# louislung/DAE_RNN_News_Recommendation

Measured on NVIDIA H100. Metric: articles/sec, higher is better.
Workload: dtype f32

## Files before the change

### dae_rnn_news_recommendation_b200/_cabi.py

```python
import ctypes
import ctypes as C
import os
from pathlib import Path

_PKG = Path(__file__).resolve().parent
LIB_PATH = Path(os.environ.get('DAE_SM100_LIB', _PKG / 'libdae_sm100.so'))

ACT = {'none': 0, 'sigmoid': 1, 'tanh': 2}
LOSS = {'cross_entropy': 0, 'mean_squared': 1, 'cosine_proximity': 2}
STRATEGY = {'none': 0, 'batch_all': 1, 'batch_hard': 2, 'explicit': 3}
OPT = {'gradient_descent': 0, 'ada_grad': 1, 'momentum': 2, 'adam': 3}
STAT = {'cost': 0, 'ae_loss': 1, 'triplet_loss': 2, 'fraction': 3, 'num': 4, 'sum_w': 5, 'n_valid': 6, 'sum_lw': 7,
        'triplet_sum': 8, 'n_active': 9}
STAT_SLOTS = 16
MAX_TRIPLET_BATCH = 32768
MAX_BLOCKED_BATCH = 262144


def act_code(name):
    return ACT.get(name, 0)


p, i32, i64, f32, u64, sz = C.c_void_p, C.c_int32, C.c_int64, C.c_float, C.c_uint64, C.c_size_t

_SIGNATURES = {
    'dae_version': (C.c_int, []),
    'dae_last_error': (C.c_int, [C.c_char_p, sz]),
    'dae_batch_prepare': (C.c_int, [p, i64, p, i32, p, i32, p, p, p, p, p, p, p]),
    'dae_batch_prepare_next': (C.c_int, [p, i64, i64, p, i32, p, i32, p, p, p, p, p, p, p]),
    'dae_batch_prepare_blocked': (C.c_int, [p, i64, p, i32, p, i32, p, p, p, p, p, p, p]),
    'dae_batch_prepare_next_blocked': (C.c_int, [p, i64, i64, p, i32, p, i32, p, p, p, p, p, p, p]),
    'dae_batch_commit': (C.c_int, [i32, p, p, p, p, p, p, p, p, p, p, p, p, p]),
    'dae_batch_prepare_explicit': (C.c_int, [p, i64, p, i32, i64, p, p, p]),
    'dae_step_advance': (C.c_int, [p, i64, p]),
    'dae_encode_csr_fwd': (C.c_int, [p, p, p, p, i32, i32, i32, f32, p, p, i32, p, i64, p, p, p, i64, p]),
    'dae_encode_csr_fwd_hot': (C.c_int, [p, p, p, i32, i32, i32, f32, p, p, i32, p, i64, p, p, i32, i32, p]),
    'dae_col_scan': (C.c_int, [p, i32, p, p, p]),
    'dae_encode_csr_bwd_gather': (C.c_int, [p, p, p, p, i32, i32, i32, f32, p, p, i32, p, p, i64, p, p, i32, p, p, p, p, p, p, p]),
    'dae_encode_csr_bwd': (C.c_int, [p, p, p, p, i32, i32, i32, f32, p, p, i32, p, p, i64, p, p, i32, p]),
    'dae_sgemm': (C.c_int, [i32, i32, i32, f32, p, i64, i64, p, i64, i64, f32, p, i64, p]),
    'dae_split_bf16': (C.c_int, [p, i32, i32, i64, p, p, i64, i32, f32, p]),
    'dae_sym_split_bf16': (C.c_int, [p, i32, i64, f32, p, p, i64, p]),
    'dae_gemm_bf16x3': (C.c_int, [i32, i32, i32, f32, p, p, i64, i32, p, p, i64, i32, p, i64, i32, i32, p, i32, i32, p]),
    'dae_gemm_config': (C.c_int, [i32, i32]),
    'dae_decode_prepare': (C.c_int, [i32, i32, p, p, p, p, p, p]),
    'dae_decode_fused_bf16x3': (C.c_int, [i32, i32, i32, p, p, i64, p, p, i64, p, p, p, p, p, i32, i32, p, p, p, p, i64, p, p, i32, p]),
    'dae_reduce_parts': (C.c_int, [p, i32, i32, p, p]),
    'dae_decode_loss_bwd': (C.c_int, [p, p, p, p, i32, i32, p, i32, i32, p, p, p, i64, p, p]),
    'dae_colsum': (C.c_int, [p, i32, i32, i64, p, p]),
    'dae_triplet_batch_all': (C.c_int, [p, i64, i32, p, p, p, i64, p, i32, p, p, i64, p]),
    'dae_triplet_config': (C.c_int, [i32]),
    'dae_gemm_sym_bf16x3': (C.c_int, [i32, i32, f32, p, p, i64, p, p, i64, p, i64, i32, p]),
    'dae_triplet_batch_hard': (C.c_int, [p, i64, i32, p, p, i64, p, p, p]),
    'dae_triplet_batch_all_rows': (C.c_int, [p, i64, i32, i32, i32, p, p, p, i64, p, i32, p, p, i64, p]),
    'dae_triplet_batch_hard_rows': (C.c_int, [p, i64, i32, i32, i32, p, p, i64, p, p, p]),
    'dae_triplet_batch_hard_finish': (C.c_int, [p, i32, p, p, i32, i64, p]),
    'dae_triplet_explicit': (C.c_int, [p, p, p, i32, i32, i64, f32, p, p, p, p, p]),
    'dae_step_finalize': (C.c_int, [p, p, i32, p, i32, i32, f32, p, p, p, p]),
    'dae_optimizer_step': (C.c_int, [p, p, p, p, i64, i32, f32, f32, f32, i32, p, p, p, i32, i32, i64, p]),
    'dae_rownorm_split_bf16': (C.c_int, [p, i32, i32, i64, i32, p, p, i64, p, i64, p]),
    'dae_row_argmax': (C.c_int, [p, i32, i32, i64, i64, i32, p, p, p]),
    'dae_similarity_topk_bf16x3': (C.c_int, [i32, i32, i32, p, p, i64, p, p, i64, i32, i64, i32, i32, p, i64, p, p, p]),
    'dae_similarity_topk_workspace': (C.c_int, [i32, i32, i32, i32, p]),
    'dae_csr_similarity_topk': (C.c_int, [p, p, p, i32, i64, i32, p, p, p, i32, i64, i32, i32, i64, i32, i32, p, i64, p, p, p]),
    'dae_csr_similarity_topk_workspace': (C.c_int, [i32, i32, i64, i32, i32, i32, p]),
    'dae_similarity_topk_excl_bf16x3': (C.c_int, [i32, i32, i32, p, p, i64, p, p, i64, i32, i64, i32, i32, p, i64, p, p, p, p, i64, p]),
    'dae_csr_similarity_topk_excl': (C.c_int, [p, p, p, i32, i64, i32, p, p, p, i32, i64, i32, i32, i64, i32, i32, p, i64, p, p, p, p,
                                               i64, p]),
    'dae_similarity_topk_groups_bf16x3': (C.c_int, [i32, i32, i32, p, p, i64, p, p, i64, i32, i64, i32, i32, p, i64, p, p, p, p, i64, p,
                                                    p]),
    'dae_csr_similarity_topk_groups': (C.c_int, [p, p, p, i32, i64, i32, p, p, p, i32, i64, i32, i32, i64, i32, i32, p, i64, p, p, p, p,
                                                 i64, p, p]),
    'dae_pair_partition': (C.c_int, [p, i64, i32, p, p, p, p, p]),
    'dae_auroc_count': (C.c_int, [p, i64, p, i64, i32, p, p]),
    'dae_similarity_pair_hist_bf16x3': (C.c_int, [i32, i32, p, p, i64, p, f32, i32, p, p, p]),
    'dae_csr_similarity_pair_hist': (C.c_int, [p, p, p, i32, i64, i32, p, f32, i32, p, i64, p, p, p]),
    'dae_csr_similarity_pair_hist_workspace': (C.c_int, [i32, i64, i32, p]),
    'dae_similarity_pairs_bf16x3': (C.c_int, [i32, i32, i32, p, p, i64, p, p, i64, i32, f32, p, i64, p, p, p, p]),
    'dae_csr_similarity_pairs': (C.c_int, [p, p, p, i32, i64, i32, p, p, p, i32, i64, i32, i32, f32, p, i64, p, i64, p, p, p, p]),
    'dae_csr_similarity_pairs_workspace': (C.c_int, [i32, i32, i64, i32, p]),
    'dae_pairs_sort': (C.c_int, [i64, i32, i32, p, p, p, p, p, i64, p, p]),
    'dae_pairs_sort_workspace': (C.c_int, [i64, i32, p]),
    'dae_allreduce_multimem': (C.c_int, [p, p, p, i32, i32, i64, i32, p]),
    'dae_mask_values': (C.c_int, [p, p, i64, f32, u64, u64, p, p]),
    'dae_salt_pepper_csr': (C.c_int, [p, p, p, i64, i64, i32, i64, f32, f32, p, u64, u64, p, p, p, i64, p, p, sz, p]),
    'dae_salt_pepper_workspace': (C.c_int, [i64, p]),
    'dae_gather_split_bf16': (C.c_int, [p, i64, p, i32, i32, p, p, i64, i32, p]),
    'dae_gru_cell_fwd': (C.c_int, [i32, i32, p, i64, p, i64, p, i64, p, i64, i32, p, p, i64, p, i64, p]),
    'dae_gru_cell_bwd': (C.c_int, [i32, i32, p, i64, p, i64, p, i64, p, i64, p, p, p, p, i64, p]),
    'dae_seq_negatives': (C.c_int, [p, i64, i32, u64, u64, u64, p, p]),
    'dae_seq_rank_loss': (C.c_int, [p, i64, p, i64, i32, p, p, i64, f32, p, i64, p, p]),
    'dae_gemm_det_workspace': (C.c_int, [p]),
    'dae_gemm_bf16x3_det': (C.c_int, [i32, i32, i32, f32, p, p, i64, i32, p, p, i64, i32, p, i64, i32, i32, p, i32, i32, p, i64, p]),
    'dae_gemm_sym_bf16x3_det': (C.c_int, [i32, i32, f32, p, p, i64, p, p, i64, p, i64, i32, p, i64, p]),
    'dae_decode_loss_parts': (C.c_int, [i32, p]),
    'dae_decode_fused_bf16x3_det': (C.c_int, [i32, i32, i32, p, p, i64, p, p, i64, p, p, p, p, p, i32, i32, p, p, p, p, i64, p, p, i32,
                                              p]),
    'dae_encode_csr_bwd_det_workspace': (C.c_int, [i32, i32, i32, i64, p]),
    'dae_encode_csr_bwd_det': (C.c_int, [p, p, p, p, i32, i32, i32, f32, p, p, i32, p, p, i64, p, p, i64, p, i64, p]),
    'dae_encode_sparse_dw_add': (C.c_int, [i32, i32, i32, i64, p, i64, p, p]),
    'dae_triplet_batch_all_det': (C.c_int, [p, i64, i32, p, p, p, i64, p, i32, p, p, i64, p, p]),
    'dae_triplet_batch_hard_det': (C.c_int, [p, i64, i32, p, p, i64, p, p, p, p]),
    'dae_triplet_batch_all_rows_det': (C.c_int, [p, i64, i32, i32, i32, p, p, p, i64, p, i32, p, p, i64, p, p]),
    'dae_triplet_batch_hard_rows_det': (C.c_int, [p, i64, i32, i32, i32, p, p, i64, p, p, p, p]),
    'dae_triplet_explicit_det': (C.c_int, [p, p, p, i32, i32, i64, f32, p, p, p, p, p, p]),
    'dae_triplet_loss_sum': (C.c_int, [p, i32, p, p]),
}


def query(name, *args, ctype=C.c_int64):
    out = ctype(0)
    call(name, *args, ctypes.addressof(out))
    return int(out.value)

_lib = None


class DaeError(RuntimeError):
    pass


def exported_symbols():
    return list(_SIGNATURES)


def lib():
    global _lib
    if _lib is None:
        if not LIB_PATH.exists():
            raise DaeError('%s not found: build it with `python -m dae_rnn_news_recommendation_b200.build` '
                           '(there is no CPU fallback)' % LIB_PATH)
        l = ctypes.CDLL(str(LIB_PATH))
        for name, (res, args) in _SIGNATURES.items():
            fn = getattr(l, name)
            fn.restype = res
            fn.argtypes = args
        _lib = l
    return _lib


def last_error():
    buf = ctypes.create_string_buffer(512)
    lib().dae_last_error(buf, 512)
    return buf.value.decode()


def call(name, *args):
    rc = getattr(lib(), name)(*args)
    if rc != 0:
        raise DaeError('%s failed (%d): %s' % (name, rc, last_error()))


def ptr(t):
    return None if t is None else t.data_ptr()
```

### dae_rnn_news_recommendation_b200/csrc/gemm_tc.cu

```cuda
#include <cuda.h>
#include <cuda_bf16.h>
#include <type_traits>
#include "common.cuh"
#include "pair_hist.cuh"
#include "pairs.cuh"
#include "topk.cuh"

namespace dae {

constexpr int BLOCK_M = 128;
constexpr int BLOCK_K = 64;
constexpr int WGMMA_K = 16;
constexpr int kThreads = 384;
constexpr int kDecodeN = 128;

__device__ __forceinline__ uint32_t smem_u32(const void* p) { return (uint32_t)__cvta_generic_to_shared(p); }

__device__ __forceinline__ void mbar_init(uint64_t* bar, uint32_t count) {
  asm volatile("mbarrier.init.shared::cta.b64 [%0], %1;" ::"r"(smem_u32(bar)), "r"(count));
}
__device__ __forceinline__ void mbar_expect_tx(uint64_t* bar, uint32_t bytes) {
  asm volatile("mbarrier.arrive.expect_tx.shared::cta.b64 _, [%0], %1;" ::"r"(smem_u32(bar)), "r"(bytes) : "memory");
}
__device__ __forceinline__ void mbar_arrive(uint64_t* bar) {
  asm volatile("mbarrier.arrive.shared::cta.b64 _, [%0];" ::"r"(smem_u32(bar)) : "memory");
}
__device__ __forceinline__ bool mbar_try_wait(uint64_t* bar, uint32_t parity) {
  uint32_t ok;
  asm volatile(
      "{\n"
      ".reg .pred p;\n"
      "mbarrier.try_wait.parity.shared::cta.b64 p, [%1], %2;\n"
      "selp.u32 %0, 1, 0, p;\n"
      "}\n"
      : "=r"(ok)
      : "r"(smem_u32(bar)), "r"(parity)
      : "memory");
  return ok != 0;
}
__device__ __forceinline__ void mbar_wait(uint64_t* bar, uint32_t parity) {
  uint32_t spins = 0;
  while (!mbar_try_wait(bar, parity)) {
    if (++spins > 4096u) {
      __nanosleep(64);
      if (spins > (1u << 26)) __trap();
    }
  }
}
__device__ __forceinline__ void fence_barrier_init() { asm volatile("fence.mbarrier_init.release.cluster;" ::: "memory"); }

__device__ __forceinline__ void tma_load_2d(const CUtensorMap* map, uint64_t* bar, void* dst, int c0, int c1) {
  asm volatile(
      "cp.async.bulk.tensor.2d.shared::cluster.global.mbarrier::complete_tx::bytes [%0], [%1, {%3, %4}], [%2];" ::"r"(smem_u32(dst)),
      "l"(map), "r"(smem_u32(bar)), "r"(c0), "r"(c1)
      : "memory");
}
__device__ __forceinline__ uint32_t cluster_ctarank() { uint32_t r; asm volatile("mov.u32 %0, %%cluster_ctarank;" : "=r"(r)); return r; }
__device__ __forceinline__ void cluster_sync_all() {
  asm volatile("barrier.cluster.arrive.release.aligned;" ::: "memory");
  asm volatile("barrier.cluster.wait.acquire.aligned;" ::: "memory");
}
__device__ __forceinline__ void tma_load_2d_mc(const CUtensorMap* map, uint64_t* bar, void* dst, int c0, int c1, uint16_t cta_mask) {
  asm volatile(
      "cp.async.bulk.tensor.2d.shared::cluster.global.mbarrier::complete_tx::bytes.multicast::cluster [%0], [%1, {%3, %4}], [%2], %5;" ::"r"(
          smem_u32(dst)),
      "l"(map), "r"(smem_u32(bar)), "r"(c0), "r"(c1), "h"(cta_mask)
      : "memory");
}
__device__ __forceinline__ void mbar_arrive_cluster(uint64_t* bar, uint32_t rank) {
  uint32_t raddr;
  asm volatile("mapa.shared::cluster.u32 %0, %1, %2;" : "=r"(raddr) : "r"(smem_u32(bar)), "r"(rank));
  asm volatile("mbarrier.arrive.release.cluster.shared::cluster.b64 _, [%0];" ::"r"(raddr) : "memory");
}
__device__ __forceinline__ void mbar_wait_cluster(uint64_t* bar, uint32_t parity) {
  uint32_t spins = 0;
  for (;;) {
    uint32_t ok;
    asm volatile(
        "{\n"
        ".reg .pred p;\n"
        "mbarrier.try_wait.parity.acquire.cluster.shared::cta.b64 p, [%1], %2;\n"
        "selp.u32 %0, 1, 0, p;\n"
        "}\n"
        : "=r"(ok)
        : "r"(smem_u32(bar)), "r"(parity)
        : "memory");
    if (ok) return;
    if (++spins > 4096u) { __nanosleep(64); if (spins > (1u << 26)) __trap(); }
  }
}

__device__ __forceinline__ void prefetch_tmap(const CUtensorMap* map) {
  asm volatile("prefetch.tensormap [%0];" ::"l"(map) : "memory");
}
__device__ __forceinline__ void named_bar_sync(int id, int threads) { asm volatile("bar.sync %0, %1;" ::"r"(id), "r"(threads) : "memory"); }

__device__ __forceinline__ void wgmma_fence() { asm volatile("wgmma.fence.sync.aligned;" ::: "memory"); }
__device__ __forceinline__ void wgmma_commit() { asm volatile("wgmma.commit_group.sync.aligned;" ::: "memory"); }
template <int N>
__device__ __forceinline__ void wgmma_wait() { asm volatile("wgmma.wait_group.sync.aligned %0;" ::"n"(N) : "memory"); }

__device__ __forceinline__ uint64_t make_desc(uint32_t saddr, uint32_t lbo_bytes, uint32_t sbo_bytes, uint32_t layout = 1) {
  uint64_t d = 0;
  d |= (uint64_t)((saddr >> 4) & 0x3FFF);
  d |= (uint64_t)((lbo_bytes >> 4) & 0x3FFF) << 16;
  d |= (uint64_t)((sbo_bytes >> 4) & 0x3FFF) << 32;
  d |= (uint64_t)layout << 62;
  return d;
}


template <int TA, int TB>
__device__ __forceinline__ void wgmma_n128(float (&d)[64], uint64_t da, uint64_t db, uint32_t scale_d) {
  asm volatile(
      "{\n"
      ".reg .pred p;\n"
      "setp.ne.b32 p, %66, 0;\n"
      "wgmma.mma_async.sync.aligned.m64n128k16.f32.bf16.bf16 "
      "{%0, %1, %2, %3, %4, %5, %6, %7, %8, %9, %10, %11, %12, %13, %14, %15, %16, %17, %18, %19, %20, %21, %22, %23, %24, %25, %26, %27, %28, %29, %30, %31, %32, %33, %34, %35, %36, %37, %38, %39, %40, %41, %42, %43, %44, %45, %46, %47, %48, %49, %50, %51, %52, %53, %54, %55, %56, %57, %58, %59, %60, %61, %62, %63}, %64, %65, p, 1, 1, %67, %68;\n"
      "}\n"
      : "+f"(d[0]), "+f"(d[1]), "+f"(d[2]), "+f"(d[3]), "+f"(d[4]), "+f"(d[5]), "+f"(d[6]), "+f"(d[7]), "+f"(d[8]), "+f"(d[9]), "+f"(d[10]), "+f"(d[11]), "+f"(d[12]), "+f"(d[13]), "+f"(d[14]), "+f"(d[15]), "+f"(d[16]), "+f"(d[17]), "+f"(d[18]), "+f"(d[19]), "+f"(d[20]), "+f"(d[21]), "+f"(d[22]), "+f"(d[23]), "+f"(d[24]), "+f"(d[25]), "+f"(d[26]), "+f"(d[27]), "+f"(d[28]), "+f"(d[29]), "+f"(d[30]), "+f"(d[31]), "+f"(d[32]), "+f"(d[33]), "+f"(d[34]), "+f"(d[35]), "+f"(d[36]), "+f"(d[37]), "+f"(d[38]), "+f"(d[39]), "+f"(d[40]), "+f"(d[41]), "+f"(d[42]), "+f"(d[43]), "+f"(d[44]), "+f"(d[45]), "+f"(d[46]), "+f"(d[47]), "+f"(d[48]), "+f"(d[49]), "+f"(d[50]), "+f"(d[51]), "+f"(d[52]), "+f"(d[53]), "+f"(d[54]), "+f"(d[55]), "+f"(d[56]), "+f"(d[57]), "+f"(d[58]), "+f"(d[59]), "+f"(d[60]), "+f"(d[61]), "+f"(d[62]), "+f"(d[63])
      : "l"(da), "l"(db), "r"(scale_d), "n"(TA), "n"(TB));
}

template <int TA, int TB>
__device__ __forceinline__ void wgmma_n64(float (&d)[32], uint64_t da, uint64_t db, uint32_t scale_d) {
  asm volatile(
      "{\n"
      ".reg .pred p;\n"
      "setp.ne.b32 p, %34, 0;\n"
      "wgmma.mma_async.sync.aligned.m64n64k16.f32.bf16.bf16 "
      "{%0, %1, %2, %3, %4, %5, %6, %7, %8, %9, %10, %11, %12, %13, %14, %15, %16, %17, %18, %19, %20, %21, %22, %23, %24, %25, %26, %27, %28, %29, %30, %31}, %32, %33, p, 1, 1, %35, %36;\n"
      "}\n"
      : "+f"(d[0]), "+f"(d[1]), "+f"(d[2]), "+f"(d[3]), "+f"(d[4]), "+f"(d[5]), "+f"(d[6]), "+f"(d[7]), "+f"(d[8]), "+f"(d[9]), "+f"(d[10]), "+f"(d[11]), "+f"(d[12]), "+f"(d[13]), "+f"(d[14]), "+f"(d[15]), "+f"(d[16]), "+f"(d[17]), "+f"(d[18]), "+f"(d[19]), "+f"(d[20]), "+f"(d[21]), "+f"(d[22]), "+f"(d[23]), "+f"(d[24]), "+f"(d[25]), "+f"(d[26]), "+f"(d[27]), "+f"(d[28]), "+f"(d[29]), "+f"(d[30]), "+f"(d[31])
      : "l"(da), "l"(db), "r"(scale_d), "n"(TA), "n"(TB));
}

struct GemmParams {
  int M, N, K;
  int k_splits;
  int stream_k;
  int atomic;
  int a_mn, b_mn;
  int a_sym_kb;
  float alpha;
  float* C;
  int64_t ldc;
  int n_store;
  int special_col;
  float* special_out;
  const int64_t* indptr; const int32_t* indices; const float* values; const int32_t* rows;
  const float* bv; const float* weight; const double* stats;
  __nv_bfloat16* dz_hi; __nv_bfloat16* dz_lo; int64_t ld_dz;
  float* row_loss_part;
  const int32_t* tile_ptr;
  float* sk_ws;
  int loss_parts;
};

struct Sched {
  int tiles_m, tiles, kb_total, kb_per_split, n_work, stream, w, n_cta;
  long long u, u_end;
  __device__ __forceinline__ void init(const GemmParams& p, int block_n, int pair = 0, int block_k = BLOCK_K) {
    const int cta = pair ? (int)(blockIdx.x >> 1) : (int)blockIdx.x;
    n_cta = pair ? (int)(gridDim.x >> 1) : (int)gridDim.x;
    tiles_m = (p.M + BLOCK_M - 1) / BLOCK_M;
    if (pair) tiles_m = (tiles_m + 1) / 2;
    tiles = tiles_m * ((p.N + block_n - 1) / block_n);
    kb_total = (p.K + block_k - 1) / block_k;
    stream = p.stream_k;
    kb_per_split = (kb_total + p.k_splits - 1) / p.k_splits;
    n_work = tiles * p.k_splits;
    w = cta;
    const long long U = (long long)tiles * kb_total;
    u = (long long)cta * U / n_cta;
    u_end = (long long)(cta + 1) * U / n_cta;
  }
  __device__ __forceinline__ bool next(int& mb, int& nb, int& kb0, int& kb1) {
    int tile;
    if (stream) {
      if (u >= u_end) return false;
      tile = (int)(u / kb_total);
      kb0 = (int)(u - (long long)tile * kb_total);
      const long long left = u_end - u;
      kb1 = (left < (long long)(kb_total - kb0)) ? kb0 + (int)left : kb_total;
      u += kb1 - kb0;
    } else {
      if (w >= n_work) return false;
      tile = w % tiles;
      kb0 = (w / tiles) * kb_per_split;
      kb1 = min(kb_total, kb0 + kb_per_split);
      w += n_cta;
    }
    mb = tile % tiles_m;
    nb = tile / tiles_m;
    return true;
  }
};

__device__ __forceinline__ uint32_t pack_bf16(float a, float b) {
  const __nv_bfloat162 v = __floats2bfloat162_rn(a, b);
  return *reinterpret_cast<const uint32_t*>(&v);
}
__device__ __forceinline__ float f_rcp(float x) { float r; asm("rcp.approx.ftz.f32 %0, %1;" : "=f"(r) : "f"(x)); return r; }
__device__ __forceinline__ float f_lg2(float x) { float r; asm("lg2.approx.ftz.f32 %0, %1;" : "=f"(r) : "f"(x)); return r; }
__device__ __forceinline__ float f_ex2(float x) { float r; asm("ex2.approx.ftz.f32 %0, %1;" : "=f"(r) : "f"(x)); return r; }
constexpr float kLog2e = 1.4426950408889634f;

template <int ACT>
__device__ __forceinline__ float act_fast(float z) {
  if (ACT == DAE_ACT_SIGMOID) return f_rcp(1.0f + f_ex2(-kLog2e * z));
  if (ACT == DAE_ACT_TANH) return 1.0f - 2.0f * f_rcp(1.0f + f_ex2(2.0f * kLog2e * z));
  return z;
}


__device__ __forceinline__ float select16(const uint32_t (&r)[16], int j) {
  uint32_t v = r[0];
#pragma unroll
  for (int k = 1; k < 16; ++k) v = (j == k) ? r[k] : v;
  return __uint_as_float(v);
}

template <int ACT, int LOSS>
__device__ __forceinline__ void decode_chunk_generic(const uint32_t (&r)[16], const float* __restrict__ bias, float sc, bool edge,
                                                     int n_lim, int nc, uint32_t (&hpk)[8], uint32_t (&lpk)[8], float& lsum) {
#pragma unroll
  for (int j2 = 0; j2 < 8; ++j2) {
    float dzp[2];
#pragma unroll
    for (int e = 0; e < 2; ++e) {
      const int j = 2 * j2 + e;
      const float z = __uint_as_float(r[j]) + bias[j];
      const float d = act_fast<ACT>(z);
      float dz, lt;
      if (LOSS == DAE_LOSS_CE) {
        const float omd = 1.0f - d;
        const float b = omd + kEps;
        lt = -f_lg2(b);
        dz = (ACT == DAE_ACT_SIGMOID) ? ((omd != 0.0f) ? sc * d : 0.0f) : sc * act_grad_from_y<ACT>(d) * f_rcp(b);
      } else {
        lt = d * d;
        dz = 2.0f * sc * d * act_grad_from_y<ACT>(d);
      }
      if (edge) { const bool in = (nc + j < n_lim); lt = in ? lt : 0.0f; dz = in ? dz : 0.0f; }
      lsum += lt;
      dzp[e] = dz;
    }
    const uint32_t hp = pack_bf16(dzp[0], dzp[1]);
    hpk[j2] = hp;
    lpk[j2] = pack_bf16(dzp[0] - __uint_as_float(hp << 16), dzp[1] - __uint_as_float(hp & 0xffff0000u));
  }
}

__device__ __forceinline__ bool decode_chunk_sigmoid_ce(const uint32_t (&r)[16], const float* __restrict__ biasc, float sc,
                                                        uint32_t (&hpk)[8], uint32_t (&lpk)[8], float& lsum) {
  bool ok = true;
#pragma unroll
  for (int g = 0; g < 4; ++g) {
    float t[4], a[4];
#pragma unroll
    for (int j = 0; j < 4; ++j) {
      t[j] = f_ex2(fmaf(__uint_as_float(r[4 * g + j]), kLog2e, biasc[4 * g + j]));
      a[j] = 1.0f + t[j];
    }
    const float p01 = a[0] * a[1], p23 = a[2] * a[3], P = p01 * p23;
    ok = ok && (P <= 22026.0f);
    const float Rs = f_rcp(P) * sc;
    lsum += f_lg2(P);
    const float r23 = Rs * p23, r01 = Rs * p01;
    const float dz0 = t[0] * (r23 * a[1]), dz1 = t[1] * (r23 * a[0]), dz2 = t[2] * (r01 * a[3]), dz3 = t[3] * (r01 * a[2]);
    const uint32_t h0 = pack_bf16(dz0, dz1), h1 = pack_bf16(dz2, dz3);
    hpk[2 * g] = h0; hpk[2 * g + 1] = h1;
    lpk[2 * g] = pack_bf16(dz0 - __uint_as_float(h0 << 16), dz1 - __uint_as_float(h0 & 0xffff0000u));
    lpk[2 * g + 1] = pack_bf16(dz2 - __uint_as_float(h1 << 16), dz3 - __uint_as_float(h1 & 0xffff0000u));
  }
  return ok;
}

template <int BLOCK_N, int TA, int TB, int BK = BLOCK_K>
__device__ __forceinline__ void mma_kblock(float (&acc)[BLOCK_N / 2], uint32_t sa_hi, uint32_t sa_lo, uint32_t sb_hi, uint32_t sb_lo,
                                           bool first) {
  static_assert(BK == 64 || BK == 32, "k-blocks are 32 or 64 wide");
  constexpr uint32_t kmaj_layout = BK == 64 ? 1u : 2u, kmaj_sbo = BK == 64 ? 1024u : 512u, mn_lbo = 64u * BK * 2u;
  constexpr uint32_t a_layout = TA ? 1u : kmaj_layout, b_layout = TB ? 1u : kmaj_layout;
  constexpr uint32_t a_sbo = TA ? 1024u : kmaj_sbo, b_sbo = TB ? 1024u : kmaj_sbo;
  constexpr uint32_t a_lbo = TA ? mn_lbo : 16u, b_lbo = TB ? mn_lbo : 16u;
  constexpr uint32_t a_step = TA ? 2048u : 32u, b_step = TB ? 2048u : 32u;
#pragma unroll
  for (int k = 0; k < BK / WGMMA_K; ++k) {
    const uint64_t da_hi = make_desc(sa_hi + k * a_step, a_lbo, a_sbo, a_layout), da_lo = make_desc(sa_lo + k * a_step, a_lbo, a_sbo, a_layout);
    const uint64_t db_hi = make_desc(sb_hi + k * b_step, b_lbo, b_sbo, b_layout), db_lo = make_desc(sb_lo + k * b_step, b_lbo, b_sbo, b_layout);
    const uint32_t sc = (first && k == 0) ? 0u : 1u;
    if constexpr (BLOCK_N == 128) {
      wgmma_n128<TA, TB>(acc, da_lo, db_hi, sc);
      wgmma_n128<TA, TB>(acc, da_hi, db_lo, 1u);
      wgmma_n128<TA, TB>(acc, da_hi, db_hi, 1u);
    } else {
      wgmma_n64<TA, TB>(acc, da_lo, db_hi, sc);
      wgmma_n64<TA, TB>(acc, da_hi, db_lo, 1u);
      wgmma_n64<TA, TB>(acc, da_hi, db_hi, 1u);
    }
  }
}

__device__ __forceinline__ void stage_ld16(const float* src, uint32_t (&r)[16]) {
#pragma unroll
  for (int q = 0; q < 4; ++q) {
    const float4 v = reinterpret_cast<const float4*>(src)[q];
    r[4 * q] = __float_as_uint(v.x); r[4 * q + 1] = __float_as_uint(v.y); r[4 * q + 2] = __float_as_uint(v.z); r[4 * q + 3] = __float_as_uint(v.w);
  }
}


template <int BLOCK_N, int STAGES, int PAIR, int BK = BLOCK_K, class SchedT>
__device__ __forceinline__ void tma_produce(const GemmParams& p, SchedT& sched, uint8_t* smem, uint64_t* full_bar, uint64_t* empty_bar,
                                            uint32_t crank, const CUtensorMap* tm_a_hi, const CUtensorMap* tm_a_lo,
                                            const CUtensorMap* tm_b_hi, const CUtensorMap* tm_b_lo, const CUtensorMap* tm_at_hi,
                                            const CUtensorMap* tm_at_lo) {
  constexpr int A_TILE = BLOCK_M * BK * 2;
  constexpr int B_TILE = BLOCK_N * BK * 2;
  constexpr int STAGE_BYTES = 2 * A_TILE + 2 * B_TILE;
  int stage = 0; uint32_t phase = 0;
  int mb, nb, kb0, kb1;
  while (sched.next(mb, nb, kb0, kb1)) {
    for (int kb = kb0; kb < kb1; ++kb) {
      if (PAIR) mbar_wait_cluster(&empty_bar[stage], phase ^ 1); else mbar_wait(&empty_bar[stage], phase ^ 1);
      uint8_t* sa_hi = smem + stage * STAGE_BYTES;
      uint8_t* sa_lo = sa_hi + A_TILE;
      uint8_t* sb_hi = sa_lo + A_TILE;
      uint8_t* sb_lo = sb_hi + B_TILE;
      const int mt = PAIR ? mb * 2 + (int)crank : mb;
      mbar_expect_tx(&full_bar[stage], STAGE_BYTES);
      if (p.a_sym_kb > 0 && kb >= p.a_sym_kb) {
#pragma unroll
        for (int j = 0; j < BLOCK_M / 64; ++j) {
          tma_load_2d(tm_at_hi, &full_bar[stage], sa_hi + j * (64 * BK * 2), mt * BLOCK_M + j * 64, (kb - p.a_sym_kb) * BK);
          tma_load_2d(tm_at_lo, &full_bar[stage], sa_lo + j * (64 * BK * 2), mt * BLOCK_M + j * 64, (kb - p.a_sym_kb) * BK);
        }
      } else if (!p.a_mn) {
        tma_load_2d(tm_a_hi, &full_bar[stage], sa_hi, kb * BK, mt * BLOCK_M);
        tma_load_2d(tm_a_lo, &full_bar[stage], sa_lo, kb * BK, mt * BLOCK_M);
      } else {
#pragma unroll
        for (int j = 0; j < BLOCK_M / 64; ++j) {
          tma_load_2d(tm_a_hi, &full_bar[stage], sa_hi + j * (64 * BK * 2), mt * BLOCK_M + j * 64, kb * BK);
          tma_load_2d(tm_a_lo, &full_bar[stage], sa_lo + j * (64 * BK * 2), mt * BLOCK_M + j * 64, kb * BK);
        }
      }
      const int kbb = (p.a_sym_kb > 0 && kb >= p.a_sym_kb) ? kb - p.a_sym_kb : kb;
      if (PAIR) {
        const int off = (int)crank * 8192, n_half = nb * BLOCK_N + (int)crank * 64;
        if (!p.b_mn) {
          tma_load_2d_mc(tm_b_hi, &full_bar[stage], sb_hi + off, kbb * BK, n_half, 0x3);
          tma_load_2d_mc(tm_b_lo, &full_bar[stage], sb_lo + off, kbb * BK, n_half, 0x3);
        } else {
          tma_load_2d_mc(tm_b_hi, &full_bar[stage], sb_hi + off, n_half, kbb * BK, 0x3);
          tma_load_2d_mc(tm_b_lo, &full_bar[stage], sb_lo + off, n_half, kbb * BK, 0x3);
        }
      } else if (!p.b_mn) {
        tma_load_2d(tm_b_hi, &full_bar[stage], sb_hi, kbb * BK, nb * BLOCK_N);
        tma_load_2d(tm_b_lo, &full_bar[stage], sb_lo, kbb * BK, nb * BLOCK_N);
      } else {
#pragma unroll
        for (int j = 0; j < BLOCK_N / 64; ++j) {
          tma_load_2d(tm_b_hi, &full_bar[stage], sb_hi + j * (64 * BK * 2), nb * BLOCK_N + j * 64, kbb * BK);
          tma_load_2d(tm_b_lo, &full_bar[stage], sb_lo + j * (64 * BK * 2), nb * BLOCK_N + j * 64, kbb * BK);
        }
      }
      if (++stage == STAGES) { stage = 0; phase ^= 1; }
    }
  }
}

template <int BLOCK_N, int STAGES, int PAIR, int MAJ, int BK = BLOCK_K>
__device__ __forceinline__ void mma_work_item(float (&acc)[BLOCK_N / 2], const GemmParams& p, uint8_t* smem, uint64_t* full_bar,
                                              uint64_t* empty_bar, int wg, int lane, uint32_t crank, int& stage, uint32_t& phase,
                                              int kb0, int kb1) {
  constexpr int A_TILE = BLOCK_M * BK * 2;
  constexpr int B_TILE = BLOCK_N * BK * 2;
  constexpr int STAGE_BYTES = 2 * A_TILE + 2 * B_TILE;
  auto release = [&](int s) {
    __syncwarp();
    if (lane == 0) { mbar_arrive(&empty_bar[s]); if (PAIR) mbar_arrive_cluster(&empty_bar[s], crank ^ 1u); }
  };
  int prev = -1;
  auto run_k = [&](auto ta, auto tb, int kb_begin, int kb_end) {
    for (int kb = kb_begin; kb < kb_end; ++kb) {
      mbar_wait(&full_bar[stage], phase);
      const uint32_t sa_hi = smem_u32(smem + stage * STAGE_BYTES) + wg * (64 * BK * 2);
      const uint32_t sa_lo = sa_hi + A_TILE;
      const uint32_t sb_hi = smem_u32(smem + stage * STAGE_BYTES) + 2 * A_TILE, sb_lo = sb_hi + B_TILE;
      wgmma_fence();
      mma_kblock<BLOCK_N, decltype(ta)::value, decltype(tb)::value, BK>(acc, sa_hi, sa_lo, sb_hi, sb_lo, kb == kb0);
      wgmma_commit();
      wgmma_wait<1>();
      if (prev >= 0) release(prev);
      prev = stage;
      if (++stage == STAGES) { stage = 0; phase ^= 1; }
    }
  };
  using K0 = std::integral_constant<int, 0>;
  using K1 = std::integral_constant<int, 1>;
  if constexpr ((MAJ & 4) != 0) {
    run_k(K0{}, K1{}, kb0, min(kb1, p.a_sym_kb));
    run_k(K1{}, K1{}, max(kb0, p.a_sym_kb), kb1);
  } else {
    run_k(std::integral_constant<int, MAJ & 1>{}, std::integral_constant<int, (MAJ >> 1) & 1>{}, kb0, kb1);
  }
  wgmma_wait<0>();
  if (prev >= 0) release(prev);
}

template <int BLOCK_N, int STAGES, int PAIR, int MAJ, int BK = BLOCK_K>
__global__ void __launch_bounds__(kThreads, 1) gemm_bf16x3_kernel(const __grid_constant__ CUtensorMap tm_a_hi,
                                                                   const __grid_constant__ CUtensorMap tm_a_lo,
                                                                   const __grid_constant__ CUtensorMap tm_b_hi,
                                                                   const __grid_constant__ CUtensorMap tm_b_lo,
                                                                   const __grid_constant__ CUtensorMap tm_at_hi,
                                                                   const __grid_constant__ CUtensorMap tm_at_lo,
                                                                   const GemmParams p) {
  static_assert(!PAIR || BLOCK_N == 128, "CTA pairs split the B tile into two 64-row halves");
  constexpr int STAGE_BYTES = 2 * BLOCK_M * BK * 2 + 2 * BLOCK_N * BK * 2;
  constexpr int SROW = BLOCK_N + 4;
  constexpr int kParts = 2;
  constexpr int HALF_N = BLOCK_N / kParts;
  extern __shared__ __align__(1024) uint8_t smem_raw[];
  uint8_t* smem = reinterpret_cast<uint8_t*>((reinterpret_cast<uintptr_t>(smem_raw) + 1023) & ~(uintptr_t)1023);
  float* stg = reinterpret_cast<float*>(smem + STAGES * STAGE_BYTES);
  __shared__ __align__(8) uint64_t full_bar[STAGES], empty_bar[STAGES];

  const int warp = threadIdx.x >> 5, lane = threadIdx.x & 31;
  Sched sched;
  sched.init(p, BLOCK_N, PAIR, BK);
  const uint32_t crank = PAIR ? cluster_ctarank() : 0u;

  if (warp == 0 && lane == 0) {
    prefetch_tmap(&tm_a_hi); prefetch_tmap(&tm_a_lo); prefetch_tmap(&tm_b_hi); prefetch_tmap(&tm_b_lo);
    if (p.a_sym_kb > 0) { prefetch_tmap(&tm_at_hi); prefetch_tmap(&tm_at_lo); }
  }
  if (warp == 1 && lane == 0) {
    for (int s = 0; s < STAGES; ++s) { mbar_init(&full_bar[s], 1); mbar_init(&empty_bar[s], PAIR ? 16 : 8); }
    fence_barrier_init();
  }
  if (PAIR) cluster_sync_all(); else __syncthreads();

  if (warp == 0) {
    if (lane == 0)
      tma_produce<BLOCK_N, STAGES, PAIR, BK>(p, sched, smem, full_bar, empty_bar, crank, &tm_a_hi, &tm_a_lo, &tm_b_hi, &tm_b_lo, &tm_at_hi,
                                         &tm_at_lo);
  } else if (warp >= 4) {
    const int wg = (warp >> 2) - 1;
    const int wi = warp & 3;
    const int quarter = wg * 2 + (wi & 1);
    const int half = wi >> 1;
    float acc[BLOCK_N / 2];
#pragma unroll
    for (int i = 0; i < BLOCK_N / 2; ++i) acc[i] = 0.0f;
    int stage = 0; uint32_t phase = 0;
    int mb, nb, kb0, kb1;
    int seg = 0;
    while (sched.next(mb, nb, kb0, kb1)) {
      if (PAIR) mb = mb * 2 + (int)crank;
      mma_work_item<BLOCK_N, STAGES, PAIR, MAJ, BK>(acc, p, smem, full_bar, empty_bar, wg, lane, crank, stage, phase, kb0, kb1);
      float* ws_tile = nullptr;
      if (p.sk_ws != nullptr && !(kb0 == 0 && kb1 == sched.kb_total))
        ws_tile = p.sk_ws + ((int64_t)blockIdx.x * 2 + (seg == 0 ? 0 : 1)) * (BLOCK_M * BLOCK_N);
      ++seg;

      named_bar_sync(1 + wg, 128);
      {
        const int r0 = wg * 64 + wi * 16 + (lane >> 2), c0 = 2 * (lane & 3);
#pragma unroll
        for (int j = 0; j < BLOCK_N / 8; ++j) {
          *reinterpret_cast<float2*>(&stg[r0 * SROW + 8 * j + c0]) = make_float2(acc[4 * j], acc[4 * j + 1]);
          *reinterpret_cast<float2*>(&stg[(r0 + 8) * SROW + 8 * j + c0]) = make_float2(acc[4 * j + 2], acc[4 * j + 3]);
        }
      }
      named_bar_sync(1 + wg, 128);
      const int n0 = nb * BLOCK_N + half * HALF_N;
      const float* tr = stg + (quarter * 32) * SROW + half * HALF_N;
      const int m_base = mb * BLOCK_M + quarter * 32;
      const bool vec_ok = ((p.ldc & 3) == 0) && ((reinterpret_cast<uintptr_t>(p.C) & 15) == 0);
#pragma unroll 1
      for (int c = 0; c < HALF_N / 16; ++c) {
        const int nc = n0 + c * 16;
        if (ws_tile != nullptr) {
          const int rsub = lane >> 4, csub = lane & 15;
          float* dst = ws_tile + (int64_t)(quarter * 32) * BLOCK_N + half * HALF_N + c * 16 + csub;
#pragma unroll 4
          for (int i = 0; i < 16; ++i) {
            const int rr = 2 * i + rsub;
            dst[(int64_t)rr * BLOCK_N] = p.alpha * tr[rr * SROW + c * 16 + csub];
          }
          continue;
        }
        const bool interior = vec_ok && (m_base + 32 <= p.M) && (nc + 16 <= p.n_store) && (p.special_col < nc || p.special_col >= nc + 16);
        if (interior) {
          const int rsub = lane >> 2, c4 = (lane & 3) * 4;
          float* dst = p.C + (int64_t)(m_base + rsub) * p.ldc + nc + c4;
          const int64_t step = 8 * p.ldc;
#pragma unroll
          for (int i = 0; i < 4; ++i) {
            float4 v = *reinterpret_cast<const float4*>(&tr[(rsub + 8 * i) * SROW + c * 16 + c4]);
            v.x *= p.alpha; v.y *= p.alpha; v.z *= p.alpha; v.w *= p.alpha;
            if (p.atomic) atomicAdd(reinterpret_cast<float4*>(dst), v); else *reinterpret_cast<float4*>(dst) = v;
            dst += step;
          }
        } else {
          const int rsub = lane >> 4, csub = lane & 15;
          const int n = nc + csub;
          for (int i = 0; i < 16; ++i) {
            const int rr = 2 * i + rsub;
            const int mm = m_base + rr;
            const float v = p.alpha * tr[rr * SROW + c * 16 + csub];
            if (mm < p.M) {
              if (n == p.special_col) {
                if (p.atomic) atomicAdd(p.special_out + mm, v); else p.special_out[mm] = v;
              } else if (n < p.n_store) {
                float* dst = p.C + (int64_t)mm * p.ldc + n;
                if (p.atomic) atomicAdd(dst, v); else *dst = v;
              }
            }
          }
        }
      }
    }
  }

  if (PAIR) cluster_sync_all();
}

constexpr int kDecodeThreads = 640;
constexpr int kDecodeBK = 32;
constexpr int kDecodeStages = 4;
constexpr int kRegsProducer = 32, kRegsMma = 104, kRegsEpilogue = 120;
static_assert(128 * kRegsProducer + 256 * kRegsMma + 256 * kRegsEpilogue <= kDecodeThreads * 96, "register budget");

template <int R> __device__ __forceinline__ void regs_dec() { asm volatile("setmaxnreg.dec.sync.aligned.u32 %0;" ::"n"(R)); }
template <int R> __device__ __forceinline__ void regs_inc() { asm volatile("setmaxnreg.inc.sync.aligned.u32 %0;" ::"n"(R)); }

template <int ACT, int LOSS>
__global__ void __launch_bounds__(kDecodeThreads, 1) decode_fused_kernel(const __grid_constant__ CUtensorMap tm_a_hi,
                                                                         const __grid_constant__ CUtensorMap tm_a_lo,
                                                                         const __grid_constant__ CUtensorMap tm_b_hi,
                                                                         const __grid_constant__ CUtensorMap tm_b_lo,
                                                                         const GemmParams p) {
  constexpr int BLOCK_N = kDecodeN, STAGES = kDecodeStages, BK = kDecodeBK;
  constexpr int STAGE_BYTES = 2 * BLOCK_M * BK * 2 + 2 * BLOCK_N * BK * 2;
  constexpr int SROW = BLOCK_N + 4;
  constexpr int kParts = 2;
  constexpr int HALF_N = BLOCK_N / kParts;
  constexpr bool kFast = (ACT == DAE_ACT_SIGMOID) && (LOSS == DAE_LOSS_CE);
  extern __shared__ __align__(1024) uint8_t smem_raw[];
  uint8_t* smem = reinterpret_cast<uint8_t*>((reinterpret_cast<uintptr_t>(smem_raw) + 1023) & ~(uintptr_t)1023);
  float* stg = reinterpret_cast<float*>(smem + STAGES * STAGE_BYTES);
  __shared__ __align__(8) uint64_t full_bar[STAGES], empty_bar[STAGES], staged_bar[2], drained_bar[2];
  __shared__ float s_bias[2][BLOCK_N];
  __shared__ float s_biasc[kFast ? 2 : 1][kFast ? BLOCK_N : 1];
  __shared__ __align__(16) uint8_t s_stage[8][2][32][48];

  const int warp = threadIdx.x >> 5, lane = threadIdx.x & 31;
  const int role = warp >> 2;
  Sched sched;

  if (warp == 0 && lane == 0) { prefetch_tmap(&tm_a_hi); prefetch_tmap(&tm_a_lo); prefetch_tmap(&tm_b_hi); prefetch_tmap(&tm_b_lo); }
  if (warp == 1 && lane == 0) {
    for (int s = 0; s < STAGES; ++s) { mbar_init(&full_bar[s], 1); mbar_init(&empty_bar[s], 8); }
    for (int h = 0; h < 2; ++h) { mbar_init(&staged_bar[h], 4); mbar_init(&drained_bar[h], 4); }
    fence_barrier_init();
  }
  __syncthreads();

  if (role == 0) {
    regs_dec<kRegsProducer>();
    sched.init(p, BLOCK_N, 0, BK);
    if (warp == 0 && lane == 0)
      tma_produce<BLOCK_N, STAGES, 0, BK>(p, sched, smem, full_bar, empty_bar, 0u, &tm_a_hi, &tm_a_lo, &tm_b_hi, &tm_b_lo, &tm_a_hi, &tm_a_lo);
  } else if (role <= 2) {
    regs_inc<kRegsMma>();
    sched.init(p, BLOCK_N, 0, BK);
    const int h = role - 1;
    const int wi = warp & 3;
    float acc[BLOCK_N / 2];
#pragma unroll
    for (int i = 0; i < BLOCK_N / 2; ++i) acc[i] = 0.0f;
    int stage = 0; uint32_t phase = 0, tphase = 0;
    int mb, nb, kb0, kb1;
    while (sched.next(mb, nb, kb0, kb1)) {
      mma_work_item<BLOCK_N, STAGES, 0, 0, BK>(acc, p, smem, full_bar, empty_bar, h, lane, 0u, stage, phase, kb0, kb1);
      mbar_wait(&drained_bar[h], tphase ^ 1);
      const int r0 = h * 64 + wi * 16 + (lane >> 2), c0 = 2 * (lane & 3);
#pragma unroll
      for (int j = 0; j < BLOCK_N / 8; ++j) {
        *reinterpret_cast<float2*>(&stg[r0 * SROW + 8 * j + c0]) = make_float2(acc[4 * j], acc[4 * j + 1]);
        *reinterpret_cast<float2*>(&stg[(r0 + 8) * SROW + 8 * j + c0]) = make_float2(acc[4 * j + 2], acc[4 * j + 3]);
      }
      __syncwarp();
      if (lane == 0) mbar_arrive(&staged_bar[h]);
      tphase ^= 1;
    }
  } else {
    regs_inc<kRegsEpilogue>();
    sched.init(p, BLOCK_N, 0, BK);
    const int h = role - 3;
    const int ew = warp - 12;
    const int wi = warp & 3;
    const int quarter = h * 2 + (wi & 1);
    const int half = wi >> 1;
    const int row_in_tile = quarter * 32 + lane;
    const int tid = threadIdx.x - 128 * role;
    const int tiles_n = (p.N + BLOCK_N - 1) / BLOCK_N;
    uint8_t* stg_hi = reinterpret_cast<uint8_t*>(&s_stage[ew][0][0][0]);
    uint8_t* stg_lo = reinterpret_cast<uint8_t*>(&s_stage[ew][1][0][0]);
    const int rsub = lane >> 1, csub = lane & 1;
    uint32_t tphase = 0;
    int mb, nb, kb0, kb1;
    while (sched.next(mb, nb, kb0, kb1)) {
      const float* srow = stg + row_in_tile * SROW + half * HALF_N;
      const int m = mb * BLOCK_M + row_in_tile;
      const int n0 = nb * BLOCK_N + half * HALF_N;
      int64_t pc = 0, pe = 0;
      int c0 = 0x7fffffff, c1 = 0x7fffffff, c2 = 0x7fffffff;
      float v0 = 0.0f, v1 = 0.0f, v2 = 0.0f;
      float sc = 0.0f;
      if (m < p.M) {
        const int64_t row = p.rows ? (int64_t)p.rows[m] : (int64_t)m;
        const int64_t rbeg = p.indptr[row];
        const int32_t* tp = p.tile_ptr + (int64_t)m * (kParts * tiles_n + 1) + nb * kParts + half;
        pc = rbeg + tp[0]; pe = rbeg + tp[1];
        if (pc < pe) { c0 = p.indices[pc]; v0 = p.values[pc]; }
        if (pc + 1 < pe) { c1 = p.indices[pc + 1]; v1 = p.values[pc + 1]; }
        if (pc + 2 < pe) { c2 = p.indices[pc + 2]; v2 = p.values[pc + 2]; }
        sc = (p.weight ? p.weight[m] : 1.0f) / ((float)p.stats[DAE_STAT_SUM_W] + kEps);
      }
      named_bar_sync(1 + h, 128);
      {
        const float b = (nb * BLOCK_N + tid < p.N) ? p.bv[nb * BLOCK_N + tid] : 0.0f;
        s_bias[h][tid] = b;
        if (kFast) s_biasc[h][tid] = b * kLog2e;
      }
      mbar_wait(&staged_bar[h], tphase);
      named_bar_sync(1 + h, 128);
      const float inv_sc = (sc != 0.0f) ? 1.0f / sc : 0.0f;
      const bool edge = (n0 + HALF_N > p.N);
      float lsum = 0.0f;
      const int m_base = mb * BLOCK_M + quarter * 32;
      const int n_lim = edge ? p.N : 0x7fffffff;
#pragma unroll 1
      for (int c = 0; c < HALF_N / 16; ++c) {
        uint32_t r[16];
        stage_ld16(srow + c * 16, r);
        const int nc = n0 + c * 16;
        if (m < p.M) {
          const float* bias = &s_bias[h][half * HALF_N + c * 16];
          uint32_t hpk[8], lpk[8];
          bool fast_ok = false;
          if (kFast && !edge) {
            const float l0 = lsum;
            fast_ok = decode_chunk_sigmoid_ce(r, &s_biasc[h][half * HALF_N + c * 16], sc, hpk, lpk, lsum);
            if (!fast_ok) { lsum = l0; decode_chunk_generic<ACT, LOSS>(r, bias, sc, edge, n_lim, nc, hpk, lpk, lsum); }
          } else {
            decode_chunk_generic<ACT, LOSS>(r, bias, sc, edge, n_lim, nc, hpk, lpk, lsum);
          }
          uint4* sh = reinterpret_cast<uint4*>(stg_hi + lane * 48);
          uint4* sl = reinterpret_cast<uint4*>(stg_lo + lane * 48);
          sh[0] = make_uint4(hpk[0], hpk[1], hpk[2], hpk[3]); sh[1] = make_uint4(hpk[4], hpk[5], hpk[6], hpk[7]);
          sl[0] = make_uint4(lpk[0], lpk[1], lpk[2], lpk[3]); sl[1] = make_uint4(lpk[4], lpk[5], lpk[6], lpk[7]);
          while (c0 < nc + 16) {
            const float x = v0;
            const int j = c0 - nc;
            __nv_bfloat16* ph = reinterpret_cast<__nv_bfloat16*>(stg_hi + lane * 48) + j;
            __nv_bfloat16* pl = reinterpret_cast<__nv_bfloat16*>(stg_lo + lane * 48) + j;
            float d;
            if (kFast && fast_ok && sc != 0.0f) d = (__bfloat162float(*ph) + __bfloat162float(*pl)) * inv_sc;
            else d = act_fast<ACT>(select16(r, j) + bias[j]);
            const float gp = act_grad_from_y<ACT>(d);
            float dz;
            if (LOSS == DAE_LOSS_CE) {
              const float a = d + kEps, b = (1.0f - d) + kEps;
              const float la = f_lg2(a), lb = f_lg2(b);
              lsum += lb - (x * la + (1.0f - x) * lb);
              dz = sc * gp * ((1.0f - x) * f_rcp(b) - x * f_rcp(a));
            } else {
              const float e2 = x - d;
              lsum += e2 * e2 - d * d;
              dz = -2.0f * sc * e2 * gp;
            }
            const __nv_bfloat16 hb = __float2bfloat16_rn(dz);
            *ph = hb;
            *pl = __float2bfloat16_rn(dz - __bfloat162float(hb));
            ++pc;
            c0 = c1; v0 = v1; c1 = c2; v1 = v2;
            c2 = 0x7fffffff;
            if (pc + 2 < pe) { c2 = p.indices[pc + 2]; v2 = p.values[pc + 2]; }
          }
        }
        __syncwarp();
        if (nc < p.ld_dz) {
#pragma unroll
          for (int i = 0; i < 2; ++i) {
            const int rr = rsub + 16 * i;
            if (m_base + rr < p.M) {
              const int64_t off = (int64_t)(m_base + rr) * p.ld_dz + nc + csub * 8;
              *reinterpret_cast<uint4*>(p.dz_hi + off) = *reinterpret_cast<const uint4*>(stg_hi + rr * 48 + csub * 16);
              *reinterpret_cast<uint4*>(p.dz_lo + off) = *reinterpret_cast<const uint4*>(stg_lo + rr * 48 + csub * 16);
            }
          }
        }
        __syncwarp();
      }
      if (lane == 0) mbar_arrive(&drained_bar[h]);
      tphase ^= 1;
      if (m < p.M) {
        const float l = (LOSS == DAE_LOSS_CE) ? lsum * 0.6931471805599453f : lsum;
        if (p.loss_parts) p.row_loss_part[(int64_t)(nb * kParts + half) * p.M + m] = l;
        else atomicAdd(p.row_loss_part + m, l);
      }
    }
  }
}

constexpr int kTopkMaxK = 32;
constexpr int kTopkMaxSplits = 32;
constexpr int kTopkMinTiles = 4;
constexpr int kTopkBK = 64;
constexpr int kTopkStages = 2;

struct TopkParams {
  GemmParams g;
  int k, splits;
  int exclude;
  int64_t diag_offset;
  float* ws_val; int32_t* ws_idx;
  const int64_t* ex_indptr; const int32_t* ex_indices;
  const int32_t* groups;
};

struct TopkSched {
  int tiles_n, splits, kb_total, n_work, n_cta, w;
  int mb, split, t, t_end;
  bool first, last;
  __device__ __forceinline__ void init(const TopkParams& tp, int block_n, int block_k) {
    const int tiles_m = (tp.g.M + BLOCK_M - 1) / BLOCK_M;
    tiles_n = (tp.g.N + block_n - 1) / block_n;
    splits = tp.splits;
    kb_total = (tp.g.K + block_k - 1) / block_k;
    n_work = tiles_m * splits;
    n_cta = (int)gridDim.x;
    w = (int)blockIdx.x - n_cta;
    mb = split = t = t_end = 0;
    first = last = false;
  }
  __device__ __forceinline__ bool next(int& mb_, int& nb, int& kb0, int& kb1) {
    first = false;
    if (t >= t_end) {
      w += n_cta;
      if (w >= n_work) return false;
      mb = w / splits;
      split = w - mb * splits;
      t = split * tiles_n / splits;
      t_end = (split + 1) * tiles_n / splits;
      first = true;
    }
    mb_ = mb; nb = t; kb0 = 0; kb1 = kb_total;
    last = (++t == t_end);
    return true;
  }
};

template <int KMAX>
__device__ __forceinline__ void topk_offer(float (&sv)[KMAX], int (&si)[KMAX], float& thr, int k, float v, int col, int n_lim,
                                           int excl) {
  if (!(v > thr) || col >= n_lim || col == excl) return;
#pragma unroll
  for (int j = KMAX - 1; j >= 0; --j) {
    const bool up = (j > 0) && (v > sv[j > 0 ? j - 1 : 0]);
    const bool here = v > sv[j];
    si[j] = up ? si[j > 0 ? j - 1 : 0] : (here ? col : si[j]);
    sv[j] = up ? sv[j > 0 ? j - 1 : 0] : (here ? v : sv[j]);
  }
  float t = sv[0];
#pragma unroll
  for (int j = 1; j < KMAX; ++j)
    asm("{\n.reg .pred q;\nsetp.eq.s32 q, %1, %2;\nselp.f32 %0, %3, %0, q;\n}\n" : "+f"(t) : "r"(j), "r"(k - 1), "f"(sv[j]));
  thr = t;
}

template <int KMAX, bool REG>
__device__ __forceinline__ void topk_offer_group(float (&sv)[KMAX], int (&si)[KMAX], int (&sg)[REG ? KMAX : 1], float& thr, int k,
                                                 float v, int col, int g, int n_lim, int excl, const int32_t* __restrict__ groups) {
  if (!(v > thr) || col >= n_lim || col == excl) return;
  int gp = KMAX - 1;
  bool drop = false;
#pragma unroll
  for (int j = 0; j < KMAX; ++j) {
    if (j < k) {
      const int gj = REG ? sg[REG ? j : 0] : (si[j] >= 0 ? __ldg(groups + si[j]) : -1);
      if (gj == g) { gp = j; drop = !(v > sv[j]); }
    }
  }
  if (drop) return;
#pragma unroll
  for (int j = KMAX - 1; j >= 0; --j) {
    const bool up = (j > 0) && j <= gp && (v > sv[j > 0 ? j - 1 : 0]);
    const bool here = j <= gp && v > sv[j];
    si[j] = up ? si[j > 0 ? j - 1 : 0] : (here ? col : si[j]);
    if constexpr (REG) sg[REG ? j : 0] = up ? sg[REG && j > 0 ? j - 1 : 0] : (here ? g : sg[REG ? j : 0]);
    sv[j] = up ? sv[j > 0 ? j - 1 : 0] : (here ? v : sv[j]);
  }
  float t = sv[0];
#pragma unroll
  for (int j = 1; j < KMAX; ++j)
    asm("{\n.reg .pred q;\nsetp.eq.s32 q, %1, %2;\nselp.f32 %0, %3, %0, q;\n}\n" : "+f"(t) : "r"(j), "r"(k - 1), "f"(sv[j]));
  thr = t;
}

template <int KMAX, bool EXCL = false, bool GROUPS = false>
__global__ void __launch_bounds__(kDecodeThreads, 1) topk_kernel(const __grid_constant__ CUtensorMap tm_a_hi,
                                                                 const __grid_constant__ CUtensorMap tm_a_lo,
                                                                 const __grid_constant__ CUtensorMap tm_b_hi,
                                                                 const __grid_constant__ CUtensorMap tm_b_lo,
                                                                 const TopkParams tp) {
  constexpr int BLOCK_N = kDecodeN, STAGES = kTopkStages, BK = kTopkBK;
  constexpr int STAGE_BYTES = 2 * BLOCK_M * BK * 2 + 2 * BLOCK_N * BK * 2;
  constexpr int SROW = BLOCK_N + 4;
  constexpr int HALF_N = BLOCK_N / 2;
  const GemmParams& p = tp.g;
  extern __shared__ __align__(1024) uint8_t smem_raw[];
  uint8_t* smem = reinterpret_cast<uint8_t*>((reinterpret_cast<uintptr_t>(smem_raw) + 1023) & ~(uintptr_t)1023);
  float* stg = reinterpret_cast<float*>(smem + STAGES * STAGE_BYTES);
  __shared__ __align__(8) uint64_t full_bar[STAGES], empty_bar[STAGES], staged_bar[2], drained_bar[2];

  const int warp = threadIdx.x >> 5, lane = threadIdx.x & 31;
  const int role = warp >> 2;
  TopkSched sched;

  if (warp == 0 && lane == 0) { prefetch_tmap(&tm_a_hi); prefetch_tmap(&tm_a_lo); prefetch_tmap(&tm_b_hi); prefetch_tmap(&tm_b_lo); }
  if (warp == 1 && lane == 0) {
    for (int s = 0; s < STAGES; ++s) { mbar_init(&full_bar[s], 1); mbar_init(&empty_bar[s], 8); }
    for (int h = 0; h < 2; ++h) { mbar_init(&staged_bar[h], 4); mbar_init(&drained_bar[h], 4); }
    fence_barrier_init();
  }
  __syncthreads();

  if (role == 0) {
    regs_dec<kRegsProducer>();
    sched.init(tp, BLOCK_N, BK);
    if (warp == 0 && lane == 0)
      tma_produce<BLOCK_N, STAGES, 0, BK>(p, sched, smem, full_bar, empty_bar, 0u, &tm_a_hi, &tm_a_lo, &tm_b_hi, &tm_b_lo, &tm_a_hi, &tm_a_lo);
  } else if (role <= 2) {
    regs_inc<kRegsMma>();
    sched.init(tp, BLOCK_N, BK);
    const int h = role - 1;
    const int wi = warp & 3;
    float acc[BLOCK_N / 2];
#pragma unroll
    for (int i = 0; i < BLOCK_N / 2; ++i) acc[i] = 0.0f;
    int stage = 0; uint32_t phase = 0, tphase = 0;
    int mb, nb, kb0, kb1;
    while (sched.next(mb, nb, kb0, kb1)) {
      mma_work_item<BLOCK_N, STAGES, 0, 0, BK>(acc, p, smem, full_bar, empty_bar, h, lane, 0u, stage, phase, kb0, kb1);
      mbar_wait(&drained_bar[h], tphase ^ 1);
      const int r0 = h * 64 + wi * 16 + (lane >> 2), c0 = 2 * (lane & 3);
#pragma unroll
      for (int j = 0; j < BLOCK_N / 8; ++j) {
        *reinterpret_cast<float2*>(&stg[r0 * SROW + 8 * j + c0]) = make_float2(acc[4 * j], acc[4 * j + 1]);
        *reinterpret_cast<float2*>(&stg[(r0 + 8) * SROW + 8 * j + c0]) = make_float2(acc[4 * j + 2], acc[4 * j + 3]);
      }
      __syncwarp();
      if (lane == 0) mbar_arrive(&staged_bar[h]);
      tphase ^= 1;
    }
  } else {
    regs_inc<kRegsEpilogue>();
    sched.init(tp, BLOCK_N, BK);
    const int h = role - 3;
    const int wi = warp & 3;
    const int quarter = h * 2 + (wi & 1);
    const int half = wi >> 1;
    const int row_in_tile = quarter * 32 + lane;
    const int k = tp.k;
    const float* srow = stg + row_in_tile * SROW + half * HALF_N;
    float sv[KMAX];
    int si[KMAX];
    constexpr bool REG_GROUPS = GROUPS && KMAX <= 16;
    [[maybe_unused]] int sg[REG_GROUPS ? KMAX : 1];
    [[maybe_unused]] __shared__ __align__(16) int32_t s_grp[8][HALF_N];
    [[maybe_unused]] const int ew = warp - 12;
    float thr = neg_inf();
    int m = 0, excl = -1;
    [[maybe_unused]] int64_t ex_cur = 0, ex_end = 0;
    [[maybe_unused]] int ex_next = INT_MAX;
    uint32_t tphase = 0;
    int mb, nb, kb0, kb1;
    while (sched.next(mb, nb, kb0, kb1)) {
      if (sched.first) {
#pragma unroll
        for (int j = 0; j < KMAX; ++j) { sv[j] = neg_inf(); si[j] = -1; }
        if constexpr (REG_GROUPS) {
#pragma unroll
          for (int j = 0; j < KMAX; ++j) sg[j] = -1;
        }
        thr = neg_inf();
        m = mb * BLOCK_M + row_in_tile;
        const int64_t e = (int64_t)m + tp.diag_offset;
        excl = (tp.exclude && e >= 0 && e < p.N) ? (int)e : -1;
        if constexpr (EXCL) {
          ex_next = INT_MAX;
          if (m < p.M && (!GROUPS || tp.ex_indptr)) {
            const int c_first = nb * BLOCK_N + half * HALF_N;
            int64_t lo = tp.ex_indptr[m], hi = tp.ex_indptr[m + 1];
            ex_end = hi;
            while (lo < hi) {
              const int64_t mid = lo + ((hi - lo) >> 1);
              if (tp.ex_indices[mid] < c_first) lo = mid + 1; else hi = mid;
            }
            ex_cur = lo;
            if (ex_cur < ex_end) ex_next = tp.ex_indices[ex_cur];
          }
        }
      }
      const int n0 = nb * BLOCK_N + half * HALF_N;
      if constexpr (GROUPS) {
        const int j0 = n0 + lane, j1 = n0 + 32 + lane;
        s_grp[ew][lane] = j0 < p.N ? tp.groups[j0] : -1;
        s_grp[ew][lane + 32] = j1 < p.N ? tp.groups[j1] : -1;
        __syncwarp();
      }
      mbar_wait(&staged_bar[h], tphase);
      if (m < p.M) {
        if constexpr (EXCL) {
          float* wrow = stg + row_in_tile * SROW + half * HALF_N;
          while (ex_next < n0 + HALF_N) {
            if (ex_next >= n0) wrow[ex_next - n0] = neg_inf();
            ex_next = (++ex_cur < ex_end) ? tp.ex_indices[ex_cur] : INT_MAX;
          }
        }
#pragma unroll 1
        for (int c = 0; c < HALF_N; c += 4) {
          const float4 v = *reinterpret_cast<const float4*>(srow + c);
          if (fmaxf(fmaxf(v.x, v.y), fmaxf(v.z, v.w)) > thr) {
            if constexpr (GROUPS) {
              const int4 g = *reinterpret_cast<const int4*>(&s_grp[ew][c]);
              topk_offer_group<KMAX, REG_GROUPS>(sv, si, sg, thr, k, v.x, n0 + c, g.x, p.N, excl, tp.groups);
              topk_offer_group<KMAX, REG_GROUPS>(sv, si, sg, thr, k, v.y, n0 + c + 1, g.y, p.N, excl, tp.groups);
              topk_offer_group<KMAX, REG_GROUPS>(sv, si, sg, thr, k, v.z, n0 + c + 2, g.z, p.N, excl, tp.groups);
              topk_offer_group<KMAX, REG_GROUPS>(sv, si, sg, thr, k, v.w, n0 + c + 3, g.w, p.N, excl, tp.groups);
            } else {
              topk_offer<KMAX>(sv, si, thr, k, v.x, n0 + c, p.N, excl);
// ... 100 lines not shown
      for (int j = 0; j < BLOCK_N / 8; ++j) {
        *reinterpret_cast<float2*>(&stg[r0 * SROW + 8 * j + c0]) = make_float2(acc[4 * j], acc[4 * j + 1]);
        *reinterpret_cast<float2*>(&stg[(r0 + 8) * SROW + 8 * j + c0]) = make_float2(acc[4 * j + 2], acc[4 * j + 3]);
      }
      __syncwarp();
      if (lane == 0) mbar_arrive(&staged_bar[h]);
      tphase ^= 1;
    }
  } else {
    regs_inc<kRegsEpilogue>();
    sched.init(hp, BK);
    const int h = role - 3;
    const int ew = warp - 12;
    const int wi = warp & 3;
    const int quarter = h * 2 + (wi & 1);
    const int half = wi >> 1;
    const int row_in_tile = quarter * 32 + lane;
    const float* srow = stg + row_in_tile * SROW + half * HALF_N;
    const float range = hp.range, scale = hp.scale;
    const uint32_t bins = hp.bins;
    uint32_t tphase = 0;
    int mb, nb, kb0, kb1;
    while (sched.next(mb, nb, kb0, kb1)) {
      const int i = mb * BLOCK_M + row_in_tile;
      const int n0 = nb * BLOCK_N + half * HALF_N;
      {
        const int j0 = n0 + lane, j1 = n0 + 32 + lane;
        s_lab[ew][lane] = j0 < p.N ? hp.labels[j0] : -1;
        s_lab[ew][lane + 32] = j1 < p.N ? hp.labels[j1] : -1;
      }
      const int li = i < p.N ? hp.labels[i] : -1;
      const int c_end = li < 0 ? 0 : min(HALF_N, i - n0);
      __syncwarp();
      double sum_rel = 0.0, sum_unrel = 0.0;
      uint32_t run_key = 0, run_n = 0;
      auto offer = [&](float s, int lj, bool in) {
        if (!in || lj < 0) return;
        const bool rel = (lj == li);
        const uint32_t key = (rel ? 0u : bins) + pair_bin(s, range, scale, bins);
        if (rel) sum_rel += (double)s; else sum_unrel += (double)s;
        if (key != run_key && run_n) { red_add_u64(hp.hist + run_key, run_n); run_n = 0; }
        run_key = key;
        ++run_n;
      };
      mbar_wait(&staged_bar[h], tphase);
#pragma unroll 1
      for (int c = 0; c < c_end; c += 4) {
        const float4 v = *reinterpret_cast<const float4*>(srow + c);
        const int4 l = *reinterpret_cast<const int4*>(&s_lab[ew][c]);
        offer(v.x, l.x, true);
        offer(v.y, l.y, c + 1 < c_end);
        offer(v.z, l.z, c + 2 < c_end);
        offer(v.w, l.w, c + 3 < c_end);
      }
      __syncwarp();
      if (lane == 0) mbar_arrive(&drained_bar[h]);
      tphase ^= 1;
      if (run_n) red_add_u64(hp.hist + run_key, run_n);
      sum_rel = warp_sum(sum_rel);
      sum_unrel = warp_sum(sum_unrel);
      if (lane == 0) {
        if (sum_rel != 0.0) atomicAdd(hp.sums, sum_rel);
        if (sum_unrel != 0.0) atomicAdd(hp.sums + 1, sum_unrel);
      }
    }
  }
}

struct PairsParams {
  GemmParams g;
  int self;
  float tau;
  unsigned long long* count;
  unsigned long long capacity;
  int32_t* i_out; int32_t* j_out; float* s_out;
};

struct PairsSched {
  long long t, n_tiles;
  int tiles_n, self, n_cta, kb_total;
  __device__ __forceinline__ void init(const PairsParams& pp, int block_n, int block_k) {
    const long long tm = (pp.g.M + BLOCK_M - 1) / BLOCK_M;
    tiles_n = (pp.g.N + block_n - 1) / block_n;
    self = pp.self;
    n_tiles = self ? tm * (tm + 1) / 2 : tm * tiles_n;
    kb_total = (pp.g.K + block_k - 1) / block_k;
    n_cta = (int)gridDim.x;
    t = blockIdx.x;
  }
  __device__ __forceinline__ bool next(int& mb, int& nb, int& kb0, int& kb1) {
    if (t >= n_tiles) return false;
    if (self) {
      long long r = (long long)((sqrt(8.0 * (double)t + 1.0) - 1.0) * 0.5);
      while (r * (r + 1) / 2 > t) --r;
      while ((r + 1) * (r + 2) / 2 <= t) ++r;
      mb = (int)r;
      nb = (int)(t - r * (r + 1) / 2);
    } else {
      mb = (int)(t / tiles_n);
      nb = (int)(t - (long long)mb * tiles_n);
    }
    kb0 = 0; kb1 = kb_total;
    t += n_cta;
    return true;
  }
};

__global__ void __launch_bounds__(kDecodeThreads, 1) pairs_kernel(const __grid_constant__ CUtensorMap tm_a_hi,
                                                                  const __grid_constant__ CUtensorMap tm_a_lo,
                                                                  const __grid_constant__ CUtensorMap tm_b_hi,
                                                                  const __grid_constant__ CUtensorMap tm_b_lo,
                                                                  const PairsParams pp) {
  constexpr int BLOCK_N = kDecodeN, STAGES = kTopkStages, BK = kTopkBK;
  constexpr int STAGE_BYTES = 2 * BLOCK_M * BK * 2 + 2 * BLOCK_N * BK * 2;
  constexpr int SROW = BLOCK_N + 4;
  constexpr int HALF_N = BLOCK_N / 2;
  const GemmParams& p = pp.g;
  extern __shared__ __align__(1024) uint8_t smem_raw[];
  uint8_t* smem = reinterpret_cast<uint8_t*>((reinterpret_cast<uintptr_t>(smem_raw) + 1023) & ~(uintptr_t)1023);
  float* stg = reinterpret_cast<float*>(smem + STAGES * STAGE_BYTES);
  __shared__ __align__(8) uint64_t full_bar[STAGES], empty_bar[STAGES], staged_bar[2], drained_bar[2];

  const int warp = threadIdx.x >> 5, lane = threadIdx.x & 31;
  const int role = warp >> 2;
  PairsSched sched;

  if (warp == 0 && lane == 0) { prefetch_tmap(&tm_a_hi); prefetch_tmap(&tm_a_lo); prefetch_tmap(&tm_b_hi); prefetch_tmap(&tm_b_lo); }
  if (warp == 1 && lane == 0) {
    for (int s = 0; s < STAGES; ++s) { mbar_init(&full_bar[s], 1); mbar_init(&empty_bar[s], 8); }
    for (int h = 0; h < 2; ++h) { mbar_init(&staged_bar[h], 4); mbar_init(&drained_bar[h], 4); }
    fence_barrier_init();
  }
  __syncthreads();

  if (role == 0) {
    regs_dec<kRegsProducer>();
    sched.init(pp, BLOCK_N, BK);
    if (warp == 0 && lane == 0)
      tma_produce<BLOCK_N, STAGES, 0, BK>(p, sched, smem, full_bar, empty_bar, 0u, &tm_a_hi, &tm_a_lo, &tm_b_hi, &tm_b_lo, &tm_a_hi, &tm_a_lo);
  } else if (role <= 2) {
    regs_inc<kRegsMma>();
    sched.init(pp, BLOCK_N, BK);
    const int h = role - 1;
    const int wi = warp & 3;
    float acc[BLOCK_N / 2];
#pragma unroll
    for (int i = 0; i < BLOCK_N / 2; ++i) acc[i] = 0.0f;
    int stage = 0; uint32_t phase = 0, tphase = 0;
    int mb, nb, kb0, kb1;
    while (sched.next(mb, nb, kb0, kb1)) {
      mma_work_item<BLOCK_N, STAGES, 0, 0, BK>(acc, p, smem, full_bar, empty_bar, h, lane, 0u, stage, phase, kb0, kb1);
      mbar_wait(&drained_bar[h], tphase ^ 1);
      const int r0 = h * 64 + wi * 16 + (lane >> 2), c0 = 2 * (lane & 3);
#pragma unroll
      for (int j = 0; j < BLOCK_N / 8; ++j) {
        *reinterpret_cast<float2*>(&stg[r0 * SROW + 8 * j + c0]) = make_float2(acc[4 * j], acc[4 * j + 1]);
        *reinterpret_cast<float2*>(&stg[(r0 + 8) * SROW + 8 * j + c0]) = make_float2(acc[4 * j + 2], acc[4 * j + 3]);
      }
      __syncwarp();
      if (lane == 0) mbar_arrive(&staged_bar[h]);
      tphase ^= 1;
    }
  } else {
    regs_inc<kRegsEpilogue>();
    sched.init(pp, BLOCK_N, BK);
    const int h = role - 3;
    const int wi = warp & 3;
    const int quarter = h * 2 + (wi & 1);
    const int half = wi >> 1;
    const int row_in_tile = quarter * 32 + lane;
    const float* srow = stg + row_in_tile * SROW + half * HALF_N;
    const float tau = pp.tau;
    uint32_t tphase = 0;
    int mb, nb, kb0, kb1;
    while (sched.next(mb, nb, kb0, kb1)) {
      const int i = mb * BLOCK_M + row_in_tile;
      const int n0 = nb * BLOCK_N + half * HALF_N;
      const int lim = pp.self ? i : p.N;
      const int c_end = i < p.M ? max(0, min(HALF_N, lim - n0)) : 0;
      mbar_wait(&staged_bar[h], tphase);
      int hits = 0;
#pragma unroll 1
      for (int c = 0; c < c_end; c += 4) {
        const float4 v = *reinterpret_cast<const float4*>(srow + c);
        if (fmaxf(fmaxf(v.x, v.y), fmaxf(v.z, v.w)) >= tau)
          hits += (v.x >= tau) + (c + 1 < c_end && v.y >= tau) + (c + 2 < c_end && v.z >= tau) + (c + 3 < c_end && v.w >= tau);
      }
      if (__any_sync(0xffffffffu, hits != 0)) {
        unsigned long long slot = pair_slots(pp.count, hits);
        if (hits) {
#pragma unroll 1
          for (int c = 0; c < c_end; ++c) {
            const float s = srow[c];
            if (s >= tau) pair_put(slot++, pp.capacity, i, n0 + c, s, pp.i_out, pp.j_out, pp.s_out);
          }
        }
      }
      __syncwarp();
      if (lane == 0) mbar_arrive(&drained_bar[h]);
      tphase ^= 1;
    }
  }
}

__global__ void decode_tile_ptr_kernel(const int64_t* __restrict__ indptr, const int32_t* __restrict__ indices,
                                       const int32_t* __restrict__ rows, int M, int n_half_tiles, int half_n,
                                       int32_t* __restrict__ tile_ptr) {
  const int t = blockIdx.x * blockDim.x + threadIdx.x;
  if (t > n_half_tiles) return;
  for (int m = blockIdx.y; m < M; m += gridDim.y) {
    const int64_t row = rows ? (int64_t)rows[m] : (int64_t)m;
    const int64_t b = indptr[row], e = indptr[row + 1];
    const int target = t * half_n;
    int64_t lo = b, hi = e;
    while (lo < hi) { const int64_t mid = (lo + hi) >> 1; if (indices[mid] < target) lo = mid + 1; else hi = mid; }
    tile_ptr[(int64_t)m * (n_half_tiles + 1) + t] = (int32_t)(lo - b);
  }
}

__global__ void split_bf16_kernel(const float* __restrict__ src, int rows, int cols, int64_t ld_src, __nv_bfloat16* __restrict__ hi,
                                  __nv_bfloat16* __restrict__ lo, int64_t ld_dst, int ones_col, float scale) {
  const int64_t total = (int64_t)rows * ld_dst;
  for (int64_t i = (int64_t)blockIdx.x * blockDim.x + threadIdx.x; i < total; i += (int64_t)gridDim.x * blockDim.x) {
    const int64_t r = i / ld_dst;
    const int c = (int)(i - r * ld_dst);
    float v = (c < cols) ? src[r * ld_src + c] * scale : 0.0f;
    if (c == ones_col) v = 1.0f;
    const __nv_bfloat16 h = __float2bfloat16_rn(v);
    hi[i] = h;
    lo[i] = __float2bfloat16_rn(v - __bfloat162float(h));
  }
}

__global__ void sym_split_kernel(const float* __restrict__ G, int B, int64_t ldg, float alpha, __nv_bfloat16* __restrict__ hi,
                                 __nv_bfloat16* __restrict__ lo, int64_t ld) {
  __shared__ float t[32][33];
  const int bx = blockIdx.x * 32, by = blockIdx.y * 32;
  const int tx = threadIdx.x, ty = threadIdx.y;
  for (int j = ty; j < 32; j += 8) {
    const int r = bx + j, c = by + tx;
    t[j][tx] = (r < B && c < B) ? G[(int64_t)r * ldg + c] : 0.0f;
  }
  __syncthreads();
  for (int j = ty; j < 32; j += 8) {
    const int r = by + j, c = bx + tx;
    if (r < B && c < ld) {
      float v = 0.0f;
      if (c < B) v = alpha * (G[(int64_t)r * ldg + c] + t[tx][j]);
      const __nv_bfloat16 h = __float2bfloat16_rn(v);
      hi[(int64_t)r * ld + c] = h;
      lo[(int64_t)r * ld + c] = __float2bfloat16_rn(v - __bfloat162float(h));
    }
  }
}

typedef CUresult (*PFN_encodeTiled)(CUtensorMap*, CUtensorMapDataType, cuuint32_t, void*, const cuuint64_t*, const cuuint64_t*,
                                    const cuuint32_t*, const cuuint32_t*, CUtensorMapInterleave, CUtensorMapSwizzle,
                                    CUtensorMapL2promotion, CUtensorMapFloatOOBfill);

static PFN_encodeTiled get_encode() {
  static PFN_encodeTiled fn = nullptr;
  if (!fn) {
    void* sym = nullptr;
    cudaDriverEntryPointQueryResult q;
    if (cudaGetDriverEntryPoint("cuTensorMapEncodeTiled", &sym, cudaEnableDefault, &q) == cudaSuccess && q == cudaDriverEntryPointSuccess)
      fn = reinterpret_cast<PFN_encodeTiled>(sym);
  }
  return fn;
}

static int make_map(CUtensorMap* m, const void* base, uint64_t inner, uint64_t outer, uint64_t ld, uint32_t box_outer,
                    uint32_t box_inner = 64) {
  PFN_encodeTiled enc = get_encode();
  if (!enc) { set_error("cuTensorMapEncodeTiled entry point not found"); return DAE_ERR_CUDA; }
  cuuint64_t dims[2] = {inner, outer};
  cuuint64_t strides[1] = {ld * 2};
  cuuint32_t box[2] = {box_inner, box_outer};
  cuuint32_t estr[2] = {1, 1};
  CUresult r = enc(m, CU_TENSOR_MAP_DATA_TYPE_BFLOAT16, 2, const_cast<void*>(base), dims, strides, box, estr,
                   CU_TENSOR_MAP_INTERLEAVE_NONE, box_inner == 64 ? CU_TENSOR_MAP_SWIZZLE_128B : CU_TENSOR_MAP_SWIZZLE_64B,
                   CU_TENSOR_MAP_L2_PROMOTION_L2_256B,
                   CU_TENSOR_MAP_FLOAT_OOB_FILL_NONE);
  if (r != CUDA_SUCCESS) { set_error("cuTensorMapEncodeTiled failed (%d): inner=%llu outer=%llu ld=%llu", (int)r,
                                     (unsigned long long)inner, (unsigned long long)outer, (unsigned long long)ld); return DAE_ERR_CUDA; }
  return DAE_OK;
}

struct Operand { const void* hi; const void* lo; int64_t ld; int mn_major; };

template <typename Kern>
static int ensure_smem_attr(Kern kern, int smem, bool (&done)[64]) {
  int dev = 0;
  DAE_CUDA(cudaGetDevice(&dev));
  if (dev < 0 || dev >= 64 || !done[dev]) {
    DAE_CUDA(cudaFuncSetAttribute(kern, cudaFuncAttributeMaxDynamicSharedMemorySize, smem));
    if (dev >= 0 && dev < 64) done[dev] = true;
  }
  return DAE_OK;
}


static int g_pair_mode = -1;
static int g_lean = 0;

template <int BLOCK_N, int STAGES, int PAIR, int MAJ, int BK = BLOCK_K>
static int launch_gemm_maj(const Operand& A, const Operand& B, GemmParams p, cudaStream_t st, int* grid_out = nullptr) {
  CUtensorMap ta_hi, ta_lo, tb_hi, tb_lo;
  int rc;
  constexpr int B_ROWS = PAIR ? BLOCK_N / 2 : BLOCK_N;
  if (!A.mn_major) {
    const uint64_t a_cols = p.a_sym_kb > 0 ? (uint64_t)p.M : (uint64_t)p.K;
    if ((rc = make_map(&ta_hi, A.hi, a_cols, p.M, A.ld, BLOCK_M, BK))) return rc;
    if ((rc = make_map(&ta_lo, A.lo, a_cols, p.M, A.ld, BLOCK_M, BK))) return rc;
  } else {
    if ((rc = make_map(&ta_hi, A.hi, p.M, p.K, A.ld, BK))) return rc;
    if ((rc = make_map(&ta_lo, A.lo, p.M, p.K, A.ld, BK))) return rc;
  }
  if (!B.mn_major) {
    if ((rc = make_map(&tb_hi, B.hi, p.K, p.N, B.ld, B_ROWS, BK))) return rc;
    if ((rc = make_map(&tb_lo, B.lo, p.K, p.N, B.ld, B_ROWS, BK))) return rc;
  } else {
    const uint64_t b_rows = p.a_sym_kb > 0 ? (uint64_t)p.M : (uint64_t)p.K;
    if ((rc = make_map(&tb_hi, B.hi, p.N, b_rows, B.ld, BK))) return rc;
    if ((rc = make_map(&tb_lo, B.lo, p.N, b_rows, B.ld, BK))) return rc;
  }
  p.a_mn = A.mn_major; p.b_mn = B.mn_major;
  CUtensorMap tat_hi = ta_hi, tat_lo = ta_lo;
  if (p.a_sym_kb > 0) {
    if (PAIR || A.mn_major) { set_error("dae_gemm_sym_bf16x3: unsupported configuration"); return DAE_ERR_UNSUPPORTED; }
    if ((rc = make_map(&tat_hi, A.hi, p.M, p.M, A.ld, 64))) return rc;
    if ((rc = make_map(&tat_lo, A.lo, p.M, p.M, A.ld, 64))) return rc;
  }
  constexpr int smem = STAGES * (2 * BLOCK_M * BK * 2 + 2 * BLOCK_N * BK * 2) + BLOCK_M * (BLOCK_N + 4) * 4 + 1024;
  int tiles_m = (p.M + BLOCK_M - 1) / BLOCK_M;
  if (PAIR) tiles_m = (tiles_m + 1) / 2;
  const int tiles_n = (p.N + BLOCK_N - 1) / BLOCK_N;
  const int kblocks = (p.K + BK - 1) / BK;
  auto kern = gemm_bf16x3_kernel<BLOCK_N, STAGES, PAIR, MAJ, BK>;
  static bool attr_done[64] = {false};
  if ((rc = ensure_smem_attr(kern, smem, attr_done))) return rc;
  const int slots = PAIR ? sm_count() / 2 : sm_count();
  int n;
  if (p.stream_k) {
    const long long units = (long long)tiles_m * tiles_n * kblocks;
    long long g = units / (6 * BLOCK_K / BK);
    if (g < 1) g = 1;
    n = (int)(g < slots ? g : slots);
  } else {
    const int items = tiles_m * tiles_n * p.k_splits;
    n = items < slots ? items : slots;
  }
  if (grid_out) *grid_out = n;
  if (!PAIR) {
    kern<<<n, kThreads, smem, st>>>(ta_hi, ta_lo, tb_hi, tb_lo, tat_hi, tat_lo, p);
  } else {
    cudaLaunchConfig_t cfg{};
    cfg.gridDim = dim3(2 * n); cfg.blockDim = dim3(kThreads); cfg.dynamicSmemBytes = smem; cfg.stream = st;
    cudaLaunchAttribute at[1];
    at[0].id = cudaLaunchAttributeClusterDimension;
    at[0].val.clusterDim.x = 2; at[0].val.clusterDim.y = 1; at[0].val.clusterDim.z = 1;
    cfg.attrs = at; cfg.numAttrs = 1;
    DAE_CUDA(cudaLaunchKernelEx(&cfg, kern, ta_hi, ta_lo, tb_hi, tb_lo, tat_hi, tat_lo, p));
  }
  return DAE_OK;
}

template <int BLOCK_N, int STAGES, int PAIR, int BK = BLOCK_K>
static int launch_gemm(const Operand& A, const Operand& B, GemmParams p, cudaStream_t st, int* grid_out = nullptr) {
  if (!A.mn_major && !B.mn_major) return launch_gemm_maj<BLOCK_N, STAGES, PAIR, 0, BK>(A, B, p, st, grid_out);
  if (A.mn_major && !B.mn_major) return launch_gemm_maj<BLOCK_N, STAGES, PAIR, 1, BK>(A, B, p, st, grid_out);
  if (!A.mn_major) return launch_gemm_maj<BLOCK_N, STAGES, PAIR, 2, BK>(A, B, p, st, grid_out);
  return launch_gemm_maj<BLOCK_N, STAGES, PAIR, 3, BK>(A, B, p, st, grid_out);
}

constexpr int kMaxFixupCtas = 1024;
constexpr int kFixupSlices = 16;

template <int BLOCK_N>
__global__ void __launch_bounds__(256) sk_fixup_kernel(const GemmParams p, int tiles_m, int tiles, int kb_total, int n_cta) {
  __shared__ int s_slot[kMaxFixupCtas];
  __shared__ int s_n;
  const int t = blockIdx.x;
  if (threadIdx.x == 0) {
    const long long U = (long long)tiles * kb_total, T0 = (long long)t * kb_total, T1 = T0 + kb_total;
    auto u_of = [&](int c) { return (long long)c * U / n_cta; };
    int c0 = (int)(T0 * n_cta / U);
    while (c0 + 1 < n_cta && u_of(c0 + 1) <= T0) ++c0;
    while (c0 > 0 && u_of(c0) > T0) --c0;
    int n = 0;
    if (u_of(c0 + 1) < T1) {
      for (int c = c0; c < n_cta && u_of(c) < T1; ++c) {
        if (u_of(c + 1) == u_of(c)) continue;
        s_slot[n++] = 2 * c + (u_of(c) >= T0 ? 0 : 1);
      }
    }
    s_n = n;
  }
  __syncthreads();
  const int n = s_n;
  if (n == 0) return;
  const int mb = t % tiles_m, nb = t / tiles_m;
  constexpr int kPer = BLOCK_M * BLOCK_N / kFixupSlices;
  for (int e = blockIdx.y * kPer + threadIdx.x; e < (blockIdx.y + 1) * kPer; e += blockDim.x) {
    const int m = mb * BLOCK_M + e / BLOCK_N, col = nb * BLOCK_N + e % BLOCK_N;
    if (m >= p.M || (col != p.special_col && col >= p.n_store)) continue;
    float s = p.sk_ws[(int64_t)s_slot[0] * (BLOCK_M * BLOCK_N) + e];
    for (int i = 1; i < n; ++i) s = s + p.sk_ws[(int64_t)s_slot[i] * (BLOCK_M * BLOCK_N) + e];
    float* dst = (col == p.special_col) ? p.special_out + m : p.C + (int64_t)m * p.ldc + col;
    *dst = p.atomic ? *dst + s : s;
  }
}

static int64_t sk_workspace_bytes() { return (int64_t)2 * sm_count() * BLOCK_M * 128 * (int64_t)sizeof(float); }

template <int ACT, int LOSS>
static int launch_decode(const Operand& A, const Operand& B, const GemmParams& p, cudaStream_t st) {
  CUtensorMap ta_hi, ta_lo, tb_hi, tb_lo;
  int rc;
  if ((rc = make_map(&ta_hi, A.hi, p.K, p.M, A.ld, BLOCK_M, kDecodeBK))) return rc;
  if ((rc = make_map(&ta_lo, A.lo, p.K, p.M, A.ld, BLOCK_M, kDecodeBK))) return rc;
  if ((rc = make_map(&tb_hi, B.hi, p.K, p.N, B.ld, kDecodeN, kDecodeBK))) return rc;
  if ((rc = make_map(&tb_lo, B.lo, p.K, p.N, B.ld, kDecodeN, kDecodeBK))) return rc;
  constexpr int smem = kDecodeStages * (2 * BLOCK_M * kDecodeBK * 2 + 2 * kDecodeN * kDecodeBK * 2) + BLOCK_M * (kDecodeN + 4) * 4 + 1024;
  auto kern = decode_fused_kernel<ACT, LOSS>;
  static bool attr_done[64] = {false};
  if ((rc = ensure_smem_attr(kern, smem, attr_done))) return rc;
  const int tiles = ((p.M + BLOCK_M - 1) / BLOCK_M) * ((p.N + kDecodeN - 1) / kDecodeN);
  const int n = tiles < sm_count() ? tiles : sm_count();
  kern<<<n, kDecodeThreads, smem, st>>>(ta_hi, ta_lo, tb_hi, tb_lo, p);
  return DAE_OK;
}

template <int KMAX, bool EXCL, bool GROUPS = false>
static int launch_topk(const Operand& A, const Operand& B, const TopkParams& tp, cudaStream_t st) {
  CUtensorMap ta_hi, ta_lo, tb_hi, tb_lo;
  int rc;
  const GemmParams& p = tp.g;
  if ((rc = make_map(&ta_hi, A.hi, p.K, p.M, A.ld, BLOCK_M, kTopkBK))) return rc;
  if ((rc = make_map(&ta_lo, A.lo, p.K, p.M, A.ld, BLOCK_M, kTopkBK))) return rc;
  if ((rc = make_map(&tb_hi, B.hi, p.K, p.N, B.ld, kDecodeN, kTopkBK))) return rc;
  if ((rc = make_map(&tb_lo, B.lo, p.K, p.N, B.ld, kDecodeN, kTopkBK))) return rc;
  constexpr int smem = kTopkStages * (2 * BLOCK_M * kTopkBK * 2 + 2 * kDecodeN * kTopkBK * 2) + BLOCK_M * (kDecodeN + 4) * 4 + 1024;
  auto kern = topk_kernel<KMAX, EXCL, GROUPS>;
  static bool attr_done[64] = {false};
  if ((rc = ensure_smem_attr(kern, smem, attr_done))) return rc;
  const int items = ((p.M + BLOCK_M - 1) / BLOCK_M) * tp.splits;
  const int n = items < sm_count() ? items : sm_count();
  kern<<<n, kDecodeThreads, smem, st>>>(ta_hi, ta_lo, tb_hi, tb_lo, tp);
  return DAE_OK;
}

static int launch_pair_hist(const Operand& X, const PairHistParams& hp, cudaStream_t st) {
  CUtensorMap ta_hi, ta_lo, tb_hi, tb_lo;
  int rc;
  const GemmParams& p = hp.g;
  if ((rc = make_map(&ta_hi, X.hi, p.K, p.M, X.ld, BLOCK_M, kTopkBK))) return rc;
  if ((rc = make_map(&ta_lo, X.lo, p.K, p.M, X.ld, BLOCK_M, kTopkBK))) return rc;
  if ((rc = make_map(&tb_hi, X.hi, p.K, p.N, X.ld, kDecodeN, kTopkBK))) return rc;
  if ((rc = make_map(&tb_lo, X.lo, p.K, p.N, X.ld, kDecodeN, kTopkBK))) return rc;
  constexpr int smem = kTopkStages * (2 * BLOCK_M * kTopkBK * 2 + 2 * kDecodeN * kTopkBK * 2) + BLOCK_M * (kDecodeN + 4) * 4 + 1024;
  static bool attr_done[64] = {false};
  if ((rc = ensure_smem_attr(pair_hist_kernel, smem, attr_done))) return rc;
  const long long tm = (p.M + BLOCK_M - 1) / BLOCK_M, tiles = tm * (tm + 1) / 2;
  const int n = tiles < sm_count() ? (int)tiles : sm_count();
  pair_hist_kernel<<<n, kDecodeThreads, smem, st>>>(ta_hi, ta_lo, tb_hi, tb_lo, hp);
  return DAE_OK;
}

static int launch_pairs(const Operand& A, const Operand& B, const PairsParams& pp, cudaStream_t st) {
  CUtensorMap ta_hi, ta_lo, tb_hi, tb_lo;
  int rc;
  const GemmParams& p = pp.g;
  if ((rc = make_map(&ta_hi, A.hi, p.K, p.M, A.ld, BLOCK_M, kTopkBK))) return rc;
  if ((rc = make_map(&ta_lo, A.lo, p.K, p.M, A.ld, BLOCK_M, kTopkBK))) return rc;
  if ((rc = make_map(&tb_hi, B.hi, p.K, p.N, B.ld, kDecodeN, kTopkBK))) return rc;
  if ((rc = make_map(&tb_lo, B.lo, p.K, p.N, B.ld, kDecodeN, kTopkBK))) return rc;
  constexpr int smem = kTopkStages * (2 * BLOCK_M * kTopkBK * 2 + 2 * kDecodeN * kTopkBK * 2) + BLOCK_M * (kDecodeN + 4) * 4 + 1024;
  static bool attr_done[64] = {false};
  if ((rc = ensure_smem_attr(pairs_kernel, smem, attr_done))) return rc;
  const long long tm = (p.M + BLOCK_M - 1) / BLOCK_M, tn = (p.N + kDecodeN - 1) / kDecodeN;
  const long long tiles = pp.self ? tm * (tm + 1) / 2 : tm * tn;
  const int n = tiles < sm_count() ? (int)tiles : sm_count();
  pairs_kernel<<<n, kDecodeThreads, smem, st>>>(ta_hi, ta_lo, tb_hi, tb_lo, pp);
  return DAE_OK;
}

static int topk_splits(int n_query, int n_corpus, int requested) {
  const int tiles_m = (n_query + BLOCK_M - 1) / BLOCK_M, tiles_n = (n_corpus + kDecodeN - 1) / kDecodeN;
  int s = requested;
  if (s <= 0) {
    s = (sm_count() + tiles_m - 1) / tiles_m;
    const int by_len = tiles_n / kTopkMinTiles;
    if (s > by_len) s = by_len;
  }
  if (s > tiles_n) s = tiles_n;
  if (s > kTopkMaxSplits) s = kTopkMaxSplits;
  return s < 1 ? 1 : s;
}

static int64_t topk_workspace_bytes(int n_query, int k, int splits) {
  return (int64_t)n_query * 2 * splits * k * (int64_t)(sizeof(float) + sizeof(int32_t));
}

static bool use_pair() { return g_pair_mode == 1 && !g_lean; }

}

using namespace dae;

extern "C" int dae_split_bf16(const float* src, int32_t rows, int32_t cols, int64_t ld_src, void* hi, void* lo, int64_t ld_dst,
                              int32_t ones_col, float scale, void* stream) {
  DAE_REQUIRE(src && hi && lo && rows > 0 && cols > 0 && ld_src >= cols && ld_dst >= cols, "dae_split_bf16: bad arguments");
  const int64_t total = (int64_t)rows * ld_dst;
  const int cap = sm_count() * 16;
  const int blocks = (int)((total + 255) / 256 < cap ? (total + 255) / 256 : cap);
  split_bf16_kernel<<<blocks, 256, 0, (cudaStream_t)stream>>>(src, rows, cols, ld_src, (__nv_bfloat16*)hi, (__nv_bfloat16*)lo, ld_dst,
                                                              ones_col, scale);
  DAE_CHECK_LAUNCH("dae_split_bf16");
  return DAE_OK;
}

extern "C" int dae_sym_split_bf16(const float* G, int32_t B, int64_t ldg, float alpha, void* hi, void* lo, int64_t ld, void* stream) {
  DAE_REQUIRE(G && hi && lo && B > 0 && ldg >= B && ld >= B, "dae_sym_split_bf16: bad arguments");
  dim3 grid((unsigned)((ld + 31) / 32), (B + 31) / 32), block(32, 8);
  sym_split_kernel<<<grid, block, 0, (cudaStream_t)stream>>>(G, B, ldg, alpha, (__nv_bfloat16*)hi, (__nv_bfloat16*)lo, ld);
  DAE_CHECK_LAUNCH("dae_sym_split_bf16");
  return DAE_OK;
}

extern "C" int dae_gemm_config(int32_t pair_mode, int32_t lean) {
  dae::g_pair_mode = pair_mode < 0 ? -1 : (pair_mode ? 1 : 0);
  dae::g_lean = lean ? 1 : 0;
  return DAE_OK;
}

extern "C" int dae_gemm_bf16x3(int32_t M, int32_t N, int32_t K, float alpha, const void* a_hi, const void* a_lo, int64_t lda,
                               int32_t a_mn_major, const void* b_hi, const void* b_lo, int64_t ldb, int32_t b_mn_major, float* C,
                               int64_t ldc, int32_t n_store, int32_t special_col, float* special_out, int32_t k_splits,
                               int32_t accumulate, void* stream) {
  DAE_REQUIRE(a_hi && a_lo && b_hi && b_lo && C && M > 0 && N > 0 && K > 0, "dae_gemm_bf16x3: bad arguments");
  DAE_REQUIRE(lda % 8 == 0 && ldb % 8 == 0, "dae_gemm_bf16x3: operand leading dimensions must be multiples of 8 (TMA 16-byte strides)");
  DAE_REQUIRE(((uintptr_t)a_hi | (uintptr_t)a_lo | (uintptr_t)b_hi | (uintptr_t)b_lo) % 16 == 0, "dae_gemm_bf16x3: operands must be 16-byte aligned");
  cudaStream_t st = (cudaStream_t)stream;
  if (n_store <= 0 || n_store > N) n_store = N;
  const int kblocks = (K + BLOCK_K - 1) / BLOCK_K;
  const int tm = (M + 127) / 128, tn128 = (N + 127) / 128, tn64 = (N + 63) / 64;
  const int sms = sm_count();
  int stream_k = 0;
  if (k_splits < 0) {
    const int t = tm * tn128;
    stream_k = (t % sms == 0) ? 0 : 1;
    k_splits = 1;
  }
  if (k_splits < 1) k_splits = 1;
  if (k_splits > kblocks) k_splits = kblocks;
  {
    const int per = (kblocks + k_splits - 1) / k_splits;
    k_splits = (kblocks + per - 1) / per;
  }
  const bool partial = (k_splits > 1) || stream_k;
  if (partial && !accumulate) {
    DAE_CUDA(cudaMemset2DAsync(C, ldc * sizeof(float), 0, (size_t)n_store * sizeof(float), M, st));
    if (special_col >= 0 && special_out) DAE_CUDA(cudaMemsetAsync(special_out, 0, sizeof(float) * M, st));
  }
  GemmParams p{};
  p.M = M; p.N = N; p.K = K; p.k_splits = k_splits; p.stream_k = stream_k; p.atomic = (partial || accumulate) ? 1 : 0; p.alpha = alpha;
  p.C = C; p.ldc = ldc; p.n_store = n_store;
  p.special_col = (special_out ? special_col : -1); p.special_out = special_out;
  Operand A{a_hi, a_lo, lda, a_mn_major}, B{b_hi, b_lo, ldb, b_mn_major};
  int rc;
  const int tiles128 = tm * tn128 * k_splits, tiles64 = tm * tn64 * k_splits;
  const float cost128 = 2.0f * (float)((tiles128 + sms - 1) / sms), cost64 = 1.1f * (float)((tiles64 + sms - 1) / sms);
  if (g_lean) rc = launch_gemm<64, 2, 0>(A, B, p, st);
  else if (use_pair()) rc = launch_gemm<128, 2, 1>(A, B, p, st);
  else if (stream_k) rc = launch_gemm<128, 4, 0, 32>(A, B, p, st);
  else if (!stream_k && cost64 < cost128) rc = launch_gemm<64, 3, 0>(A, B, p, st);
  else rc = launch_gemm<128, 2, 0>(A, B, p, st);
  if (rc) return rc;
  DAE_CHECK_LAUNCH("dae_gemm_bf16x3");
  return DAE_OK;
}

extern "C" int dae_gemm_sym_bf16x3(int32_t M, int32_t N, float alpha, const void* g_hi, const void* g_lo, int64_t ldg, const void* b_hi,
                                   const void* b_lo, int64_t ldb, float* C, int64_t ldc, int32_t accumulate, void* stream) {
  DAE_REQUIRE(g_hi && g_lo && b_hi && b_lo && C && M > 0 && N > 0, "dae_gemm_sym_bf16x3: bad arguments");
  DAE_REQUIRE(ldg % 8 == 0 && ldb % 8 == 0 && ldg >= M && ldb >= N, "dae_gemm_sym_bf16x3: leading dimensions must be multiples of 8 and cover the matrices");
  DAE_REQUIRE(((uintptr_t)g_hi | (uintptr_t)g_lo | (uintptr_t)b_hi | (uintptr_t)b_lo) % 16 == 0, "dae_gemm_sym_bf16x3: operands must be 16-byte aligned");
  GemmParams p{};
  const int kb_half = (M + BLOCK_K - 1) / BLOCK_K;
  p.M = M; p.N = N; p.K = 2 * kb_half * BLOCK_K; p.k_splits = 1; p.stream_k = 1; p.atomic = 1; p.alpha = alpha;
  p.C = C; p.ldc = ldc; p.n_store = N; p.special_col = -1; p.special_out = nullptr; p.a_sym_kb = kb_half;
  if (!accumulate) DAE_CUDA(cudaMemset2DAsync(C, ldc * sizeof(float), 0, (size_t)N * sizeof(float), M, (cudaStream_t)stream));
  Operand A{g_hi, g_lo, ldg, 0}, B{b_hi, b_lo, ldb, 1};
  int rc = launch_gemm_maj<128, 2, 0, 6>(A, B, p, (cudaStream_t)stream);
  if (rc) return rc;
  DAE_CHECK_LAUNCH("dae_gemm_sym_bf16x3");
  return DAE_OK;
}

extern "C" int dae_gemm_det_workspace(int64_t* bytes) {
  DAE_REQUIRE(bytes, "dae_gemm_det_workspace: null pointer");
  *bytes = sk_workspace_bytes();
  return DAE_OK;
}

extern "C" int dae_gemm_bf16x3_det(int32_t M, int32_t N, int32_t K, float alpha, const void* a_hi, const void* a_lo, int64_t lda,
                                   int32_t a_mn_major, const void* b_hi, const void* b_lo, int64_t ldb, int32_t b_mn_major, float* C,
                                   int64_t ldc, int32_t n_store, int32_t special_col, float* special_out, int32_t k_splits,
                                   int32_t accumulate, void* workspace, int64_t workspace_bytes, void* stream) {
  DAE_REQUIRE(a_hi && a_lo && b_hi && b_lo && C && M > 0 && N > 0 && K > 0, "dae_gemm_bf16x3_det: bad arguments");
  DAE_REQUIRE(lda % 8 == 0 && ldb % 8 == 0, "dae_gemm_bf16x3_det: operand leading dimensions must be multiples of 8 (TMA 16-byte strides)");
  DAE_REQUIRE(((uintptr_t)a_hi | (uintptr_t)a_lo | (uintptr_t)b_hi | (uintptr_t)b_lo) % 16 == 0, "dae_gemm_bf16x3_det: operands must be 16-byte aligned");
  DAE_REQUIRE(k_splits == 1 || k_splits == -1, "dae_gemm_bf16x3_det: k_splits must be 1 or -1 (stream-K), got %d", k_splits);
  DAE_REQUIRE(workspace && workspace_bytes >= sk_workspace_bytes(), "dae_gemm_bf16x3_det: workspace of %lld bytes, need %lld",
              (long long)workspace_bytes, (long long)sk_workspace_bytes());
  cudaStream_t st = (cudaStream_t)stream;
  if (n_store <= 0 || n_store > N) n_store = N;
  const int tm = (M + 127) / 128, tn = (N + 127) / 128;
  const int stream_k = (k_splits < 0 && (tm * tn) % sm_count() != 0) ? 1 : 0;
  GemmParams p{};
  p.M = M; p.N = N; p.K = K; p.k_splits = 1; p.stream_k = stream_k; p.atomic = accumulate ? 1 : 0; p.alpha = alpha;
  p.C = C; p.ldc = ldc; p.n_store = n_store;
  p.special_col = (special_out ? special_col : -1); p.special_out = special_out;
  Operand A{a_hi, a_lo, lda, a_mn_major}, B{b_hi, b_lo, ldb, b_mn_major};
  int rc;
  if (stream_k) {
    p.sk_ws = (float*)workspace;
    int n = 0;
    if ((rc = launch_gemm<128, 4, 0, 32>(A, B, p, st, &n))) return rc;
    DAE_REQUIRE(n <= kMaxFixupCtas, "dae_gemm_bf16x3_det: %d stream-K CTAs exceed the fixup's %d", n, kMaxFixupCtas);
    sk_fixup_kernel<128><<<dim3(tm * tn, kFixupSlices), 256, 0, st>>>(p, tm, tm * tn, (K + 31) / 32, n);
  } else {
    const int sms = sm_count(), tn64 = (N + 63) / 64;
    const float cost128 = 2.0f * (float)((tm * tn + sms - 1) / sms), cost64 = 1.1f * (float)((tm * tn64 + sms - 1) / sms);
    rc = (cost64 < cost128) ? launch_gemm<64, 3, 0>(A, B, p, st) : launch_gemm<128, 2, 0>(A, B, p, st);
    if (rc) return rc;
  }
  DAE_CHECK_LAUNCH("dae_gemm_bf16x3_det");
  return DAE_OK;
}

extern "C" int dae_gemm_sym_bf16x3_det(int32_t M, int32_t N, float alpha, const void* g_hi, const void* g_lo, int64_t ldg, const void* b_hi,
                                       const void* b_lo, int64_t ldb, float* C, int64_t ldc, int32_t accumulate, void* workspace,
                                       int64_t workspace_bytes, void* stream) {
  DAE_REQUIRE(g_hi && g_lo && b_hi && b_lo && C && M > 0 && N > 0, "dae_gemm_sym_bf16x3_det: bad arguments");
  DAE_REQUIRE(ldg % 8 == 0 && ldb % 8 == 0 && ldg >= M && ldb >= N, "dae_gemm_sym_bf16x3_det: leading dimensions must be multiples of 8 and cover the matrices");
  DAE_REQUIRE(((uintptr_t)g_hi | (uintptr_t)g_lo | (uintptr_t)b_hi | (uintptr_t)b_lo) % 16 == 0, "dae_gemm_sym_bf16x3_det: operands must be 16-byte aligned");
  DAE_REQUIRE(workspace && workspace_bytes >= sk_workspace_bytes(), "dae_gemm_sym_bf16x3_det: workspace of %lld bytes, need %lld",
              (long long)workspace_bytes, (long long)sk_workspace_bytes());
  cudaStream_t st = (cudaStream_t)stream;
  GemmParams p{};
  const int kb_half = (M + BLOCK_K - 1) / BLOCK_K;
  p.M = M; p.N = N; p.K = 2 * kb_half * BLOCK_K; p.k_splits = 1; p.stream_k = 1; p.atomic = accumulate ? 1 : 0; p.alpha = alpha;
  p.C = C; p.ldc = ldc; p.n_store = N; p.special_col = -1; p.special_out = nullptr; p.a_sym_kb = kb_half;
  p.sk_ws = (float*)workspace;
  Operand A{g_hi, g_lo, ldg, 0}, B{b_hi, b_lo, ldb, 1};
  int n = 0;
  int rc = launch_gemm_maj<128, 2, 0, 6>(A, B, p, st, &n);
  if (rc) return rc;
  DAE_REQUIRE(n <= kMaxFixupCtas, "dae_gemm_sym_bf16x3_det: %d stream-K CTAs exceed the fixup's %d", n, kMaxFixupCtas);
  const int tm = (M + 127) / 128, tn = (N + 127) / 128;
  sk_fixup_kernel<128><<<dim3(tm * tn, kFixupSlices), 256, 0, st>>>(p, tm, tm * tn, 2 * kb_half, n);
  DAE_CHECK_LAUNCH("dae_gemm_sym_bf16x3_det");
  return DAE_OK;
}

extern "C" int dae_decode_prepare(int32_t Brows, int32_t F, const int64_t* indptr, const int32_t* indices, const int32_t* rows,
                                  float* row_loss_part, int32_t* tile_ptr, void* stream) {
  DAE_REQUIRE(Brows > 0 && F > 0 && indptr && indices && row_loss_part && tile_ptr, "dae_decode_prepare: bad arguments");
  cudaStream_t st = (cudaStream_t)stream;
  DAE_CUDA(cudaMemsetAsync(row_loss_part, 0, sizeof(float) * Brows, st));
  const int n_half = 2 * ((F + kDecodeN - 1) / kDecodeN);
  dim3 grid((n_half + 1 + 127) / 128, Brows < 65535 ? Brows : 65535);
  decode_tile_ptr_kernel<<<grid, 128, 0, st>>>(indptr, indices, rows, Brows, n_half, kDecodeN / 2, tile_ptr);
  DAE_CHECK_LAUNCH("dae_decode_prepare");
  return DAE_OK;
}

extern "C" int dae_decode_fused_bf16x3(int32_t Brows, int32_t F, int32_t K, const void* e_hi, const void* e_lo, int64_t lde,
                                       const void* w_hi, const void* w_lo, int64_t ldw, const int64_t* indptr, const int32_t* indices,
                                       const float* values, const int32_t* rows, const float* bv, int32_t dec_act, int32_t loss_func,
                                       const float* weight, const double* stats, void* dz_hi, void* dz_lo, int64_t ld_dz,
                                       float* row_loss_part, int32_t* tile_ptr, int32_t prepared, void* stream) {
  DAE_REQUIRE(e_hi && e_lo && w_hi && w_lo && indptr && indices && values && bv && stats && dz_hi && dz_lo && row_loss_part && tile_ptr,
              "dae_decode_fused_bf16x3: null pointer");
  DAE_REQUIRE(loss_func == DAE_LOSS_CE || loss_func == DAE_LOSS_MSE, "dae_decode_fused_bf16x3: cosine loss uses the unfused path");
  DAE_REQUIRE(lde % 8 == 0 && ldw % 8 == 0 && ld_dz % 32 == 0 && ld_dz >= F, "dae_decode_fused_bf16x3: bad leading dimensions");
  cudaStream_t st = (cudaStream_t)stream;
  GemmParams p{};
  p.M = Brows; p.N = F; p.K = K; p.k_splits = 1; p.alpha = 1.0f; p.special_col = -1;
  p.indptr = indptr; p.indices = indices; p.values = values; p.rows = rows; p.bv = bv; p.weight = weight; p.stats = stats;
  p.dz_hi = (__nv_bfloat16*)dz_hi; p.dz_lo = (__nv_bfloat16*)dz_lo; p.ld_dz = ld_dz; p.row_loss_part = row_loss_part;
  p.tile_ptr = tile_ptr;
  if (!prepared) {
    int rc0 = dae_decode_prepare(Brows, F, indptr, indices, rows, row_loss_part, tile_ptr, stream);
    if (rc0) return rc0;
  }
  Operand A{e_hi, e_lo, lde, 0}, B{w_hi, w_lo, ldw, 0};
  int rc = 0;
#define DAE_DEC(ACT, LOSS) rc = launch_decode<ACT, LOSS>(A, B, p, st)
  if (loss_func == DAE_LOSS_CE) {
    if (dec_act == DAE_ACT_SIGMOID) DAE_DEC(DAE_ACT_SIGMOID, DAE_LOSS_CE);
    else if (dec_act == DAE_ACT_TANH) DAE_DEC(DAE_ACT_TANH, DAE_LOSS_CE);
    else DAE_DEC(DAE_ACT_NONE, DAE_LOSS_CE);
  } else {
    if (dec_act == DAE_ACT_SIGMOID) DAE_DEC(DAE_ACT_SIGMOID, DAE_LOSS_MSE);
    else if (dec_act == DAE_ACT_TANH) DAE_DEC(DAE_ACT_TANH, DAE_LOSS_MSE);
    else DAE_DEC(DAE_ACT_NONE, DAE_LOSS_MSE);
  }
#undef DAE_DEC
  if (rc) return rc;
  DAE_CHECK_LAUNCH("dae_decode_fused_bf16x3");
  return DAE_OK;
}

extern "C" int dae_decode_loss_parts(int32_t F, int32_t* n_parts) {
  DAE_REQUIRE(F > 0 && n_parts, "dae_decode_loss_parts: bad arguments");
  *n_parts = 2 * ((F + kDecodeN - 1) / kDecodeN);
  return DAE_OK;
}

extern "C" int dae_decode_fused_bf16x3_det(int32_t Brows, int32_t F, int32_t K, const void* e_hi, const void* e_lo, int64_t lde,
                                           const void* w_hi, const void* w_lo, int64_t ldw, const int64_t* indptr, const int32_t* indices,
                                           const float* values, const int32_t* rows, const float* bv, int32_t dec_act, int32_t loss_func,
                                           const float* weight, const double* stats, void* dz_hi, void* dz_lo, int64_t ld_dz,
                                           float* row_loss_parts, int32_t* tile_ptr, int32_t prepared, void* stream) {
  DAE_REQUIRE(e_hi && e_lo && w_hi && w_lo && indptr && indices && values && bv && stats && dz_hi && dz_lo && row_loss_parts && tile_ptr,
              "dae_decode_fused_bf16x3_det: null pointer");
  DAE_REQUIRE(loss_func == DAE_LOSS_CE || loss_func == DAE_LOSS_MSE, "dae_decode_fused_bf16x3_det: cosine loss uses the unfused path");
  DAE_REQUIRE(lde % 8 == 0 && ldw % 8 == 0 && ld_dz % 32 == 0 && ld_dz >= F, "dae_decode_fused_bf16x3_det: bad leading dimensions");
  cudaStream_t st = (cudaStream_t)stream;
  GemmParams p{};
  p.M = Brows; p.N = F; p.K = K; p.k_splits = 1; p.alpha = 1.0f; p.special_col = -1;
  p.indptr = indptr; p.indices = indices; p.values = values; p.rows = rows; p.bv = bv; p.weight = weight; p.stats = stats;
  p.dz_hi = (__nv_bfloat16*)dz_hi; p.dz_lo = (__nv_bfloat16*)dz_lo; p.ld_dz = ld_dz; p.row_loss_part = row_loss_parts;
  p.tile_ptr = tile_ptr; p.loss_parts = 1;
  if (!prepared) {
    int rc0 = dae_decode_prepare(Brows, F, indptr, indices, rows, row_loss_parts, tile_ptr, stream);
    if (rc0) return rc0;
  }
  Operand A{e_hi, e_lo, lde, 0}, B{w_hi, w_lo, ldw, 0};
  int rc = 0;
#define DAE_DEC(ACT, LOSS) rc = launch_decode<ACT, LOSS>(A, B, p, st)
  if (loss_func == DAE_LOSS_CE) {
    if (dec_act == DAE_ACT_SIGMOID) DAE_DEC(DAE_ACT_SIGMOID, DAE_LOSS_CE);
    else if (dec_act == DAE_ACT_TANH) DAE_DEC(DAE_ACT_TANH, DAE_LOSS_CE);
    else DAE_DEC(DAE_ACT_NONE, DAE_LOSS_CE);
  } else {
    if (dec_act == DAE_ACT_SIGMOID) DAE_DEC(DAE_ACT_SIGMOID, DAE_LOSS_MSE);
    else if (dec_act == DAE_ACT_TANH) DAE_DEC(DAE_ACT_TANH, DAE_LOSS_MSE);
    else DAE_DEC(DAE_ACT_NONE, DAE_LOSS_MSE);
  }
#undef DAE_DEC
  if (rc) return rc;
  DAE_CHECK_LAUNCH("dae_decode_fused_bf16x3_det");
  return DAE_OK;
}

extern "C" int dae_similarity_topk_workspace(int32_t n_query, int32_t n_corpus, int32_t k, int32_t splits, int64_t* bytes) {
  DAE_REQUIRE(bytes && n_query > 0 && n_corpus > 0, "dae_similarity_topk_workspace: bad arguments");
  DAE_REQUIRE(k >= 1 && k <= kTopkMaxK, "dae_similarity_topk_workspace: k = %d is outside the supported range 1 <= k <= %d", k, kTopkMaxK);
  *bytes = topk_workspace_bytes(n_query, k, topk_splits(n_query, n_corpus, splits));
  return DAE_OK;
}

extern "C" int dae_similarity_topk_bf16x3(int32_t n_query, int32_t n_corpus, int32_t dim, const void* q_hi, const void* q_lo, int64_t ldq,
                                          const void* c_hi, const void* c_lo, int64_t ldc, int32_t k, int64_t diag_offset, int32_t exclude,
                                          int32_t splits, void* workspace, int64_t workspace_bytes, int32_t* idx_out, float* val_out,
                                          void* stream) {
  DAE_REQUIRE(q_hi && q_lo && c_hi && c_lo && workspace && idx_out && val_out, "dae_similarity_topk_bf16x3: null pointer");
  DAE_REQUIRE(n_query > 0 && n_corpus > 0 && dim > 0, "dae_similarity_topk_bf16x3: bad sizes");
  DAE_REQUIRE(k >= 1 && k <= kTopkMaxK, "dae_similarity_topk_bf16x3: k = %d is outside the supported range 1 <= k <= %d", k, kTopkMaxK);
  DAE_REQUIRE(ldq >= dim && ldc >= dim && ldq % 8 == 0 && ldc % 8 == 0,
              "dae_similarity_topk_bf16x3: leading dimensions must cover dim and be multiples of 8 (TMA 16-byte strides)");
  DAE_REQUIRE(((uintptr_t)q_hi | (uintptr_t)q_lo | (uintptr_t)c_hi | (uintptr_t)c_lo | (uintptr_t)workspace) % 16 == 0,
              "dae_similarity_topk_bf16x3: operands and workspace must be 16-byte aligned");
  const int s = topk_splits(n_query, n_corpus, splits);
  const int64_t need = topk_workspace_bytes(n_query, k, s);
  DAE_REQUIRE(workspace_bytes >= need, "dae_similarity_topk_bf16x3: workspace of %lld bytes, %lld needed (dae_similarity_topk_workspace)",
              (long long)workspace_bytes, (long long)need);
  cudaStream_t st = (cudaStream_t)stream;
  TopkParams tp{};
  tp.g.M = n_query; tp.g.N = n_corpus; tp.g.K = dim; tp.g.k_splits = 1; tp.g.alpha = 1.0f; tp.g.special_col = -1;
  tp.k = k; tp.splits = s; tp.exclude = exclude ? 1 : 0; tp.diag_offset = diag_offset;
  tp.ws_val = reinterpret_cast<float*>(workspace);
  tp.ws_idx = reinterpret_cast<int32_t*>(reinterpret_cast<float*>(workspace) + (int64_t)n_query * 2 * s * k);
  Operand A{q_hi, q_lo, ldq, 0}, B{c_hi, c_lo, ldc, 0};
  int rc = (k <= 16) ? launch_topk<16, false>(A, B, tp, st) : launch_topk<32, false>(A, B, tp, st);
  if (rc) return rc;
  DAE_CHECK_LAUNCH("dae_similarity_topk_bf16x3");
  topk_merge_kernel<<<(n_query + 7) / 8, 256, 0, st>>>(tp.ws_val, tp.ws_idx, n_query, 2 * s, k, idx_out, val_out);
  DAE_CHECK_LAUNCH("dae_similarity_topk_bf16x3 (merge)");
  return DAE_OK;
}

extern "C" int dae_similarity_topk_excl_bf16x3(int32_t n_query, int32_t n_corpus, int32_t dim, const void* q_hi, const void* q_lo,
                                               int64_t ldq, const void* c_hi, const void* c_lo, int64_t ldc, int32_t k,
                                               int64_t diag_offset, int32_t exclude, int32_t splits, void* workspace,
                                               int64_t workspace_bytes, int32_t* idx_out, float* val_out, const int64_t* ex_indptr,
                                               const int32_t* ex_indices, int64_t ex_nnz, void* stream) {
  DAE_REQUIRE(q_hi && q_lo && c_hi && c_lo && workspace && idx_out && val_out && ex_indptr && (ex_nnz == 0 || ex_indices),
              "dae_similarity_topk_excl_bf16x3: null pointer");
  DAE_REQUIRE(n_query > 0 && n_corpus > 0 && dim > 0 && ex_nnz >= 0, "dae_similarity_topk_excl_bf16x3: bad sizes");
  DAE_REQUIRE(k >= 1 && k <= kTopkMaxK, "dae_similarity_topk_excl_bf16x3: k = %d is outside the supported range 1 <= k <= %d", k,
              kTopkMaxK);
  DAE_REQUIRE(ldq >= dim && ldc >= dim && ldq % 8 == 0 && ldc % 8 == 0,
              "dae_similarity_topk_excl_bf16x3: leading dimensions must cover dim and be multiples of 8 (TMA 16-byte strides)");
  DAE_REQUIRE(((uintptr_t)q_hi | (uintptr_t)q_lo | (uintptr_t)c_hi | (uintptr_t)c_lo | (uintptr_t)workspace) % 16 == 0 &&
                  (uintptr_t)ex_indptr % 8 == 0 && (uintptr_t)ex_indices % 4 == 0,
              "dae_similarity_topk_excl_bf16x3: operands and workspace must be 16-byte, ex_indptr 8-byte, ex_indices 4-byte aligned");
  const int s = topk_splits(n_query, n_corpus, splits);
  const int64_t need = topk_workspace_bytes(n_query, k, s);
  DAE_REQUIRE(workspace_bytes >= need,
              "dae_similarity_topk_excl_bf16x3: workspace of %lld bytes, %lld needed (dae_similarity_topk_workspace)",
              (long long)workspace_bytes, (long long)need);
  cudaStream_t st = (cudaStream_t)stream;
  TopkParams tp{};
  tp.g.M = n_query; tp.g.N = n_corpus; tp.g.K = dim; tp.g.k_splits = 1; tp.g.alpha = 1.0f; tp.g.special_col = -1;
  tp.k = k; tp.splits = s; tp.exclude = exclude ? 1 : 0; tp.diag_offset = diag_offset;
  tp.ws_val = reinterpret_cast<float*>(workspace);
  tp.ws_idx = reinterpret_cast<int32_t*>(reinterpret_cast<float*>(workspace) + (int64_t)n_query * 2 * s * k);
  tp.ex_indptr = ex_indptr; tp.ex_indices = ex_indices;
  Operand A{q_hi, q_lo, ldq, 0}, B{c_hi, c_lo, ldc, 0};
  int rc = (k <= 16) ? launch_topk<16, true>(A, B, tp, st) : launch_topk<32, true>(A, B, tp, st);
  if (rc) return rc;
  DAE_CHECK_LAUNCH("dae_similarity_topk_excl_bf16x3");
  topk_merge_kernel<<<(n_query + 7) / 8, 256, 0, st>>>(tp.ws_val, tp.ws_idx, n_query, 2 * s, k, idx_out, val_out);
  DAE_CHECK_LAUNCH("dae_similarity_topk_excl_bf16x3 (merge)");
  return DAE_OK;
}

extern "C" int dae_similarity_topk_groups_bf16x3(int32_t n_query, int32_t n_corpus, int32_t dim, const void* q_hi, const void* q_lo,
                                                 int64_t ldq, const void* c_hi, const void* c_lo, int64_t ldc, int32_t k,
                                                 int64_t diag_offset, int32_t exclude, int32_t splits, void* workspace,
                                                 int64_t workspace_bytes, int32_t* idx_out, float* val_out, const int64_t* ex_indptr,
                                                 const int32_t* ex_indices, int64_t ex_nnz, const int32_t* groups, void* stream) {
  DAE_REQUIRE(q_hi && q_lo && c_hi && c_lo && workspace && idx_out && val_out && groups && (ex_nnz == 0 || (ex_indptr && ex_indices)),
              "dae_similarity_topk_groups_bf16x3: null pointer");
  DAE_REQUIRE(n_query > 0 && n_corpus > 0 && dim > 0 && ex_nnz >= 0, "dae_similarity_topk_groups_bf16x3: bad sizes");
  DAE_REQUIRE(k >= 1 && k <= kTopkMaxK, "dae_similarity_topk_groups_bf16x3: k = %d is outside the supported range 1 <= k <= %d", k,
              kTopkMaxK);
  DAE_REQUIRE(ldq >= dim && ldc >= dim && ldq % 8 == 0 && ldc % 8 == 0,
              "dae_similarity_topk_groups_bf16x3: leading dimensions must cover dim and be multiples of 8 (TMA 16-byte strides)");
  DAE_REQUIRE(((uintptr_t)q_hi | (uintptr_t)q_lo | (uintptr_t)c_hi | (uintptr_t)c_lo | (uintptr_t)workspace) % 16 == 0 &&
                  (uintptr_t)ex_indptr % 8 == 0 && ((uintptr_t)ex_indices | (uintptr_t)groups) % 4 == 0,
              "dae_similarity_topk_groups_bf16x3: operands and workspace must be 16-byte, ex_indptr 8-byte, ex_indices and groups "
              "4-byte aligned");
  const int s = topk_splits(n_query, n_corpus, splits);
  const int64_t need = topk_workspace_bytes(n_query, k, s);
  DAE_REQUIRE(workspace_bytes >= need,
              "dae_similarity_topk_groups_bf16x3: workspace of %lld bytes, %lld needed (dae_similarity_topk_workspace)",
              (long long)workspace_bytes, (long long)need);
  cudaStream_t st = (cudaStream_t)stream;
  TopkParams tp{};
  tp.g.M = n_query; tp.g.N = n_corpus; tp.g.K = dim; tp.g.k_splits = 1; tp.g.alpha = 1.0f; tp.g.special_col = -1;
  tp.k = k; tp.splits = s; tp.exclude = exclude ? 1 : 0; tp.diag_offset = diag_offset;
  tp.ws_val = reinterpret_cast<float*>(workspace);
  tp.ws_idx = reinterpret_cast<int32_t*>(reinterpret_cast<float*>(workspace) + (int64_t)n_query * 2 * s * k);
  tp.ex_indptr = ex_indptr; tp.ex_indices = ex_indices; tp.groups = groups;
  Operand A{q_hi, q_lo, ldq, 0}, B{c_hi, c_lo, ldc, 0};
  int rc = (k <= 16) ? launch_topk<16, true, true>(A, B, tp, st) : launch_topk<32, true, true>(A, B, tp, st);
  if (rc) return rc;
  DAE_CHECK_LAUNCH("dae_similarity_topk_groups_bf16x3");
  topk_merge_groups_kernel<<<(n_query + 7) / 8, 256, 0, st>>>(tp.ws_val, tp.ws_idx, groups, n_query, 2 * s, k, idx_out, val_out);
  DAE_CHECK_LAUNCH("dae_similarity_topk_groups_bf16x3 (merge)");
  return DAE_OK;
}

extern "C" int dae_similarity_pair_hist_bf16x3(int32_t n, int32_t dim, const void* x_hi, const void* x_lo, int64_t ldx,
                                               const int32_t* labels, float range, int32_t bins, uint64_t* hist, double* sums,
                                               void* stream) {
  DAE_REQUIRE(x_hi && x_lo && labels && hist && sums, "dae_similarity_pair_hist_bf16x3: null pointer");
  DAE_REQUIRE(n >= 2 && dim > 0, "dae_similarity_pair_hist_bf16x3: bad sizes (n = %d >= 2 rows and dim = %d > 0 needed)", n, dim);
  DAE_REQUIRE(hist_bins_ok(bins), "dae_similarity_pair_hist_bf16x3: bins = %d is not a power of two in [2^%d, 2^%d]", bins,
              kHistMinLog2Bins, kHistMaxLog2Bins);
  DAE_REQUIRE(hist_range_ok(range), "dae_similarity_pair_hist_bf16x3: range M = %g is not a power of two in [2^-64, 2^64]", (double)range);
  DAE_REQUIRE(ldx >= dim && ldx % 8 == 0,
              "dae_similarity_pair_hist_bf16x3: the leading dimension must cover dim and be a multiple of 8 (TMA 16-byte strides)");
  DAE_REQUIRE(((uintptr_t)x_hi | (uintptr_t)x_lo) % 16 == 0 && ((uintptr_t)hist | (uintptr_t)sums) % 8 == 0 && (uintptr_t)labels % 4 == 0,
              "dae_similarity_pair_hist_bf16x3: operands must be 16-byte, hist and sums 8-byte, labels 4-byte aligned");
  PairHistParams hp{};
  hp.g.M = n; hp.g.N = n; hp.g.K = dim; hp.g.k_splits = 1; hp.g.alpha = 1.0f; hp.g.special_col = -1;
  hp.labels = labels; hp.range = range; hp.scale = (float)bins / (2.0f * range); hp.bins = (uint32_t)bins;
  hp.hist = reinterpret_cast<unsigned long long*>(hist); hp.sums = sums;
  Operand X{x_hi, x_lo, ldx, 0};
  int rc = launch_pair_hist(X, hp, (cudaStream_t)stream);
  if (rc) return rc;
  DAE_CHECK_LAUNCH("dae_similarity_pair_hist_bf16x3");
  return DAE_OK;
}

extern "C" int dae_similarity_pairs_bf16x3(int32_t n_query, int32_t n_corpus, int32_t dim, const void* q_hi, const void* q_lo, int64_t ldq,
                                           const void* c_hi, const void* c_lo, int64_t ldc, int32_t self, float threshold, uint64_t* count,
                                           int64_t capacity, int32_t* i_out, int32_t* j_out, float* s_out, void* stream) {
  DAE_REQUIRE(q_hi && q_lo && c_hi && c_lo && count, "dae_similarity_pairs_bf16x3: null pointer");
  DAE_REQUIRE(capacity >= 0, "dae_similarity_pairs_bf16x3: capacity = %lld < 0", (long long)capacity);
  DAE_REQUIRE(capacity == 0 || (i_out && j_out && s_out), "dae_similarity_pairs_bf16x3: null output with capacity %lld > 0",
              (long long)capacity);
  DAE_REQUIRE(n_query > 0 && n_corpus > 0 && dim > 0, "dae_similarity_pairs_bf16x3: bad sizes");
  DAE_REQUIRE(!self || (n_query == n_corpus && q_hi == c_hi && q_lo == c_lo && ldq == ldc),
              "dae_similarity_pairs_bf16x3: self mode needs the corpus operands to be the query operands");
  DAE_REQUIRE(pair_threshold_ok(threshold), "dae_similarity_pairs_bf16x3: threshold %g is not finite", (double)threshold);
  DAE_REQUIRE(ldq >= dim && ldc >= dim && ldq % 8 == 0 && ldc % 8 == 0,
              "dae_similarity_pairs_bf16x3: leading dimensions must cover dim and be multiples of 8 (TMA 16-byte strides)");
  DAE_REQUIRE(((uintptr_t)q_hi | (uintptr_t)q_lo | (uintptr_t)c_hi | (uintptr_t)c_lo) % 16 == 0 && (uintptr_t)count % 8 == 0 &&
                  ((uintptr_t)i_out | (uintptr_t)j_out | (uintptr_t)s_out) % 4 == 0,
              "dae_similarity_pairs_bf16x3: operands must be 16-byte, the counter 8-byte and the outputs 4-byte aligned");
  PairsParams pp{};
  pp.g.M = n_query; pp.g.N = n_corpus; pp.g.K = dim; pp.g.k_splits = 1; pp.g.alpha = 1.0f; pp.g.special_col = -1;
  pp.self = self ? 1 : 0; pp.tau = threshold;
  pp.count = reinterpret_cast<unsigned long long*>(count); pp.capacity = (unsigned long long)capacity;
  pp.i_out = i_out; pp.j_out = j_out; pp.s_out = s_out;
  Operand A{q_hi, q_lo, ldq, 0}, B{c_hi, c_lo, ldc, 0};
  int rc = launch_pairs(A, B, pp, (cudaStream_t)stream);
  if (rc) return rc;
  DAE_CHECK_LAUNCH("dae_similarity_pairs_bf16x3");
  return DAE_OK;
}
```

### dae_rnn_news_recommendation_b200/csrc/triplet.cu

```cuda
#include <cuda_bf16.h>
#include "common.cuh"

namespace dae {

constexpr int kTY = 8, kTX = 32, kTJ = 4, kTK = 4;
constexpr int kJTile = kTY * kTJ;
constexpr int kKTile = kTX * kTK;
constexpr int kTripThreads = kTY * kTX;

__device__ __forceinline__ float fast_rcp(float x) { float r; asm("rcp.approx.ftz.f32 %0, %1;" : "=f"(r) : "f"(x)); return r; }
__device__ __forceinline__ float fast_lg2(float x) { float r; asm("lg2.approx.ftz.f32 %0, %1;" : "=f"(r) : "f"(x)); return r; }
__device__ __forceinline__ float fast_ex2(float x) { float r; asm("ex2.approx.ftz.f32 %0, %1;" : "=f"(r) : "f"(x)); return r; }
constexpr float kLog2e = 1.4426950408889634f;
constexpr float kLn2 = 0.6931471805599453f;

typedef float2 f2;
__device__ __forceinline__ f2 pk(float lo, float hi) { return make_float2(lo, hi); }
__device__ __forceinline__ void upk(f2 v, float& lo, float& hi) { lo = v.x; hi = v.y; }
__device__ __forceinline__ f2 mul2(f2 a, f2 b) { return make_float2(__fmul_rn(a.x, b.x), __fmul_rn(a.y, b.y)); }
__device__ __forceinline__ f2 add2(f2 a, f2 b) { return make_float2(__fadd_rn(a.x, b.x), __fadd_rn(a.y, b.y)); }
__device__ __forceinline__ f2 fma2(f2 a, f2 b, f2 c) { return make_float2(__fmaf_rn(a.x, b.x, c.x), __fmaf_rn(a.y, b.y, c.y)); }

__device__ __forceinline__ void triplet_pair_tile(f2 U, const f2 (&V)[kTK], f2& rs, f2 (&cs)[kTK], float& lg) {
  const f2 one = pk(1.0f, 1.0f);
  f2 e[kTK], t[kTK];
#pragma unroll
  for (int b = 0; b < kTK; ++b) { e[b] = mul2(U, V[b]); t[b] = fma2(U, V[b], one); }
  const f2 p01 = mul2(t[0], t[1]), p23 = mul2(t[2], t[3]), P = mul2(p01, p23);
  float Px, Py;
  upk(P, Px, Py);
  lg += fast_lg2(Px) + fast_lg2(Py);
  const f2 r = pk(fast_rcp(Px), fast_rcp(Py));
  const f2 r01 = mul2(r, p23), r23 = mul2(r, p01);
  const f2 s0 = mul2(e[0], mul2(r01, t[1])), s1 = mul2(e[1], mul2(r01, t[0]));
  const f2 s2 = mul2(e[2], mul2(r23, t[3])), s3 = mul2(e[3], mul2(r23, t[2]));
  rs = add2(rs, add2(add2(s0, s1), add2(s2, s3)));
  cs[0] = add2(cs[0], s0); cs[1] = add2(cs[1], s1); cs[2] = add2(cs[2], s2); cs[3] = add2(cs[3], s3);
}

constexpr float kSeriesMax = 0x1p-12f;
__device__ __forceinline__ float ln_1p_small(float e) { return fmaf(-0.5f * e, e, e); }

template <int TIER>
__device__ __forceinline__ void triplet_tile(const float (&s_j)[kTJ], const float (&u_j)[kTJ], const float (&s_k)[kTK],
                                             const float (&v_k)[kTK], float (&sg)[kTJ][kTK], float& lg) {
#pragma unroll
  for (int a = 0; a < kTJ; ++a) {
    if (TIER == 0) {
      const float e0 = u_j[a] * v_k[0], e1 = u_j[a] * v_k[1], e2 = u_j[a] * v_k[2], e3 = u_j[a] * v_k[3];
      const float t0 = e0 + 1.0f, t1 = e1 + 1.0f, t2 = e2 + 1.0f, t3 = e3 + 1.0f;
      const float p01 = t0 * t1, p23 = t2 * t3, P = p01 * p23;
      lg += fast_lg2(P);
      const float r = fast_rcp(P);
      const float r01 = r * p23, r23 = r * p01;
      sg[a][0] = e0 * (r01 * t1); sg[a][1] = e1 * (r01 * t0); sg[a][2] = e2 * (r23 * t3); sg[a][3] = e3 * (r23 * t2);
    } else if (TIER == 1) {
#pragma unroll
      for (int b = 0; b < kTK; ++b) {
        const float e = u_j[a] * v_k[b];
        const float t = e + 1.0f;
        if (e < kSeriesMax) lg = fmaf(ln_1p_small(e), kLog2e, lg); else lg += fast_lg2(t);
        sg[a][b] = e * fast_rcp(t);
      }
    } else if (TIER == 3) {
#pragma unroll
      for (int b = 0; b < kTK; ++b) {
        const bool pos = (s_j[a] < 1.0e38f) && (s_k[b] > s_j[a]);
        const float x = s_k[b] - s_j[a];
        const float em = fast_ex2(-fabsf(x) * kLog2e);
        lg += pos ? (fmaxf(x, 0.0f) * kLog2e + fast_lg2(1.0f + em)) : 0.0f;
        sg[a][b] = pos ? 1.0f : 0.0f;
      }
    } else {
#pragma unroll
      for (int b = 0; b < kTK; ++b) {
        const bool valid = (s_j[a] < 1.0e38f) && (s_k[b] > -1.0e38f);
        const float x = s_k[b] - s_j[a];
        const float em = fast_ex2(-fabsf(x) * kLog2e);
        const float t = 1.0f + em;
        const float r = fast_rcp(t);
        const float l1p = (em < kSeriesMax) ? ln_1p_small(em) * kLog2e : fast_lg2(t);
        lg += valid ? (fmaxf(x, 0.0f) * kLog2e + l1p) : 0.0f;
        sg[a][b] = valid ? (x >= 0.0f ? r : em * r) : 0.0f;
      }
    }
  }
}

__device__ __forceinline__ int f32_ordered(float f) { const int b = __float_as_int(f); return b < 0 ? -(b & 0x7fffffff) : b; }
__device__ __forceinline__ float f32_from_ordered(int o) { return __int_as_float(o < 0 ? ((-o) | (int)0x80000000) : o); }
__device__ __noinline__ float pos_threshold_small(float a) {
  int lo = f32_ordered(a), hi = f32_ordered(__fadd_rn(a, 1e-15f));
  while (hi - lo > 1) {
    const int mid = lo + ((hi - lo) >> 1);
    if (__fsub_rn(f32_from_ordered(mid), a) <= 1e-16f) lo = mid; else hi = mid;
  }
  return f32_from_ordered(lo);
}
__device__ __forceinline__ float pos_threshold(float a) { return fabsf(a) >= 0x1p-29f ? a : pos_threshold_small(a); }

template <int TIER>
__device__ __forceinline__ void triplet_sweep(const float* sj, const float* uj, float* gj, const float* sk, const float* vk, float* gk,
                                              int Pj, int Pk, int Pk_max, int tx, int ty, float& lacc, int& npos) {
  for (int jt = 0; jt < Pj; jt += kJTile) {
    float s_j[kTJ], u_j[kTJ], rs[kTJ];
#pragma unroll
    for (int a = 0; a < kTJ; ++a) { s_j[a] = sj[jt + ty * kTJ + a]; u_j[a] = uj[jt + ty * kTJ + a]; rs[a] = 0.0f; }
    if (TIER == 0) {
      const f2 U01 = pk(u_j[0], u_j[1]), U23 = pk(u_j[2], u_j[3]);
      f2 rs01 = pk(0.0f, 0.0f), rs23 = pk(0.0f, 0.0f);
      for (int kt = 0; kt < Pk; kt += kKTile) {
        const int q0 = kt + tx * kTK;
        const float4 s4 = *reinterpret_cast<const float4*>(sk + q0);
        const float4 v4 = *reinterpret_cast<const float4*>(vk + q0);
        const float s_k[kTK] = {s4.x, s4.y, s4.z, s4.w};
        const f2 V[kTK] = {pk(v4.x, v4.x), pk(v4.y, v4.y), pk(v4.z, v4.z), pk(v4.w, v4.w)};
        f2 cs[kTK] = {pk(0.0f, 0.0f), pk(0.0f, 0.0f), pk(0.0f, 0.0f), pk(0.0f, 0.0f)};
        triplet_pair_tile(U01, V, rs01, cs, lacc);
        triplet_pair_tile(U23, V, rs23, cs, lacc);
#pragma unroll
        for (int a = 0; a < kTJ; ++a) {
#pragma unroll
          for (int b = 0; b < kTK; ++b)
            asm("{ .reg .pred p; setp.gt.f32 p, %1, %2; @p add.s32 %0, %0, 1; }" : "+r"(npos) : "f"(s_k[b]), "f"(s_j[a]));
        }
        float4* g = reinterpret_cast<float4*>(gk + ty * Pk_max + q0);
        float4 o = *g;
        float lo, hi;
        upk(cs[0], lo, hi); o.x += lo + hi;
        upk(cs[1], lo, hi); o.y += lo + hi;
        upk(cs[2], lo, hi); o.z += lo + hi;
        upk(cs[3], lo, hi); o.w += lo + hi;
        *g = o;
      }
      upk(rs01, rs[0], rs[1]);
      upk(rs23, rs[2], rs[3]);
    } else
    for (int kt = 0; kt < Pk; kt += kKTile) {
      const int q0 = kt + tx * kTK;
      const float4 s4 = *reinterpret_cast<const float4*>(sk + q0);
      const float4 v4 = *reinterpret_cast<const float4*>(vk + q0);
      const float s_k[kTK] = {s4.x, s4.y, s4.z, s4.w};
      const float v_k[kTK] = {v4.x, v4.y, v4.z, v4.w};
      float sg[kTJ][kTK];
      triplet_tile<TIER>(s_j, u_j, s_k, v_k, sg, lacc);
      float cs[kTK] = {0.0f, 0.0f, 0.0f, 0.0f};
#pragma unroll
      for (int a = 0; a < kTJ; ++a) {
#pragma unroll
        for (int b = 0; b < kTK; ++b) {
          asm("{ .reg .pred p; setp.gt.f32 p, %1, %2; @p add.s32 %0, %0, 1; }" : "+r"(npos) : "f"(s_k[b]), "f"(s_j[a]));
          rs[a] += sg[a][b];
          cs[b] += sg[a][b];
        }
      }
      float4* g = reinterpret_cast<float4*>(gk + ty * Pk_max + q0);
      float4 o = *g;
      o.x += cs[0]; o.y += cs[1]; o.z += cs[2]; o.w += cs[3];
      *g = o;
    }
#pragma unroll
    for (int a = 0; a < kTJ; ++a) {
      const float t = warp_sum(rs[a]);
      if (tx == 0) gj[jt + ty * kTJ + a] = t;
    }
  }
}

__global__ void __launch_bounds__(kTripThreads) triplet_batch_all_kernel(const float* __restrict__ S, int64_t lds, int B,
                                                                         const int32_t* __restrict__ seg_lo,
                                                                         const int32_t* __restrict__ seg_hi, float* __restrict__ G,
                                                                         int64_t ldg, double* __restrict__ stats, int Pj_max, int Pk_max,
                                                                         int pos_only, __nv_bfloat16* __restrict__ g_hi,
                                                                         __nv_bfloat16* __restrict__ g_lo, int64_t ld_split,
                                                                         double* __restrict__ loss_slots) {
  extern __shared__ __align__(16) float smem[];
  __shared__ float red_f[32];
  __shared__ double red_d[32];
  const int i = blockIdx.x;
  const int tid = threadIdx.x, tx = tid & 31, ty = tid >> 5;
  const int lo = seg_lo[i], hi = seg_hi[i];
  const int nj = hi - lo;
  const int nk = B - nj;
  const float* srow = S + (int64_t)i * lds;
  float* grow = G + (int64_t)i * ldg;

  if (nj <= 1 || nk == 0) {
    if (loss_slots && tid == 0) loss_slots[i] = 0.0;
    for (int c = tid; c < B; c += kTripThreads) {
      grow[c] = 0.0f;
      if (g_hi) { g_hi[(int64_t)i * ld_split + c] = __float2bfloat16_rn(0.0f); g_lo[(int64_t)i * ld_split + c] = __float2bfloat16_rn(0.0f); }
    }
    return;
  }
  float mx = -3.0e38f, mn = 3.0e38f;
  for (int c = tid; c < B; c += kTripThreads) { const float s = srow[c]; mx = fmaxf(mx, s); mn = fminf(mn, s); }
#pragma unroll
  for (int o = 16; o > 0; o >>= 1) { mx = fmaxf(mx, __shfl_xor_sync(0xffffffffu, mx, o)); mn = fminf(mn, __shfl_xor_sync(0xffffffffu, mn, o)); }
  if (tx == 0) { red_f[ty] = mx; red_f[8 + ty] = mn; }
  __syncthreads();
  mx = red_f[0]; mn = red_f[8];
#pragma unroll
  for (int w = 1; w < kTY; ++w) { mx = fmaxf(mx, red_f[w]); mn = fminf(mn, red_f[8 + w]); }
  const float range = mx - mn;
  const int tier = pos_only ? 3 : ((range < 10.0f) ? 0 : ((range < 80.0f) ? 1 : 2));
  const float mid = 0.5f * (mx + mn);

  const int Pj = (nj + kJTile - 1) / kJTile * kJTile;
  const int Pk = (nk + kKTile - 1) / kKTile * kKTile;
  float* sj = smem;
  float* uj = sj + Pj_max;
  float* gj = uj + Pj_max;
  float* sk = gj + Pj_max;
  float* vk = sk + Pk_max;
  float* gk = vk + Pk_max;

  for (int p = tid; p < Pj; p += kTripThreads) {
    const int c = lo + p;
    const bool ok = (p < nj) && (c != i);
    const float s = ok ? srow[c] : 3.0e38f;
    sj[p] = ok ? pos_threshold(s) : s;
    uj[p] = ok ? fast_ex2((mid - s) * kLog2e) : 0.0f;
    gj[p] = 0.0f;
  }
  for (int q = tid; q < Pk; q += kTripThreads) {
    const int c = (q < lo) ? q : q + nj;
    const bool ok = q < nk;
    const float s = ok ? srow[c] : -3.0e38f;
    sk[q] = s;
    vk[q] = ok ? fast_ex2((s - mid) * kLog2e) : 0.0f;
  }
  for (int e = tid; e < kTY * Pk; e += kTripThreads) gk[(e / Pk) * Pk_max + (e % Pk)] = 0.0f;
  __syncthreads();

  float lacc = 0.0f;
  int npos = 0;
  if (tier == 0) triplet_sweep<0>(sj, uj, gj, sk, vk, gk, Pj, Pk, Pk_max, tx, ty, lacc, npos);
  else if (tier == 1) triplet_sweep<1>(sj, uj, gj, sk, vk, gk, Pj, Pk, Pk_max, tx, ty, lacc, npos);
  else if (tier == 2) triplet_sweep<2>(sj, uj, gj, sk, vk, gk, Pj, Pk, Pk_max, tx, ty, lacc, npos);
  else triplet_sweep<3>(sj, uj, gj, sk, vk, gk, Pj, Pk, Pk_max, tx, ty, lacc, npos);
  __syncthreads();
  const float inv = pos_only ? 1.0f : (float)(1.0 / (stats[DAE_STAT_N_VALID] + 1e-16));
  for (int c = tid; c < B; c += kTripThreads) {
    float g;
    if (c >= lo && c < hi) {
      g = -gj[c - lo] * inv;
    } else {
      const int q = (c < lo) ? c : c - nj;
      float t = 0.0f;
#pragma unroll
      for (int w = 0; w < kTY; ++w) t += gk[w * Pk_max + q];
      g = t * inv;
    }
    grow[c] = g;
    if (g_hi) {
      const __nv_bfloat16 h = __float2bfloat16_rn(g);
      g_hi[(int64_t)i * ld_split + c] = h;
      g_lo[(int64_t)i * ld_split + c] = __float2bfloat16_rn(g - __bfloat162float(h));
    }
  }
  const double lsum = block_sum((double)lacc * (double)kLn2, red_d);
  const double psum = block_sum((double)npos, red_d);
  if (tid == 0) {
    if (loss_slots) loss_slots[blockIdx.x] = lsum; else atomicAdd(stats + DAE_STAT_TRIPLET_SUM, lsum);
    atomicAdd(stats + DAE_STAT_NUM, psum);
  }
}

constexpr int kChunkJ = 512;
constexpr int kChunkK = 1024;
static_assert(kChunkJ % kJTile == 0 && kChunkK % kKTile == 0, "chunks must hold whole register tiles");

__global__ void __launch_bounds__(kTripThreads) triplet_batch_all_tiled_kernel(const float* __restrict__ S, int64_t lds, int row0, int B,
                                                                               const int32_t* __restrict__ seg_lo,
                                                                               const int32_t* __restrict__ seg_hi, float* G, int64_t ldg,
                                                                               double* __restrict__ stats, int pos_only,
                                                                               __nv_bfloat16* __restrict__ g_hi,
                                                                               __nv_bfloat16* __restrict__ g_lo, int64_t ld_split,
                                                                               double* __restrict__ loss_slots) {
  __shared__ __align__(16) float sj[kChunkJ];
  __shared__ __align__(16) float uj[kChunkJ];
  __shared__ __align__(16) float gj[kChunkJ];
  __shared__ __align__(16) float sk[kChunkK];
  __shared__ __align__(16) float vk[kChunkK];
  __shared__ __align__(16) float gk[kTY * kChunkK];
  __shared__ float red_f[32];
  __shared__ double red_d[32];
  const int r = blockIdx.x, i = row0 + r;
  const int tid = threadIdx.x, tx = tid & 31, ty = tid >> 5;
  const int lo = seg_lo[i], hi = seg_hi[i];
  const int nj = hi - lo;
  const int nk = B - nj;
  const float* srow = S + (int64_t)r * lds;
  float* grow = G + (int64_t)r * ldg;

  if (nj <= 1 || nk == 0) {
    if (loss_slots && tid == 0) loss_slots[i] = 0.0;
    for (int c = tid; c < B; c += kTripThreads) {
      grow[c] = 0.0f;
      if (g_hi) { g_hi[(int64_t)r * ld_split + c] = __float2bfloat16_rn(0.0f); g_lo[(int64_t)r * ld_split + c] = __float2bfloat16_rn(0.0f); }
    }
    return;
  }
  float mx = -3.0e38f, mn = 3.0e38f;
  for (int c = tid; c < B; c += kTripThreads) { const float s = srow[c]; mx = fmaxf(mx, s); mn = fminf(mn, s); }
#pragma unroll
  for (int o = 16; o > 0; o >>= 1) { mx = fmaxf(mx, __shfl_xor_sync(0xffffffffu, mx, o)); mn = fminf(mn, __shfl_xor_sync(0xffffffffu, mn, o)); }
  if (tx == 0) { red_f[ty] = mx; red_f[8 + ty] = mn; }
  __syncthreads();
  mx = red_f[0]; mn = red_f[8];
#pragma unroll
  for (int w = 1; w < kTY; ++w) { mx = fmaxf(mx, red_f[w]); mn = fminf(mn, red_f[8 + w]); }
  const float range = mx - mn;
  const int tier = pos_only ? 3 : ((range < 10.0f) ? 0 : ((range < 80.0f) ? 1 : 2));
  const float mid = 0.5f * (mx + mn);
  const float inv = pos_only ? 1.0f : (float)(1.0 / (stats[DAE_STAT_N_VALID] + 1e-16));

  double lsum = 0.0;
  int npos = 0;
  for (int k0 = 0; k0 < nk; k0 += kChunkK) {
    const int ck = min(kChunkK, nk - k0);
    const int Pk = (ck + kKTile - 1) / kKTile * kKTile;
    __syncthreads();
    for (int q = tid; q < Pk; q += kTripThreads) {
      const int qq = k0 + q;
      const int c = (qq < lo) ? qq : qq + nj;
      const bool ok = q < ck;
      const float s = ok ? srow[c] : -3.0e38f;
      sk[q] = s;
      vk[q] = ok ? fast_ex2((s - mid) * kLog2e) : 0.0f;
    }
    for (int e = tid; e < kTY * Pk; e += kTripThreads) gk[(e / Pk) * kChunkK + (e % Pk)] = 0.0f;
    for (int j0 = 0; j0 < nj; j0 += kChunkJ) {
      const int cj = min(kChunkJ, nj - j0);
      const int Pj = (cj + kJTile - 1) / kJTile * kJTile;
      __syncthreads();
      for (int p = tid; p < Pj; p += kTripThreads) {
        const int c = lo + j0 + p;
        const bool ok = (p < cj) && (c != i);
        const float s = ok ? srow[c] : 3.0e38f;
        sj[p] = ok ? pos_threshold(s) : s;
        uj[p] = ok ? fast_ex2((mid - s) * kLog2e) : 0.0f;
        gj[p] = 0.0f;
      }
      __syncthreads();
      float lacc = 0.0f;
      if (tier == 0) triplet_sweep<0>(sj, uj, gj, sk, vk, gk, Pj, Pk, kChunkK, tx, ty, lacc, npos);
      else if (tier == 1) triplet_sweep<1>(sj, uj, gj, sk, vk, gk, Pj, Pk, kChunkK, tx, ty, lacc, npos);
      else if (tier == 2) triplet_sweep<2>(sj, uj, gj, sk, vk, gk, Pj, Pk, kChunkK, tx, ty, lacc, npos);
      else triplet_sweep<3>(sj, uj, gj, sk, vk, gk, Pj, Pk, kChunkK, tx, ty, lacc, npos);
      lsum += (double)lacc;
      __syncthreads();
      for (int p = tid; p < cj; p += kTripThreads) {
        float* g = grow + lo + j0 + p;
        *g = (k0 == 0 ? 0.0f : *g) + gj[p];
      }
    }
    __syncthreads();
    for (int q = tid; q < ck; q += kTripThreads) {
      const int qq = k0 + q;
      const int c = (qq < lo) ? qq : qq + nj;
      float t = 0.0f;
#pragma unroll
      for (int w = 0; w < kTY; ++w) t += gk[w * kChunkK + q];
      const float g = t * inv;
      grow[c] = g;
      if (g_hi) {
        const __nv_bfloat16 h = __float2bfloat16_rn(g);
        g_hi[(int64_t)r * ld_split + c] = h;
        g_lo[(int64_t)r * ld_split + c] = __float2bfloat16_rn(g - __bfloat162float(h));
      }
    }
  }
  for (int p = tid; p < nj; p += kTripThreads) {
    const int c = lo + p;
    const float g = -grow[c] * inv;
    grow[c] = g;
    if (g_hi) {
      const __nv_bfloat16 h = __float2bfloat16_rn(g);
      g_hi[(int64_t)r * ld_split + c] = h;
      g_lo[(int64_t)r * ld_split + c] = __float2bfloat16_rn(g - __bfloat162float(h));
    }
  }
  const double ls = block_sum(lsum * (double)kLn2, red_d);
  const double ps = block_sum((double)npos, red_d);
  if (tid == 0) {
    if (loss_slots) loss_slots[row0 + (int64_t)blockIdx.x] = ls; else atomicAdd(stats + DAE_STAT_TRIPLET_SUM, ls);
    atomicAdd(stats + DAE_STAT_NUM, ps);
  }
}

constexpr int kHardThreads = 256;

__device__ __forceinline__ float block_max(float v, float* red) {
#pragma unroll
  for (int o = 16; o > 0; o >>= 1) v = fmaxf(v, __shfl_xor_sync(0xffffffffu, v, o));
  __syncthreads();
  if ((threadIdx.x & 31) == 0) red[threadIdx.x >> 5] = v;
  __syncthreads();
  float r = red[0];
  for (int w = 1; w < (int)(blockDim.x >> 5); ++w) r = fmaxf(r, red[w]);
  __syncthreads();
  return r;
}

__global__ void __launch_bounds__(kHardThreads) triplet_batch_hard_kernel(const float* __restrict__ S, int64_t lds, int row0, int B,
                                                                          const float* __restrict__ labels, float* __restrict__ G,
                                                                          int64_t ldg, float* __restrict__ weight,
                                                                          double* __restrict__ stats, double* __restrict__ loss_slots) {
  __shared__ float red[32];
  __shared__ float redi[32];
  const int a = row0 + (int)blockIdx.x, tid = threadIdx.x;
  const float* srow = S + (int64_t)blockIdx.x * lds;
  float* grow = G + (int64_t)blockIdx.x * ldg;
  const float la = labels[a];
  float m = -3.0e38f, hn = -3.0e38f;
  for (int c = tid; c < B; c += kHardThreads) {
    const float s = srow[c];
    m = fmaxf(m, s);
    const float an = (labels[c] != la) ? 1.0f : 0.0f;
    hn = fmaxf(hn, an * s);
  }
  m = block_max(m, red);
  hn = block_max(hn, red);
  float hpn = -3.0e38f;
  for (int c = tid; c < B; c += kHardThreads) {
    const float ap = (c != a && labels[c] == la) ? 1.0f : 0.0f;
    hpn = fmaxf(hpn, -(srow[c] + m * (1.0f - ap)));
  }
  const float hp = -block_max(hpn, red);
  const float td = fmaxf(hn - hp, 0.0f);
  const bool active = td > 0.0f;
  float tp = 0.0f, tn = 0.0f, tm = 0.0f, tp_masked = 0.0f;
  for (int c = tid; c < B; c += kHardThreads) {
    const float s = srow[c];
    const float ap = (c != a && labels[c] == la) ? 1.0f : 0.0f;
    const float an = (labels[c] != la) ? 1.0f : 0.0f;
    if (s + m * (1.0f - ap) == hp) { tp += 1.0f; if (ap == 0.0f) tp_masked += 1.0f; }
    if (an * s == hn) tn += 1.0f;
    if (s == m) tm += 1.0f;
  }
  tp = block_sum(tp, red);
  tn = block_sum(tn, redi);
  tm = block_sum(tm, red);
  tp_masked = block_sum(tp_masked, redi);
  const float q = active ? 1.0f / (1.0f + expf(-td)) : 0.0f;
  const float dm = -q * tp_masked / tp;
  for (int c = tid; c < B; c += kHardThreads) {
    const float s = srow[c];
    const float ap = (c != a && labels[c] == la) ? 1.0f : 0.0f;
    const float an = (labels[c] != la) ? 1.0f : 0.0f;
    float g = 0.0f;
    if (active) {
      if (s + m * (1.0f - ap) == hp) g -= q / tp;
      if (an * s == hn) g += an * q / tn;
      if (s == m) g += dm / tm;
      float w = 0.0f;
      if (s == hp) w += 1.0f;
      if (s == hn) w += 1.0f;
      if (c == a) w += 1.0f;
      if (w != 0.0f) atomicAdd(weight + c, w);
    }
    grow[c] = g;
  }
  if (tid == 0 && loss_slots) loss_slots[a] = active ? (double)(fmaxf(td, 0.0f) + log1pf(expf(-td))) : 0.0;
  if (tid == 0 && active) {
    if (!loss_slots) atomicAdd(stats + DAE_STAT_TRIPLET_SUM, (double)(fmaxf(td, 0.0f) + log1pf(expf(-td))));
    atomicAdd(stats + DAE_STAT_N_ACTIVE, 1.0);
  }
}

__global__ void triplet_hard_scale_kernel(float* __restrict__ G, int64_t ldg, int B, const float* __restrict__ weight,
                                          double* __restrict__ stats) {
  const float inv = (float)(1.0 / (stats[DAE_STAT_N_ACTIVE] + 1e-16));
  const int c = blockIdx.x * blockDim.x + threadIdx.x;
  const int r = blockIdx.y;
  if (c < B) G[(int64_t)r * ldg + c] *= inv;
  if (r == 0 && blockIdx.x == 0) {
    __shared__ double red[32];
    double s = 0.0;
    for (int i = threadIdx.x; i < B; i += blockDim.x) s += (double)weight[i];
    s = block_sum(s, red);
    if (threadIdx.x == 0) stats[DAE_STAT_SUM_W] = s;
  }
}

__global__ void triplet_hard_finish_kernel(const float* __restrict__ weight, int B, double* __restrict__ stats, float* __restrict__ dE2,
                                           int H, int64_t ld) {
  if (blockIdx.x == 0) {
    __shared__ double red[32];
    double s = 0.0;
    for (int i = threadIdx.x; i < B; i += blockDim.x) s += (double)weight[i];
    s = block_sum(s, red);
    if (threadIdx.x == 0) stats[DAE_STAT_SUM_W] = s;
  }
  if (!dE2) return;
  const float inv = (float)(1.0 / (stats[DAE_STAT_N_ACTIVE] + 1e-16));
  const int64_t total = (int64_t)B * H;
  for (int64_t e = (int64_t)blockIdx.x * blockDim.x + threadIdx.x; e < total; e += (int64_t)gridDim.x * blockDim.x) {
    const int64_t r = e / H;
    dE2[r * ld + (e - r * H)] *= inv;
  }
}

__global__ void triplet_explicit_kernel(const float* __restrict__ E, const float* __restrict__ Ep, const float* __restrict__ En,
                                        int B, int H, int64_t ld, float alpha, float* __restrict__ dE, float* __restrict__ dEp,
                                        float* __restrict__ dEn, double* __restrict__ stats, double* __restrict__ loss_slots) {
  const int lane = threadIdx.x & 31;
  const int r = blockIdx.x * (blockDim.x >> 5) + (threadIdx.x >> 5);
  if (r >= B) return;
  const float* e = E + (int64_t)r * ld;
  const float* ep = Ep + (int64_t)r * ld;
  const float* en = En + (int64_t)r * ld;
  float dp = 0.0f;
  for (int h = lane; h < H; h += 32) dp += e[h] * ep[h] - e[h] * en[h];
  dp = warp_sum(dp);
  const float x = -dp;
  const float sp = fmaxf(x, 0.0f) + log1pf(expf(-fabsf(x)));
  const float sg = 1.0f / (1.0f + expf(-x));
  const float c = alpha * sg / (float)B;
  for (int h = lane; h < H; h += 32) {
    const float ev = e[h];
    dE[(int64_t)r * ld + h] += c * (en[h] - ep[h]);
    dEp[(int64_t)r * ld + h] += -c * ev;
    dEn[(int64_t)r * ld + h] += c * ev;
  }
  if (lane == 0) { if (loss_slots) loss_slots[r] = (double)sp; else atomicAdd(stats + DAE_STAT_TRIPLET_SUM, (double)sp); }
  if (r == 0 && lane == 0) stats[DAE_STAT_N_ACTIVE] = (double)B;
}

constexpr int kSmemSweepMaxB = 4096;
static int g_force_tiled = 0;

}

extern "C" int dae_triplet_config(int32_t force_tiled) {
  dae::g_force_tiled = force_tiled ? 1 : 0;
  return DAE_OK;
}

static int dae_triplet_batch_all_impl(const float* S, int64_t lds, int32_t B, const int32_t* seg_lo, const int32_t* seg_hi, float* G,
                                     int64_t ldg, double* stats, int32_t pos_only, void* g_hi, void* g_lo, int64_t ld_split, void* stream, double* loss_slots) {
  using namespace dae;
  DAE_REQUIRE(S && seg_lo && seg_hi && G && stats && B >= 1 && lds >= B && ldg >= B, "dae_triplet_batch_all: bad arguments");
  DAE_REQUIRE(B <= DAE_MAX_TRIPLET_BATCH, "dae_triplet_batch_all: B <= %d rows, the cap of the B x B mining buffers (got %d)",
              DAE_MAX_TRIPLET_BATCH, B);
  DAE_REQUIRE(!g_hi || (g_lo && ld_split >= B), "dae_triplet_batch_all: bad split outputs");
  cudaStream_t st = (cudaStream_t)stream;
  if (B > kSmemSweepMaxB || g_force_tiled) {
    triplet_batch_all_tiled_kernel<<<B, kTripThreads, 0, st>>>(S, lds, 0, B, seg_lo, seg_hi, G, ldg, stats, pos_only, (__nv_bfloat16*)g_hi,
                                                               (__nv_bfloat16*)g_lo, ld_split, loss_slots);
    DAE_CHECK_LAUNCH("dae_triplet_batch_all(tiled)");
    return DAE_OK;
  }
  const int Pj = (B + kJTile - 1) / kJTile * kJTile;
  const int Pk = (B + kKTile - 1) / kKTile * kKTile;
  const size_t smem = sizeof(float) * ((size_t)3 * Pj + (size_t)2 * Pk + (size_t)kTY * Pk);
  DAE_REQUIRE(smem + 1024 <= 227 * 1024, "dae_triplet_batch_all: B=%d needs %zu B of shared memory", B, smem);
  {
    static size_t attr_smem[64] = {0};
    int dev = 0;
    DAE_CUDA(cudaGetDevice(&dev));
    if (dev < 0 || dev >= 64 || smem > attr_smem[dev]) {
      DAE_CUDA(cudaFuncSetAttribute(triplet_batch_all_kernel, cudaFuncAttributeMaxDynamicSharedMemorySize, (int)smem));
      if (dev >= 0 && dev < 64) attr_smem[dev] = smem;
    }
  }
  triplet_batch_all_kernel<<<B, kTripThreads, smem, st>>>(S, lds, B, seg_lo, seg_hi, G, ldg, stats, Pj, Pk, pos_only, (__nv_bfloat16*)g_hi,
                                                          (__nv_bfloat16*)g_lo, ld_split, loss_slots);
  DAE_CHECK_LAUNCH("dae_triplet_batch_all");
  return DAE_OK;
}

static int dae_triplet_batch_hard_impl(const float* S, int64_t lds, int32_t B, const float* labels, float* G, int64_t ldg,
                                      float* weight, double* stats, void* stream, double* loss_slots) {
  using namespace dae;
  DAE_REQUIRE(S && labels && G && weight && stats && B >= 1 && lds >= B && ldg >= B, "dae_triplet_batch_hard: bad arguments");
  cudaStream_t st = (cudaStream_t)stream;
  DAE_CUDA(cudaMemsetAsync(weight, 0, sizeof(float) * B, st));
  triplet_batch_hard_kernel<<<B, kHardThreads, 0, st>>>(S, lds, 0, B, labels, G, ldg, weight, stats, loss_slots);
  dim3 grid((B + 255) / 256, B);
  triplet_hard_scale_kernel<<<grid, 256, 0, st>>>(G, ldg, B, weight, stats);
  DAE_CHECK_LAUNCH("dae_triplet_batch_hard");
  return DAE_OK;
}

static int dae_triplet_batch_all_rows_impl(const float* S_blk, int64_t lds, int32_t row0, int32_t n_rows, int32_t B, const int32_t* seg_lo,
                                          const int32_t* seg_hi, float* G_blk, int64_t ldg, double* stats, int32_t pos_only, void* g_hi,
                                          void* g_lo, int64_t ld_split, void* stream, double* loss_slots) {
  using namespace dae;
  DAE_REQUIRE(S_blk && seg_lo && seg_hi && G_blk && stats && B >= 1 && lds >= B && ldg >= B,
              "dae_triplet_batch_all_rows: bad arguments");
  DAE_REQUIRE(B <= DAE_MAX_BLOCKED_BATCH, "dae_triplet_batch_all_rows: B <= %d rows (got %d)", DAE_MAX_BLOCKED_BATCH, B);
  DAE_REQUIRE(row0 >= 0 && n_rows >= 1 && (int64_t)row0 + n_rows <= B,
              "dae_triplet_batch_all_rows: anchor rows [%d, %lld) outside the batch of %d", row0, (long long)row0 + n_rows, B);
  DAE_REQUIRE(!g_hi || (g_lo && ld_split >= B), "dae_triplet_batch_all_rows: bad split outputs");
  triplet_batch_all_tiled_kernel<<<n_rows, kTripThreads, 0, (cudaStream_t)stream>>>(S_blk, lds, row0, B, seg_lo, seg_hi, G_blk, ldg, stats,
                                                                                    pos_only, (__nv_bfloat16*)g_hi, (__nv_bfloat16*)g_lo,
                                                                                    ld_split, loss_slots);
  DAE_CHECK_LAUNCH("dae_triplet_batch_all_rows");
  return DAE_OK;
}

static int dae_triplet_batch_hard_rows_impl(const float* S_blk, int64_t lds, int32_t row0, int32_t n_rows, int32_t B, const float* labels,
                                           float* G_blk, int64_t ldg, float* weight, double* stats, void* stream, double* loss_slots) {
  using namespace dae;
  DAE_REQUIRE(S_blk && labels && G_blk && weight && stats && B >= 1 && lds >= B && ldg >= B, "dae_triplet_batch_hard_rows: bad arguments");
  DAE_REQUIRE(B <= DAE_MAX_BLOCKED_BATCH, "dae_triplet_batch_hard_rows: B <= %d rows (got %d)", DAE_MAX_BLOCKED_BATCH, B);
  DAE_REQUIRE(row0 >= 0 && n_rows >= 1 && (int64_t)row0 + n_rows <= B,
              "dae_triplet_batch_hard_rows: anchor rows [%d, %lld) outside the batch of %d", row0, (long long)row0 + n_rows, B);
  triplet_batch_hard_kernel<<<n_rows, kHardThreads, 0, (cudaStream_t)stream>>>(S_blk, lds, row0, B, labels, G_blk, ldg, weight, stats, loss_slots);
  DAE_CHECK_LAUNCH("dae_triplet_batch_hard_rows");
  return DAE_OK;
}

extern "C" int dae_triplet_batch_hard_finish(const float* weight, int32_t B, double* stats, float* dE2, int32_t H, int64_t ld, void* stream) {
  using namespace dae;
  DAE_REQUIRE(weight && stats && B >= 1 && B <= DAE_MAX_BLOCKED_BATCH, "dae_triplet_batch_hard_finish: bad arguments");
  DAE_REQUIRE(!dE2 || (H >= 1 && ld >= H), "dae_triplet_batch_hard_finish: bad dE2 shape");
  int blocks = 1;
  if (dE2) {
    const int64_t want = ((int64_t)B * H + 255) / 256;
    blocks = (int)(want < 4096 ? want : 4096);
  }
  triplet_hard_finish_kernel<<<blocks, 256, 0, (cudaStream_t)stream>>>(weight, B, stats, dE2, H, ld);
  DAE_CHECK_LAUNCH("dae_triplet_batch_hard_finish");
  return DAE_OK;
}

static int dae_triplet_explicit_impl(const float* E, const float* Ep, const float* En, int32_t B, int32_t H, int64_t ld, float alpha,
                                    float* dE, float* dEp, float* dEn, double* stats, void* stream, double* loss_slots) {
  using namespace dae;
  DAE_REQUIRE(E && Ep && En && dE && dEp && dEn && stats && B >= 1 && H >= 1 && ld >= H, "dae_triplet_explicit: bad arguments");
  triplet_explicit_kernel<<<(B + 7) / 8, 256, 0, (cudaStream_t)stream>>>(E, Ep, En, B, H, ld, alpha, dE, dEp, dEn, stats, loss_slots);
  DAE_CHECK_LAUNCH("dae_triplet_explicit");
  return DAE_OK;
}

extern "C" int dae_triplet_batch_all(const float* S, int64_t lds, int32_t B, const int32_t* seg_lo, const int32_t* seg_hi, float* G,
                                     int64_t ldg, double* stats, int32_t pos_only, void* g_hi, void* g_lo, int64_t ld_split, void* stream) {
  return dae_triplet_batch_all_impl(S, lds, B, seg_lo, seg_hi, G, ldg, stats, pos_only, g_hi, g_lo, ld_split, stream, nullptr);
}
extern "C" int dae_triplet_batch_all_det(const float* S, int64_t lds, int32_t B, const int32_t* seg_lo, const int32_t* seg_hi, float* G,
                                     int64_t ldg, double* stats, int32_t pos_only, void* g_hi, void* g_lo, int64_t ld_split, double* loss_slots, void* stream) {
  DAE_REQUIRE(loss_slots, "dae_triplet_batch_all_det: null loss_slots");
  return dae_triplet_batch_all_impl(S, lds, B, seg_lo, seg_hi, G, ldg, stats, pos_only, g_hi, g_lo, ld_split, stream, loss_slots);
}

extern "C" int dae_triplet_batch_hard(const float* S, int64_t lds, int32_t B, const float* labels, float* G, int64_t ldg,
                                      float* weight, double* stats, void* stream) {
  return dae_triplet_batch_hard_impl(S, lds, B, labels, G, ldg, weight, stats, stream, nullptr);
}
extern "C" int dae_triplet_batch_hard_det(const float* S, int64_t lds, int32_t B, const float* labels, float* G, int64_t ldg,
// ... 55 lines not shown
```

### include/dae_sm100.h

```cpp
#ifndef DAE_SM100_H
#define DAE_SM100_H

#include <stddef.h>
#include <stdint.h>

#ifdef __cplusplus
extern "C" {
#endif

#define DAE_OK 0
#define DAE_ERR_BAD_ARG (-1)
#define DAE_ERR_CUDA (-2)
#define DAE_ERR_UNSUPPORTED (-3)

#define DAE_ACT_NONE 0
#define DAE_ACT_SIGMOID 1
#define DAE_ACT_TANH 2

#define DAE_LOSS_CE 0
#define DAE_LOSS_MSE 1
#define DAE_LOSS_COSINE 2

#define DAE_TRIPLET_NONE 0
#define DAE_TRIPLET_BATCH_ALL 1
#define DAE_TRIPLET_BATCH_HARD 2
#define DAE_MAX_TRIPLET_BATCH 32768
#define DAE_MAX_BLOCKED_BATCH 262144

#define DAE_OPT_SGD 0
#define DAE_OPT_ADAGRAD 1
#define DAE_OPT_MOMENTUM 2
#define DAE_OPT_ADAM 3

#define DAE_STAT_COST 0
#define DAE_STAT_AE_LOSS 1
#define DAE_STAT_TRIPLET_LOSS 2
#define DAE_STAT_FRACTION 3
#define DAE_STAT_NUM 4
#define DAE_STAT_SUM_W 5
#define DAE_STAT_N_VALID 6
#define DAE_STAT_SUM_LW 7
#define DAE_STAT_TRIPLET_SUM 8
#define DAE_STAT_N_ACTIVE 9
#define DAE_STAT_SLOTS 16

int dae_version(void);
int dae_last_error(char* buf, size_t len);

int dae_step_advance(int64_t* ctl, int64_t row_stride, void* stream);
int dae_batch_prepare(const int32_t* perm, int64_t offset, const int64_t* ctl, int32_t B, const float* labels_all,
                      int32_t strategy, int32_t* rows_out, float* labels_out, int32_t* seg_lo,
                      int32_t* seg_hi, float* weight_out, double* stats, void* stream);
int dae_batch_prepare_next(const int32_t* perm, int64_t n_perm, int64_t stride, const int64_t* ctl, int32_t B,
                           const float* labels_all, int32_t strategy, int32_t* rows_s, float* labels_s,
                           int32_t* seg_lo_s, int32_t* seg_hi_s, float* weight_s, double* stats_s, void* stream);
int dae_batch_prepare_blocked(const int32_t* perm, int64_t offset, const int64_t* ctl, int32_t B, const float* labels_all,
                              int32_t strategy, int32_t* rows_out, float* labels_out, int32_t* seg_lo,
                              int32_t* seg_hi, float* weight_out, double* stats, void* stream);
int dae_batch_prepare_next_blocked(const int32_t* perm, int64_t n_perm, int64_t stride, const int64_t* ctl, int32_t B,
                                   const float* labels_all, int32_t strategy, int32_t* rows_s, float* labels_s,
                                   int32_t* seg_lo_s, int32_t* seg_hi_s, float* weight_s, double* stats_s, void* stream);
int dae_batch_commit(int32_t B, const int32_t* rows_s, const float* labels_s, const int32_t* seg_lo_s,
                     const int32_t* seg_hi_s, const float* weight_s, const double* stats_s, int32_t* rows,
                     float* labels_b, int32_t* seg_lo, int32_t* seg_hi, float* weight, double* stats, void* stream);
int dae_batch_prepare_explicit(const int32_t* perm, int64_t offset, const int64_t* ctl, int32_t B, int64_t n_each,
                               int32_t* rows_out, double* stats, void* stream);

int dae_encode_csr_fwd(const int64_t* indptr, const int32_t* indices, const float* values,
                       const int32_t* rows, int32_t n_rows, int32_t F, int32_t H, float in_scale,
                       const float* W, const float* bh, int32_t enc_act, float* E, int64_t ldE,
                       int32_t* col_count, void* e_hi, void* e_lo, int64_t ld_split, void* stream);

int dae_encode_csr_bwd(const int64_t* indptr, const int32_t* indices, const float* values,
                       const int32_t* rows, int32_t n_rows, int32_t F, int32_t H, float in_scale,
                       const float* E, const float* bh, int32_t enc_act, float* dE, const float* dE_add,
                       int64_t ldE, float* dW, float* dbh, int32_t dbh_zeroed, void* stream);

int dae_col_scan(const int32_t* col_count, int32_t F, int32_t* col_start, int32_t* col_cursor, void* stream);
int dae_encode_csr_bwd_gather(const int64_t* indptr, const int32_t* indices, const float* values,
                              const int32_t* rows, int32_t n_rows, int32_t F, int32_t H, float in_scale,
                              const float* E, const float* bh, int32_t enc_act, float* dE, const float* dE_add,
                              int64_t ldE, float* dW, float* dbh, int32_t dbh_zeroed, const int32_t* col_count,
                              int32_t* col_start, int32_t* col_cursor, int32_t* ent_col, int32_t* ent_row,
                              float* ent_val, void* stream);

int dae_encode_csr_fwd_hot(const int64_t* indptr, const int32_t* indices, const float* values, int32_t n_rows,
                           int32_t F, int32_t H, float in_scale, const float* W, const float* bh, int32_t enc_act,
                           float* E, int64_t ldE, const int32_t* hot_cols, const int32_t* hot_slot, int32_t K,
                           int32_t groups, void* stream);

int dae_sgemm(int32_t M, int32_t N, int32_t K, float alpha, const float* A, int64_t sam, int64_t sak,
              const float* B, int64_t sbn, int64_t sbk, float beta, float* C, int64_t ldc, void* stream);

int dae_split_bf16(const float* src, int32_t rows, int32_t cols, int64_t ld_src, void* hi, void* lo,
                   int64_t ld_dst, int32_t ones_col, float scale, void* stream);
int dae_sym_split_bf16(const float* G, int32_t B, int64_t ldg, float alpha, void* hi, void* lo, int64_t ld,
                       void* stream);
int dae_gemm_bf16x3(int32_t M, int32_t N, int32_t K, float alpha, const void* a_hi, const void* a_lo,
                    int64_t lda, int32_t a_mn_major, const void* b_hi, const void* b_lo, int64_t ldb,
                    int32_t b_mn_major, float* C, int64_t ldc, int32_t n_store, int32_t special_col,
                    float* special_out, int32_t k_splits, int32_t accumulate, void* stream);
int dae_gemm_sym_bf16x3(int32_t M, int32_t N, float alpha, const void* g_hi, const void* g_lo, int64_t ldg,
                        const void* b_hi, const void* b_lo, int64_t ldb, float* C, int64_t ldc, int32_t accumulate,
                        void* stream);
int dae_gemm_config(int32_t pair_mode, int32_t lean);
int dae_decode_prepare(int32_t Brows, int32_t F, const int64_t* indptr, const int32_t* indices, const int32_t* rows,
                       float* row_loss_part, int32_t* tile_ptr, void* stream);
int dae_decode_fused_bf16x3(int32_t Brows, int32_t F, int32_t K, const void* e_hi, const void* e_lo,
                            int64_t lde, const void* w_hi, const void* w_lo, int64_t ldw,
                            const int64_t* indptr, const int32_t* indices, const float* values,
                            const int32_t* rows, const float* bv, int32_t dec_act, int32_t loss_func,
                            const float* weight, const double* stats, void* dz_hi, void* dz_lo,
                            int64_t ld_dz, float* row_loss_part, int32_t* tile_ptr, int32_t prepared, void* stream);
int dae_reduce_parts(const float* parts, int32_t n_parts, int32_t n, float* out, void* stream);

int dae_decode_loss_bwd(const int64_t* indptr, const int32_t* indices, const float* values,
                        const int32_t* rows, int32_t n_rows, int32_t F, const float* bv, int32_t dec_act,
                        int32_t loss_func, const float* weight, const double* stats, float* Z, int64_t ldz,
                        float* row_loss, void* stream);

int dae_colsum(const float* M, int32_t n_rows, int32_t n_cols, int64_t ld, float* out, void* stream);

int dae_triplet_batch_all(const float* S, int64_t lds, int32_t B, const int32_t* seg_lo, const int32_t* seg_hi,
                          float* G, int64_t ldg, double* stats, int32_t pos_only, void* g_hi, void* g_lo,
                          int64_t ld_split, void* stream);
int dae_triplet_config(int32_t force_tiled);
int dae_triplet_batch_hard(const float* S, int64_t lds, int32_t B, const float* labels, float* G, int64_t ldg,
                           float* weight, double* stats, void* stream);
int dae_triplet_batch_all_rows(const float* S_blk, int64_t lds, int32_t row0, int32_t n_rows, int32_t B, const int32_t* seg_lo,
                               const int32_t* seg_hi, float* G_blk, int64_t ldg, double* stats, int32_t pos_only, void* g_hi,
                               void* g_lo, int64_t ld_split, void* stream);
int dae_triplet_batch_hard_rows(const float* S_blk, int64_t lds, int32_t row0, int32_t n_rows, int32_t B, const float* labels,
                                float* G_blk, int64_t ldg, float* weight, double* stats, void* stream);
int dae_triplet_batch_hard_finish(const float* weight, int32_t B, double* stats, float* dE2, int32_t H, int64_t ld, void* stream);
int dae_triplet_explicit(const float* E, const float* Ep, const float* En, int32_t B, int32_t H, int64_t ld,
                         float alpha, float* dE, float* dEp, float* dEn, double* stats, void* stream);

int dae_step_finalize(const float* row_loss, const float* parts, int32_t n_parts, const float* weight, int32_t B,
                      int32_t strategy, float alpha, double* stats, double* stats_log, const int64_t* ctl, void* stream);

int dae_optimizer_step(float* theta, const float* grad, float* slot1, float* slot2, int64_t n, int32_t opt,
                       float lr, float momentum, float grad_scale, int32_t step, const int64_t* ctl, void* w_hi,
                       void* w_lo, int32_t F, int32_t H, int64_t ld_split, void* stream);

int dae_mask_values(const float* values, const uint8_t* keep, int64_t nnz, float corr_frac, uint64_t seed,
                    uint64_t epoch, float* values_out, void* stream);

int dae_salt_pepper_csr(const int64_t* indptr, const int32_t* indices, const float* values, int64_t row0, int64_t n, int32_t F,
                        int64_t v, float lo, float hi, const uint32_t* draws, uint64_t seed, uint64_t epoch, int64_t* indptr_out,
                        int32_t* indices_out, float* values_out, int64_t cap, int32_t* overflow, void* ws, size_t ws_bytes,
                        void* stream);
int dae_salt_pepper_workspace(int64_t n, size_t* bytes);

int dae_rownorm_split_bf16(const float* X, int32_t rows, int32_t cols, int64_t ld, int32_t norm_kind, void* hi, void* lo,
                           int64_t ld_dst, float* x_out, int64_t ld_out, void* stream);
int dae_row_argmax(float* S, int32_t rows, int32_t cols, int64_t ld, int64_t diag_offset, int32_t zero_diag,
                   int32_t* idx_out, float* val_out, void* stream);

int dae_similarity_topk_bf16x3(int32_t n_query, int32_t n_corpus, int32_t dim, const void* q_hi, const void* q_lo,
                               int64_t ldq, const void* c_hi, const void* c_lo, int64_t ldc, int32_t k,
                               int64_t diag_offset, int32_t exclude, int32_t splits, void* workspace,
                               int64_t workspace_bytes, int32_t* idx_out, float* val_out, void* stream);
int dae_similarity_topk_workspace(int32_t n_query, int32_t n_corpus, int32_t k, int32_t splits, int64_t* bytes);

int dae_csr_similarity_topk(const int64_t* q_indptr, const int32_t* q_indices, const float* q_values, int32_t n_query,
                            int64_t q_nnz, int32_t q_features, const int64_t* c_indptr, const int32_t* c_indices,
                            const float* c_values, int32_t n_corpus, int64_t c_nnz, int32_t c_features, int32_t k,
                            int64_t diag_offset, int32_t exclude, int32_t splits, void* workspace, int64_t workspace_bytes,
                            int32_t* idx_out, float* val_out, void* stream);
int dae_csr_similarity_topk_workspace(int32_t n_query, int32_t n_corpus, int64_t corpus_nnz, int32_t n_features, int32_t k,
                                      int32_t splits, int64_t* bytes);

int dae_similarity_topk_excl_bf16x3(int32_t n_query, int32_t n_corpus, int32_t dim, const void* q_hi, const void* q_lo,
                                    int64_t ldq, const void* c_hi, const void* c_lo, int64_t ldc, int32_t k,
                                    int64_t diag_offset, int32_t exclude, int32_t splits, void* workspace,
                                    int64_t workspace_bytes, int32_t* idx_out, float* val_out, const int64_t* ex_indptr,
                                    const int32_t* ex_indices, int64_t ex_nnz, void* stream);
int dae_csr_similarity_topk_excl(const int64_t* q_indptr, const int32_t* q_indices, const float* q_values, int32_t n_query,
                                 int64_t q_nnz, int32_t q_features, const int64_t* c_indptr, const int32_t* c_indices,
                                 const float* c_values, int32_t n_corpus, int64_t c_nnz, int32_t c_features, int32_t k,
                                 int64_t diag_offset, int32_t exclude, int32_t splits, void* workspace, int64_t workspace_bytes,
                                 int32_t* idx_out, float* val_out, const int64_t* ex_indptr, const int32_t* ex_indices,
                                 int64_t ex_nnz, void* stream);

int dae_similarity_topk_groups_bf16x3(int32_t n_query, int32_t n_corpus, int32_t dim, const void* q_hi, const void* q_lo,
                                      int64_t ldq, const void* c_hi, const void* c_lo, int64_t ldc, int32_t k,
                                      int64_t diag_offset, int32_t exclude, int32_t splits, void* workspace,
                                      int64_t workspace_bytes, int32_t* idx_out, float* val_out, const int64_t* ex_indptr,
                                      const int32_t* ex_indices, int64_t ex_nnz, const int32_t* groups, void* stream);
int dae_csr_similarity_topk_groups(const int64_t* q_indptr, const int32_t* q_indices, const float* q_values, int32_t n_query,
                                   int64_t q_nnz, int32_t q_features, const int64_t* c_indptr, const int32_t* c_indices,
                                   const float* c_values, int32_t n_corpus, int64_t c_nnz, int32_t c_features, int32_t k,
                                   int64_t diag_offset, int32_t exclude, int32_t splits, void* workspace, int64_t workspace_bytes,
                                   int32_t* idx_out, float* val_out, const int64_t* ex_indptr, const int32_t* ex_indices,
                                   int64_t ex_nnz, const int32_t* groups, void* stream);

int dae_pair_partition(const float* S, int64_t lds, int32_t n, const int32_t* labels, float* related, float* unrelated,
                       uint64_t* cursors, void* stream);
int dae_auroc_count(const float* queries, int64_t n_queries, const float* sorted_targets, int64_t n_targets,
                    int32_t query_is_positive, uint64_t* twice_u, void* stream);

int dae_similarity_pair_hist_bf16x3(int32_t n, int32_t dim, const void* x_hi, const void* x_lo, int64_t ldx,
                                    const int32_t* labels, float range, int32_t bins, uint64_t* hist, double* sums,
                                    void* stream);
int dae_csr_similarity_pair_hist(const int64_t* indptr, const int32_t* indices, const float* values, int32_t n, int64_t nnz,
                                 int32_t n_features, const int32_t* labels, float range, int32_t bins, void* workspace,
                                 int64_t workspace_bytes, uint64_t* hist, double* sums, void* stream);
int dae_csr_similarity_pair_hist_workspace(int32_t n, int64_t nnz, int32_t n_features, int64_t* bytes);

int dae_similarity_pairs_bf16x3(int32_t n_query, int32_t n_corpus, int32_t dim, const void* q_hi, const void* q_lo, int64_t ldq,
                                const void* c_hi, const void* c_lo, int64_t ldc, int32_t self, float threshold, uint64_t* count,
                                int64_t capacity, int32_t* i_out, int32_t* j_out, float* s_out, void* stream);
int dae_csr_similarity_pairs(const int64_t* q_indptr, const int32_t* q_indices, const float* q_values, int32_t n_query,
                             int64_t q_nnz, int32_t q_features, const int64_t* c_indptr, const int32_t* c_indices,
                             const float* c_values, int32_t n_corpus, int64_t c_nnz, int32_t c_features, int32_t self,
                             float threshold, void* workspace, int64_t workspace_bytes, uint64_t* count, int64_t capacity,
                             int32_t* i_out, int32_t* j_out, float* s_out, void* stream);
int dae_csr_similarity_pairs_workspace(int32_t n_query, int32_t n_corpus, int64_t corpus_nnz, int32_t n_features, int64_t* bytes);
int dae_pairs_sort(int64_t n, int32_t n_corpus, int32_t key_bits, uint64_t* keys, uint64_t* keys_alt, float* s, float* s_alt,
                   void* workspace, int64_t workspace_bytes, int32_t* which, void* stream);
int dae_pairs_sort_workspace(int64_t n, int32_t key_bits, int64_t* bytes);

int dae_gemm_det_workspace(int64_t* bytes);
int dae_gemm_bf16x3_det(int32_t M, int32_t N, int32_t K, float alpha, const void* a_hi, const void* a_lo, int64_t lda,
                        int32_t a_mn_major, const void* b_hi, const void* b_lo, int64_t ldb, int32_t b_mn_major, float* C,
                        int64_t ldc, int32_t n_store, int32_t special_col, float* special_out, int32_t k_splits,
                        int32_t accumulate, void* workspace, int64_t workspace_bytes, void* stream);
int dae_gemm_sym_bf16x3_det(int32_t M, int32_t N, float alpha, const void* g_hi, const void* g_lo, int64_t ldg, const void* b_hi,
                            const void* b_lo, int64_t ldb, float* C, int64_t ldc, int32_t accumulate, void* workspace,
                            int64_t workspace_bytes, void* stream);
int dae_decode_loss_parts(int32_t F, int32_t* n_parts);
int dae_decode_fused_bf16x3_det(int32_t Brows, int32_t F, int32_t K, const void* e_hi, const void* e_lo,
                                int64_t lde, const void* w_hi, const void* w_lo, int64_t ldw,
                                const int64_t* indptr, const int32_t* indices, const float* values,
                                const int32_t* rows, const float* bv, int32_t dec_act, int32_t loss_func,
                                const float* weight, const double* stats, void* dz_hi, void* dz_lo,
                                int64_t ld_dz, float* row_loss_parts, int32_t* tile_ptr, int32_t prepared, void* stream);
int dae_encode_csr_bwd_det_workspace(int32_t n_rows, int32_t F, int32_t H, int64_t cap_nnz, int64_t* bytes);
int dae_encode_csr_bwd_det(const int64_t* indptr, const int32_t* indices, const float* values, const int32_t* rows,
                           int32_t n_rows, int32_t F, int32_t H, float in_scale, const float* E, const float* bh,
                           int32_t enc_act, float* dE, const float* dE_add, int64_t ldE, float* dbh, const int32_t* col_count,
                           int64_t cap_nnz, void* workspace, int64_t workspace_bytes, void* stream);
int dae_encode_sparse_dw_add(int32_t n_rows, int32_t F, int32_t H, int64_t cap_nnz, const void* workspace, int64_t workspace_bytes,
                             float* dW, void* stream);
int dae_triplet_batch_all_det(const float* S, int64_t lds, int32_t B, const int32_t* seg_lo, const int32_t* seg_hi,
                              float* G, int64_t ldg, double* stats, int32_t pos_only, void* g_hi, void* g_lo,
                              int64_t ld_split, double* loss_slots, void* stream);
int dae_triplet_batch_hard_det(const float* S, int64_t lds, int32_t B, const float* labels, float* G, int64_t ldg,
                               float* weight, double* stats, double* loss_slots, void* stream);
int dae_triplet_batch_all_rows_det(const float* S_blk, int64_t lds, int32_t row0, int32_t n_rows, int32_t B, const int32_t* seg_lo,
                                   const int32_t* seg_hi, float* G_blk, int64_t ldg, double* stats, int32_t pos_only, void* g_hi,
                                   void* g_lo, int64_t ld_split, double* loss_slots, void* stream);
int dae_triplet_batch_hard_rows_det(const float* S_blk, int64_t lds, int32_t row0, int32_t n_rows, int32_t B, const float* labels,
                                    float* G_blk, int64_t ldg, float* weight, double* stats, double* loss_slots, void* stream);
int dae_triplet_explicit_det(const float* E, const float* Ep, const float* En, int32_t B, int32_t H, int64_t ld,
                             float alpha, float* dE, float* dEp, float* dEn, double* stats, double* loss_slots, void* stream);
int dae_triplet_loss_sum(const double* loss_slots, int32_t n, double* stats, void* stream);

int dae_gather_split_bf16(const float* src, int64_t ld_src, const int32_t* rows, int32_t n_rows, int32_t cols, void* hi, void* lo,
                          int64_t ld_dst, int32_t ones_col, void* stream);
int dae_gru_cell_fwd(int32_t n, int32_t H, const float* xp, int64_t ld_xp, const float* hp, int64_t ld_hp, const float* h_prev,
                     int64_t ld_hprev, float* h_out, int64_t ld_h, int32_t n_split, void* h_hi, void* h_lo, int64_t ld_split,
                     float* gates, int64_t ld_gates, void* stream);
int dae_gru_cell_bwd(int32_t n, int32_t H, const float* dh_in, int64_t ld_dh_in, float* carry, int64_t ld_carry, const float* gates,
                     int64_t ld_gates, const float* h_prev, int64_t ld_hprev, void* dxp_hi, void* dxp_lo, void* dhp_hi, void* dhp_lo,
                     int64_t ld_g, void* stream);
int dae_seq_negatives(const int32_t* pos, int64_t n_pos, int32_t n_items, uint64_t seed, uint64_t epoch, uint64_t batch, int32_t* neg,
                      void* stream);
int dae_seq_rank_loss(const float* h, int64_t ld_h, const float* emb, int64_t ld_emb, int32_t H, const int32_t* pos, const int32_t* neg,
                      int64_t n_pos, float scale, float* dh, int64_t ld_dh, double* loss_sum, void* stream);

int dae_allreduce_multimem(float* multicast_grad, void* const* peer_flags, uint32_t* epochs, int32_t rank,
                           int32_t world, int64_t n, int32_t n_blocks, void* stream);

#ifdef __cplusplus
}
#endif
#endif
```

Measured before the change: 2.289 million.

## Pair tail row-tiles in decode, retune sym GEMM K-block, tighten triplet sweep

The fused decode kernel gains a tail schedule: when the last M tile is at most half full and W fits in L2, each tail work item loads a 64-row A slice once and covers two N tiles using a separate three-stage ring, so the partial tile does not waste a full 128-row MMA. The symmetric bf16x3 GEMM moves to a K block of 32 with four stages instead of 64 with two. The triplet sweep now walks only the valid j groups, strided by ty, instead of padded Pj tiles, and the tiled batch-all kernel gets a minimum of three blocks per SM in its launch bounds. These changes add scheduling complexity, and the register cap from the launch bound could cause spills.

After: 2.313 million (median of 6 runs). 1.01x the previous value.

```diff
diff --git a/dae_rnn_news_recommendation_b200/_cabi.py b/dae_rnn_news_recommendation_b200/_cabi.py
--- a/dae_rnn_news_recommendation_b200/_cabi.py
+++ b/dae_rnn_news_recommendation_b200/_cabi.py
@@ -43,6 +43,7 @@
     'dae_sym_split_bf16': (C.c_int, [p, i32, i64, f32, p, p, i64, p]),
     'dae_gemm_bf16x3': (C.c_int, [i32, i32, i32, f32, p, p, i64, i32, p, p, i64, i32, p, i64, i32, i32, p, i32, i32, p]),
     'dae_gemm_config': (C.c_int, [i32, i32]),
+    'dae_decode_config': (C.c_int, [i32]),
     'dae_decode_prepare': (C.c_int, [i32, i32, p, p, p, p, p, p]),
     'dae_decode_fused_bf16x3': (C.c_int, [i32, i32, i32, p, p, i64, p, p, i64, p, p, p, p, p, i32, i32, p, p, p, p, i64, p, p, i32, p]),
     'dae_reduce_parts': (C.c_int, [p, i32, i32, p, p]),
diff --git a/dae_rnn_news_recommendation_b200/csrc/gemm_tc.cu b/dae_rnn_news_recommendation_b200/csrc/gemm_tc.cu
--- a/dae_rnn_news_recommendation_b200/csrc/gemm_tc.cu
+++ b/dae_rnn_news_recommendation_b200/csrc/gemm_tc.cu
@@ -156,6 +156,7 @@
   const int32_t* tile_ptr;
   float* sk_ws;
   int loss_parts;
+  int tail_pairs;
 };
 
 struct Sched {
@@ -540,11 +541,63 @@
 template <int R> __device__ __forceinline__ void regs_dec() { asm volatile("setmaxnreg.dec.sync.aligned.u32 %0;" ::"n"(R)); }
 template <int R> __device__ __forceinline__ void regs_inc() { asm volatile("setmaxnreg.inc.sync.aligned.u32 %0;" ::"n"(R)); }
 
+constexpr int kTailStages = 3;
+constexpr int kTailA = 64 * kDecodeBK * 2, kTailB = kDecodeN * kDecodeBK * 2;
+constexpr int kTailStageBytes = 2 * kTailA + 4 * kTailB;
+static_assert(kTailStages * kTailStageBytes <= kDecodeStages * (2 * BLOCK_M * kDecodeBK * 2 + 2 * kDecodeN * kDecodeBK * 2),
+              "the tail stages share the operand ring");
+
+struct DecodeSched {
+  int tiles_m, full_m, n_tail, n_items, kb_total, w;
+  __device__ __forceinline__ void init(const GemmParams& p) {
+    tiles_m = (p.M + BLOCK_M - 1) / BLOCK_M;
+    n_tail = p.tail_pairs;
+    full_m = n_tail ? tiles_m - 1 : tiles_m;
+    n_items = n_tail + full_m * ((p.N + kDecodeN - 1) / kDecodeN);
+    kb_total = (p.K + kDecodeBK - 1) / kDecodeBK;
+    w = (int)blockIdx.x;
+  }
+  __device__ __forceinline__ bool next_tail(int& mb, int& nb) {
+    if (w >= n_tail) return false;
+    mb = tiles_m - 1; nb = 2 * w;
+    w += (int)gridDim.x;
+    return true;
+  }
+  __device__ __forceinline__ bool next(int& mb, int& nb, int& kb0, int& kb1) {
+    if (w >= n_items) return false;
+    const int t = w - n_tail;
+    mb = t % full_m; nb = t / full_m; kb0 = 0; kb1 = kb_total;
+    w += (int)gridDim.x;
+    return true;
+  }
+};
+
+__device__ __forceinline__ void mma_tail_item(float (&acc)[kDecodeN / 2], uint8_t* smem, uint64_t* full_bar, uint64_t* empty_bar, int h,
+                                              int lane, int& stage, uint32_t& phase, int kb_total) {
+  int prev = -1;
+  for (int kb = 0; kb < kb_total; ++kb) {
+    mbar_wait(&full_bar[stage], phase);
+    const uint32_t sa_hi = smem_u32(smem + stage * kTailStageBytes), sa_lo = sa_hi + kTailA;
+    const uint32_t sb_hi = sa_hi + 2 * kTailA + h * 2 * kTailB, sb_lo = sb_hi + kTailB;
+    wgmma_fence();
+    mma_kblock<kDecodeN, 0, 0, kDecodeBK>(acc, sa_hi, sa_lo, sb_hi, sb_lo, kb == 0);
+    wgmma_commit();
+    wgmma_wait<1>();
+    if (prev >= 0) { __syncwarp(); if (lane == 0) mbar_arrive(&empty_bar[prev]); }
+    prev = stage;
+    if (++stage == kTailStages) { stage = 0; phase ^= 1; }
+  }
+  wgmma_wait<0>();
+  if (prev >= 0) { __syncwarp(); if (lane == 0) mbar_arrive(&empty_bar[prev]); }
+}
+
 template <int ACT, int LOSS>
 __global__ void __launch_bounds__(kDecodeThreads, 1) decode_fused_kernel(const __grid_constant__ CUtensorMap tm_a_hi,
                                                                          const __grid_constant__ CUtensorMap tm_a_lo,
                                                                          const __grid_constant__ CUtensorMap tm_b_hi,
                                                                          const __grid_constant__ CUtensorMap tm_b_lo,
+                                                                         const __grid_constant__ CUtensorMap tm_t_hi,
+                                                                         const __grid_constant__ CUtensorMap tm_t_lo,
                                                                          const GemmParams p) {
   constexpr int BLOCK_N = kDecodeN, STAGES = kDecodeStages, BK = kDecodeBK;
   constexpr int STAGE_BYTES = 2 * BLOCK_M * BK * 2 + 2 * BLOCK_N * BK * 2;
@@ -556,17 +609,22 @@
   uint8_t* smem = reinterpret_cast<uint8_t*>((reinterpret_cast<uintptr_t>(smem_raw) + 1023) & ~(uintptr_t)1023);
   float* stg = reinterpret_cast<float*>(smem + STAGES * STAGE_BYTES);
   __shared__ __align__(8) uint64_t full_bar[STAGES], empty_bar[STAGES], staged_bar[2], drained_bar[2];
+  __shared__ __align__(8) uint64_t tfull_bar[kTailStages], tempty_bar[kTailStages];
   __shared__ float s_bias[2][BLOCK_N];
   __shared__ float s_biasc[kFast ? 2 : 1][kFast ? BLOCK_N : 1];
   __shared__ __align__(16) uint8_t s_stage[8][2][32][48];
 
   const int warp = threadIdx.x >> 5, lane = threadIdx.x & 31;
   const int role = warp >> 2;
-  Sched sched;
-
-  if (warp == 0 && lane == 0) { prefetch_tmap(&tm_a_hi); prefetch_tmap(&tm_a_lo); prefetch_tmap(&tm_b_hi); prefetch_tmap(&tm_b_lo); }
+  DecodeSched sched;
+
+  if (warp == 0 && lane == 0) {
+    prefetch_tmap(&tm_a_hi); prefetch_tmap(&tm_a_lo); prefetch_tmap(&tm_b_hi); prefetch_tmap(&tm_b_lo);
+    if (p.tail_pairs) { prefetch_tmap(&tm_t_hi); prefetch_tmap(&tm_t_lo); }
+  }
   if (warp == 1 && lane == 0) {
     for (int s = 0; s < STAGES; ++s) { mbar_init(&full_bar[s], 1); mbar_init(&empty_bar[s], 8); }
+    for (int s = 0; s < kTailStages; ++s) { mbar_init(&tfull_bar[s], 1); mbar_init(&tempty_bar[s], 8); }
     for (int h = 0; h < 2; ++h) { mbar_init(&staged_bar[h], 4); mbar_init(&drained_bar[h], 4); }
     fence_barrier_init();
   }
@@ -574,21 +632,52 @@
 
   if (role == 0) {
     regs_dec<kRegsProducer>();
-    sched.init(p, BLOCK_N, 0, BK);
-    if (warp == 0 && lane == 0)
+    sched.init(p);
+    if (warp == 0 && lane == 0) {
+      const int tiles_n = (p.N + BLOCK_N - 1) / BLOCK_N;
+      int stage = 0; uint32_t phase = 0;
+      int mb, nb;
+      while (sched.next_tail(mb, nb)) {
+        const int nb1 = min(nb + 1, tiles_n - 1);
+        for (int kb = 0; kb < sched.kb_total; ++kb) {
+          mbar_wait(&tempty_bar[stage], phase ^ 1);
+          uint8_t* s = smem + stage * kTailStageBytes;
+          mbar_expect_tx(&tfull_bar[stage], kTailStageBytes);
+          tma_load_2d(&tm_t_hi, &tfull_bar[stage], s, kb * BK, mb * BLOCK_M);
+          tma_load_2d(&tm_t_lo, &tfull_bar[stage], s + kTailA, kb * BK, mb * BLOCK_M);
+          tma_load_2d(&tm_b_hi, &tfull_bar[stage], s + 2 * kTailA, kb * BK, nb * BLOCK_N);
+          tma_load_2d(&tm_b_lo, &tfull_bar[stage], s + 2 * kTailA + kTailB, kb * BK, nb * BLOCK_N);
+          tma_load_2d(&tm_b_hi, &tfull_bar[stage], s + 2 * kTailA + 2 * kTailB, kb * BK, nb1 * BLOCK_N);
+          tma_load_2d(&tm_b_lo, &tfull_bar[stage], s + 2 * kTailA + 3 * kTailB, kb * BK, nb1 * BLOCK_N);
+          if (++stage == kTailStages) { stage = 0; phase ^= 1; }
+        }
+      }
+      if (p.tail_pairs) {
+        for (int s = 0; s < kTailStages; ++s) {
+          mbar_wait(&tempty_bar[stage], phase ^ 1);
+          if (++stage == kTailStages) { stage = 0; phase ^= 1; }
+        }
+      }
       tma_produce<BLOCK_N, STAGES, 0, BK>(p, sched, smem, full_bar, empty_bar, 0u, &tm_a_hi, &tm_a_lo, &tm_b_hi, &tm_b_lo, &tm_a_hi, &tm_a_lo);
+    }
   } else if (role <= 2) {
     regs_inc<kRegsMma>();
-    sched.init(p, BLOCK_N, 0, BK);
+    sched.init(p);
     const int h = role - 1;
     const int wi = warp & 3;
     float acc[BLOCK_N / 2];
 #pragma unroll
     for (int i = 0; i < BLOCK_N / 2; ++i) acc[i] = 0.0f;
-    int stage = 0; uint32_t phase = 0, tphase = 0;
+    int stage = 0, tstage = 0; uint32_t phase = 0, tphase = 0, ttphase = 0;
     int mb, nb, kb0, kb1;
-    while (sched.next(mb, nb, kb0, kb1)) {
-      mma_work_item<BLOCK_N, STAGES, 0, 0, BK>(acc, p, smem, full_bar, empty_bar, h, lane, 0u, stage, phase, kb0, kb1);
+    for (;;) {
+      if (sched.next_tail(mb, nb)) {
+        mma_tail_item(acc, smem, tfull_bar, tempty_bar, h, lane, tstage, ttphase, sched.kb_total);
+      } else if (sched.next(mb, nb, kb0, kb1)) {
+        mma_work_item<BLOCK_N, STAGES, 0, 0, BK>(acc, p, smem, full_bar, empty_bar, h, lane, 0u, stage, phase, kb0, kb1);
+      } else {
+        break;
+      }
       mbar_wait(&drained_bar[h], tphase ^ 1);
       const int r0 = h * 64 + wi * 16 + (lane >> 2), c0 = 2 * (lane & 3);
 #pragma unroll
@@ -602,7 +691,7 @@
     }
   } else {
     regs_inc<kRegsEpilogue>();
-    sched.init(p, BLOCK_N, 0, BK);
+    sched.init(p);
     const int h = role - 3;
     const int ew = warp - 12;
     const int wi = warp & 3;
@@ -616,9 +705,18 @@
     const int rsub = lane >> 1, csub = lane & 1;
     uint32_t tphase = 0;
     int mb, nb, kb0, kb1;
-    while (sched.next(mb, nb, kb0, kb1)) {
+    for (;;) {
+      int row0;
+      if (sched.next_tail(mb, nb)) {
+        nb += h;
+        row0 = (nb < tiles_n) ? mb * BLOCK_M - 64 * h : p.M;
+      } else if (sched.next(mb, nb, kb0, kb1)) {
+        row0 = mb * BLOCK_M;
+      } else {
+        break;
+      }
       const float* srow = stg + row_in_tile * SROW + half * HALF_N;
-      const int m = mb * BLOCK_M + row_in_tile;
+      const int m = row0 + row_in_tile;
       const int n0 = nb * BLOCK_N + half * HALF_N;
       int64_t pc = 0, pe = 0;
       int c0 = 0x7fffffff, c1 = 0x7fffffff, c2 = 0x7fffffff;
@@ -645,7 +743,7 @@
       const float inv_sc = (sc != 0.0f) ? 1.0f / sc : 0.0f;
       const bool edge = (n0 + HALF_N > p.N);
       float lsum = 0.0f;
-      const int m_base = mb * BLOCK_M + quarter * 32;
+      const int m_base = row0 + quarter * 32;
       const int n_lim = edge ? p.N : 0x7fffffff;
 #pragma unroll 1
       for (int c = 0; c < HALF_N / 16; ++c) {
@@ -1352,6 +1450,7 @@
 
 static int g_pair_mode = -1;
 static int g_lean = 0;
+constexpr int kSymBK = 32;
 
 template <int BLOCK_N, int STAGES, int PAIR, int MAJ, int BK = BLOCK_K>
 static int launch_gemm_maj(const Operand& A, const Operand& B, GemmParams p, cudaStream_t st, int* grid_out = nullptr) {
@@ -1378,8 +1477,8 @@
   CUtensorMap tat_hi = ta_hi, tat_lo = ta_lo;
   if (p.a_sym_kb > 0) {
     if (PAIR || A.mn_major) { set_error("dae_gemm_sym_bf16x3: unsupported configuration"); return DAE_ERR_UNSUPPORTED; }
-    if ((rc = make_map(&tat_hi, A.hi, p.M, p.M, A.ld, 64))) return rc;
-    if ((rc = make_map(&tat_lo, A.lo, p.M, p.M, A.ld, 64))) return rc;
+    if ((rc = make_map(&tat_hi, A.hi, p.M, p.M, A.ld, BK))) return rc;
+    if ((rc = make_map(&tat_lo, A.lo, p.M, p.M, A.ld, BK))) return rc;
   }
   constexpr int smem = STAGES * (2 * BLOCK_M * BK * 2 + 2 * BLOCK_N * BK * 2) + BLOCK_M * (BLOCK_N + 4) * 4 + 1024;
   int tiles_m = (p.M + BLOCK_M - 1) / BLOCK_M;
@@ -1463,21 +1562,40 @@
 
 static int64_t sk_workspace_bytes() { return (int64_t)2 * sm_count() * BLOCK_M * 128 * (int64_t)sizeof(float); }
 
+static int g_decode_pair_tail = 1;
+
+static int64_t l2_bytes() {
+  static int64_t n[64] = {0};
+  int dev = 0;
+  if (cudaGetDevice(&dev) != cudaSuccess || dev < 0 || dev >= 64) return 0;
+  if (!n[dev]) {
+    int v = 0;
+    if (cudaDeviceGetAttribute(&v, cudaDevAttrL2CacheSize, dev) != cudaSuccess || v < 0) v = 0;
+    n[dev] = v;
+  }
+  return n[dev];
+}
+
 template <int ACT, int LOSS>
-static int launch_decode(const Operand& A, const Operand& B, const GemmParams& p, cudaStream_t st) {
-  CUtensorMap ta_hi, ta_lo, tb_hi, tb_lo;
+static int launch_decode(const Operand& A, const Operand& B, GemmParams p, cudaStream_t st) {
+  CUtensorMap ta_hi, ta_lo, tb_hi, tb_lo, tt_hi, tt_lo;
   int rc;
   if ((rc = make_map(&ta_hi, A.hi, p.K, p.M, A.ld, BLOCK_M, kDecodeBK))) return rc;
   if ((rc = make_map(&ta_lo, A.lo, p.K, p.M, A.ld, BLOCK_M, kDecodeBK))) return rc;
   if ((rc = make_map(&tb_hi, B.hi, p.K, p.N, B.ld, kDecodeN, kDecodeBK))) return rc;
   if ((rc = make_map(&tb_lo, B.lo, p.K, p.N, B.ld, kDecodeN, kDecodeBK))) return rc;
+  if ((rc = make_map(&tt_hi, A.hi, p.K, p.M, A.ld, 64, kDecodeBK))) return rc;
+  if ((rc = make_map(&tt_lo, A.lo, p.K, p.M, A.ld, 64, kDecodeBK))) return rc;
   constexpr int smem = kDecodeStages * (2 * BLOCK_M * kDecodeBK * 2 + 2 * kDecodeN * kDecodeBK * 2) + BLOCK_M * (kDecodeN + 4) * 4 + 1024;
   auto kern = decode_fused_kernel<ACT, LOSS>;
   static bool attr_done[64] = {false};
   if ((rc = ensure_smem_attr(kern, smem, attr_done))) return rc;
-  const int tiles = ((p.M + BLOCK_M - 1) / BLOCK_M) * ((p.N + kDecodeN - 1) / kDecodeN);
-  const int n = tiles < sm_count() ? tiles : sm_count();
-  kern<<<n, kDecodeThreads, smem, st>>>(ta_hi, ta_lo, tb_hi, tb_lo, p);
+  const int tiles_m = (p.M + BLOCK_M - 1) / BLOCK_M, tiles_n = (p.N + kDecodeN - 1) / kDecodeN, rem = p.M % BLOCK_M;
+  const bool w_in_l2 = (int64_t)p.N * B.ld * 4 <= l2_bytes() / 2;
+  p.tail_pairs = (g_decode_pair_tail && w_in_l2 && rem >= 1 && rem <= 64) ? (tiles_n + 1) / 2 : 0;
+  const int items = p.tail_pairs + (p.tail_pairs ? tiles_m - 1 : tiles_m) * tiles_n;
+  const int n = items < sm_count() ? items : sm_count();
+  kern<<<n, kDecodeThreads, smem, st>>>(ta_hi, ta_lo, tb_hi, tb_lo, tt_hi, tt_lo, p);
   return DAE_OK;
 }
 
@@ -1581,6 +1699,11 @@
 extern "C" int dae_gemm_config(int32_t pair_mode, int32_t lean) {
   dae::g_pair_mode = pair_mode < 0 ? -1 : (pair_mode ? 1 : 0);
   dae::g_lean = lean ? 1 : 0;
+  return DAE_OK;
+}
+
+extern "C" int dae_decode_config(int32_t pair_tail) {
+  dae::g_decode_pair_tail = pair_tail ? 1 : 0;
   return DAE_OK;
 }
 
@@ -1637,12 +1760,12 @@
   DAE_REQUIRE(ldg % 8 == 0 && ldb % 8 == 0 && ldg >= M && ldb >= N, "dae_gemm_sym_bf16x3: leading dimensions must be multiples of 8 and cover the matrices");
   DAE_REQUIRE(((uintptr_t)g_hi | (uintptr_t)g_lo | (uintptr_t)b_hi | (uintptr_t)b_lo) % 16 == 0, "dae_gemm_sym_bf16x3: operands must be 16-byte aligned");
   GemmParams p{};
-  const int kb_half = (M + BLOCK_K - 1) / BLOCK_K;
-  p.M = M; p.N = N; p.K = 2 * kb_half * BLOCK_K; p.k_splits = 1; p.stream_k = 1; p.atomic = 1; p.alpha = alpha;
+  const int kb_half = (M + kSymBK - 1) / kSymBK;
+  p.M = M; p.N = N; p.K = 2 * kb_half * kSymBK; p.k_splits = 1; p.stream_k = 1; p.atomic = 1; p.alpha = alpha;
   p.C = C; p.ldc = ldc; p.n_store = N; p.special_col = -1; p.special_out = nullptr; p.a_sym_kb = kb_half;
   if (!accumulate) DAE_CUDA(cudaMemset2DAsync(C, ldc * sizeof(float), 0, (size_t)N * sizeof(float), M, (cudaStream_t)stream));
   Operand A{g_hi, g_lo, ldg, 0}, B{b_hi, b_lo, ldb, 1};
-  int rc = launch_gemm_maj<128, 2, 0, 6>(A, B, p, (cudaStream_t)stream);
+  int rc = launch_gemm_maj<128, 4, 0, 6, kSymBK>(A, B, p, (cudaStream_t)stream);
   if (rc) return rc;
   DAE_CHECK_LAUNCH("dae_gemm_sym_bf16x3");
   return DAE_OK;
@@ -1700,13 +1823,13 @@
               (long long)workspace_bytes, (long long)sk_workspace_bytes());
   cudaStream_t st = (cudaStream_t)stream;
   GemmParams p{};
-  const int kb_half = (M + BLOCK_K - 1) / BLOCK_K;
-  p.M = M; p.N = N; p.K = 2 * kb_half * BLOCK_K; p.k_splits = 1; p.stream_k = 1; p.atomic = accumulate ? 1 : 0; p.alpha = alpha;
+  const int kb_half = (M + kSymBK - 1) / kSymBK;
+  p.M = M; p.N = N; p.K = 2 * kb_half * kSymBK; p.k_splits = 1; p.stream_k = 1; p.atomic = accumulate ? 1 : 0; p.alpha = alpha;
   p.C = C; p.ldc = ldc; p.n_store = N; p.special_col = -1; p.special_out = nullptr; p.a_sym_kb = kb_half;
   p.sk_ws = (float*)workspace;
   Operand A{g_hi, g_lo, ldg, 0}, B{b_hi, b_lo, ldb, 1};
   int n = 0;
-  int rc = launch_gemm_maj<128, 2, 0, 6>(A, B, p, st, &n);
+  int rc = launch_gemm_maj<128, 4, 0, 6, kSymBK>(A, B, p, st, &n);
   if (rc) return rc;
   DAE_REQUIRE(n <= kMaxFixupCtas, "dae_gemm_sym_bf16x3_det: %d stream-K CTAs exceed the fixup's %d", n, kMaxFixupCtas);
   const int tm = (M + 127) / 128, tn = (N + 127) / 128;
diff --git a/dae_rnn_news_recommendation_b200/csrc/triplet.cu b/dae_rnn_news_recommendation_b200/csrc/triplet.cu
--- a/dae_rnn_news_recommendation_b200/csrc/triplet.cu
+++ b/dae_rnn_news_recommendation_b200/csrc/triplet.cu
@@ -101,11 +101,13 @@
 
 template <int TIER>
 __device__ __forceinline__ void triplet_sweep(const float* sj, const float* uj, float* gj, const float* sk, const float* vk, float* gk,
-                                              int Pj, int Pk, int Pk_max, int tx, int ty, float& lacc, int& npos) {
-  for (int jt = 0; jt < Pj; jt += kJTile) {
+                                              int nj, int Pk, int Pk_max, int tx, int ty, float& lacc, int& npos) {
+  const int n_grp = (nj + kTJ - 1) / kTJ;
+  for (int grp = ty; grp < n_grp; grp += kTY) {
+    const int jt = grp * kTJ;
     float s_j[kTJ], u_j[kTJ], rs[kTJ];
 #pragma unroll
-    for (int a = 0; a < kTJ; ++a) { s_j[a] = sj[jt + ty * kTJ + a]; u_j[a] = uj[jt + ty * kTJ + a]; rs[a] = 0.0f; }
+    for (int a = 0; a < kTJ; ++a) { s_j[a] = sj[jt + a]; u_j[a] = uj[jt + a]; rs[a] = 0.0f; }
     if (TIER == 0) {
       const f2 U01 = pk(u_j[0], u_j[1]), U23 = pk(u_j[2], u_j[3]);
       f2 rs01 = pk(0.0f, 0.0f), rs23 = pk(0.0f, 0.0f);
@@ -162,7 +164,7 @@
 #pragma unroll
     for (int a = 0; a < kTJ; ++a) {
       const float t = warp_sum(rs[a]);
-      if (tx == 0) gj[jt + ty * kTJ + a] = t;
+      if (tx == 0) gj[jt + a] = t;
     }
   }
 }
@@ -235,10 +237,10 @@
 
   float lacc = 0.0f;
   int npos = 0;
-  if (tier == 0) triplet_sweep<0>(sj, uj, gj, sk, vk, gk, Pj, Pk, Pk_max, tx, ty, lacc, npos);
-  else if (tier == 1) triplet_sweep<1>(sj, uj, gj, sk, vk, gk, Pj, Pk, Pk_max, tx, ty, lacc, npos);
-  else if (tier == 2) triplet_sweep<2>(sj, uj, gj, sk, vk, gk, Pj, Pk, Pk_max, tx, ty, lacc, npos);
-  else triplet_sweep<3>(sj, uj, gj, sk, vk, gk, Pj, Pk, Pk_max, tx, ty, lacc, npos);
+  if (tier == 0) triplet_sweep<0>(sj, uj, gj, sk, vk, gk, nj, Pk, Pk_max, tx, ty, lacc, npos);
+  else if (tier == 1) triplet_sweep<1>(sj, uj, gj, sk, vk, gk, nj, Pk, Pk_max, tx, ty, lacc, npos);
+  else if (tier == 2) triplet_sweep<2>(sj, uj, gj, sk, vk, gk, nj, Pk, Pk_max, tx, ty, lacc, npos);
+  else triplet_sweep<3>(sj, uj, gj, sk, vk, gk, nj, Pk, Pk_max, tx, ty, lacc, npos);
   __syncthreads();
   const float inv = pos_only ? 1.0f : (float)(1.0 / (stats[DAE_STAT_N_VALID] + 1e-16));
   for (int c = tid; c < B; c += kTripThreads) {
@@ -271,7 +273,7 @@
 constexpr int kChunkK = 1024;
 static_assert(kChunkJ % kJTile == 0 && kChunkK % kKTile == 0, "chunks must hold whole register tiles");
 
-__global__ void __launch_bounds__(kTripThreads) triplet_batch_all_tiled_kernel(const float* __restrict__ S, int64_t lds, int row0, int B,
+__global__ void __launch_bounds__(kTripThreads, 3) triplet_batch_all_tiled_kernel(const float* __restrict__ S, int64_t lds, int row0, int B,
                                                                                const int32_t* __restrict__ seg_lo,
                                                                                const int32_t* __restrict__ seg_hi, float* G, int64_t ldg,
                                                                                double* __restrict__ stats, int pos_only,
@@ -345,10 +347,10 @@
       }
       __syncthreads();
       float lacc = 0.0f;
-      if (tier == 0) triplet_sweep<0>(sj, uj, gj, sk, vk, gk, Pj, Pk, kChunkK, tx, ty, lacc, npos);
-      else if (tier == 1) triplet_sweep<1>(sj, uj, gj, sk, vk, gk, Pj, Pk, kChunkK, tx, ty, lacc, npos);
-      else if (tier == 2) triplet_sweep<2>(sj, uj, gj, sk, vk, gk, Pj, Pk, kChunkK, tx, ty, lacc, npos);
-      else triplet_sweep<3>(sj, uj, gj, sk, vk, gk, Pj, Pk, kChunkK, tx, ty, lacc, npos);
+      if (tier == 0) triplet_sweep<0>(sj, uj, gj, sk, vk, gk, cj, Pk, kChunkK, tx, ty, lacc, npos);
+      else if (tier == 1) triplet_sweep<1>(sj, uj, gj, sk, vk, gk, cj, Pk, kChunkK, tx, ty, lacc, npos);
+      else if (tier == 2) triplet_sweep<2>(sj, uj, gj, sk, vk, gk, cj, Pk, kChunkK, tx, ty, lacc, npos);
+      else triplet_sweep<3>(sj, uj, gj, sk, vk, gk, cj, Pk, kChunkK, tx, ty, lacc, npos);
       lsum += (double)lacc;
       __syncthreads();
       for (int p = tid; p < cj; p += kTripThreads) {
diff --git a/include/dae_sm100.h b/include/dae_sm100.h
--- a/include/dae_sm100.h
+++ b/include/dae_sm100.h
@@ -104,6 +104,7 @@
                         const void* b_hi, const void* b_lo, int64_t ldb, float* C, int64_t ldc, int32_t accumulate,
                         void* stream);
 int dae_gemm_config(int32_t pair_mode, int32_t lean);
+int dae_decode_config(int32_t pair_tail);
 int dae_decode_prepare(int32_t Brows, int32_t F, const int64_t* indptr, const int32_t* indices, const int32_t* rows,
                        float* row_loss_part, int32_t* tile_ptr, void* stream);
 int dae_decode_fused_bf16x3(int32_t Brows, int32_t F, int32_t K, const void* e_hi, const void* e_lo,
```
